# martingoe/physics

Hardware: AMD Instinct MI355X
Metric: rigid_body_steps_per_sec (higher is better)
Workload: dtype f32; 1 GPU; C5_256000_tower; n_bodies=256000, bodies_per_gpu=256000, dt_nanos=16666667, preroll_steps=30, rccl_ranks=0

## Files before the change

include/physics_hip.h:

```cpp
#ifndef PHYSICS_HIP_H
#define PHYSICS_HIP_H

#include <stdint.h>

#ifdef __cplusplus
extern "C" {
#endif

#define PHYS_ABI_VERSION 2u

#define PHYS_OK 0
#define PHYS_ERR_INVALID_ARG (-1)
#define PHYS_ERR_NO_DEVICE (-2)
#define PHYS_ERR_HIP (-3)
#define PHYS_ERR_SINGULAR_INERTIA (-4)
#define PHYS_ERR_CAPACITY (-5)
#define PHYS_ERR_OUT_OF_RANGE (-6)
#define PHYS_ERR_UNSUPPORTED (-7)
#define PHYS_ERR_NO_BODIES (-8)

#define PHYS_SHAPE_NONE 0u
#define PHYS_SHAPE_SPHERE 1u
#define PHYS_SHAPE_BOX 2u
#define PHYS_SHAPE_CAPSULE 3u

#define PHYS_FLAG_COLLISIONS 0x1u
#define PHYS_FLAG_GROUND_PLANE 0x2u
#define PHYS_FLAG_EXACT_ROTATION 0x4u
#define PHYS_FLAG_BROADPHASE_ONLY 0x8u
#define PHYS_FLAG_SOLVER_PER_COLOR 0x10u
#define PHYS_FLAG_SHARED_GPU 0x20u
#define PHYS_FLAG_EXCLUSIVE_GPU 0x80u
#define PHYS_FLAG_SOLVER_CLUSTER 0x40u
#define PHYS_FLAG_NO_WARM_START 0x100u

typedef struct phys_config {
    uint32_t abi_version;
    int32_t device;
    uint32_t flags;
    float gravity_force[3];
    float gravity_offset[3];
    uint32_t cg_max_iterations;
    float cg_max_error;
    float cg_min_error;
    uint32_t solver_iterations;
    float baumgarte;
    float slop;
    float friction;
    float contact_margin;
    float ground_height;
    float max_bias;
    uint64_t max_pairs;
    uint64_t max_manifolds;
    uint64_t max_ghosts;
} phys_config;

typedef struct phys_world phys_world;

typedef struct phys_stats {
    uint64_t n_bodies;
    uint64_t n_pairs;
    uint64_t n_manifolds;
    uint64_t n_contacts;
    uint32_t n_colors;
    uint32_t color_rounds;
    uint32_t cg_iterations;
    int32_t cg_converged;
    uint64_t steps;
    uint32_t overflow;
    uint32_t n_ground_manifolds;
    float max_extent;
    uint32_t n_halo_records;
    uint64_t n_cross_pairs;
    uint32_t n_ghosts;
    uint32_t n_new_manifolds;
} phys_stats;

void phys_config_default(phys_config* cfg);
const char* phys_last_error(void);
uint32_t phys_abi_version(void);

int32_t phys_create(const phys_config* cfg, phys_world** out);
int32_t phys_destroy(phys_world* w);

int32_t phys_set_bodies(phys_world* w, uint64_t n, const float* pos , const float* rot_ijkw ,
                        const float* lin_vel , const float* ang_vel , const float* mass ,
                        const float* inertia , const uint32_t* shape_type ,
                        const float* half_extent );

int32_t phys_add_constraint_fix_point(phys_world* w, uint64_t body, const float target[3]);
int32_t phys_add_constraint_fix_orientation(phys_world* w, uint64_t body, const float target_rpy[3]);
int32_t phys_clear_constraints(phys_world* w);

int32_t phys_apply_force_centre_of_gravity(phys_world* w, uint64_t body, const float force[3]);
int32_t phys_apply_force_at_position(phys_world* w, uint64_t body, const float force[3], const float point[3]);
int32_t phys_apply_force_at_offset(phys_world* w, uint64_t body, const float force[3], const float offset[3]);

int32_t phys_set_forces(phys_world* w, const float* force , const float* torque );

int32_t phys_update(phys_world* w, uint64_t dt_nanos);
int32_t phys_apply_gravity(phys_world* w);
int32_t phys_step(phys_world* w, uint64_t dt_nanos);
int32_t phys_update_n(phys_world* w, uint64_t dt_nanos, uint32_t n);
int32_t phys_sync(phys_world* w);

int32_t phys_get_transforms(phys_world* w, float* pos_out , float* rot_ijkw_out );
int32_t phys_get_velocities(phys_world* w, float* lin_out , float* ang_out );
int32_t phys_get_forces(phys_world* w, float* force_out , float* torque_out );
int32_t phys_get_instance_matrices(phys_world* w, float* out );
int32_t phys_get_lambda(phys_world* w, float* lambda_out, uint64_t cap, uint64_t* n_rows);

int32_t phys_block_spmv(int32_t device, uint64_t nrows, uint64_t ncols, uint64_t nblocks, const uint64_t* block_desc ,
                        const float* data, const float* vec, uint64_t vec_len, int32_t transpose, float* out);

int32_t phys_broadphase(phys_world* w, uint32_t* pairs_out , uint64_t cap, uint64_t* n_pairs);
int32_t phys_get_aabbs(phys_world* w, float* out );
int32_t phys_get_manifolds(phys_world* w, uint32_t* ids_out , uint32_t* counts_out ,
                           float* normals_out , float* points_out , uint64_t cap,
                           uint64_t* n_manifolds);
int32_t phys_get_stats(phys_world* w, phys_stats* out);
int32_t phys_get_color_counts(phys_world* w, uint32_t* counts_out );

#define PHYS_RAY_MISS 0xFFFFFFFEu
#define PHYS_RAY_GROUND 0xFFFFFFFFu
int32_t phys_raycast(phys_world* w, uint64_t n_rays, const float* origin , const float* dir ,
                     const float* max_t , const uint32_t* ignore_body ,
                     uint32_t* body_out , float* t_out , float* normal_out );
int32_t phys_raycast_device(phys_world* w, uint64_t n_rays, const float* origin, const float* dir, const float* max_t,
                            const uint32_t* ignore_body, uint32_t* body_out, float* t_out, float* normal_out);

int32_t phys_spherecast(phys_world* w, uint64_t n, const float* origin , const float* dir ,
                        const float* radius , const float* max_t ,
                        const uint32_t* ignore_body ,
                        uint32_t* body_out , float* t_out , float* normal_out );
int32_t phys_spherecast_device(phys_world* w, uint64_t n, const float* origin, const float* dir, const float* radius,
                               const float* max_t, const uint32_t* ignore_body, uint32_t* body_out, float* t_out,
                               float* normal_out);
int32_t phys_overlap(phys_world* w, uint64_t n, const uint32_t* shape_type , const float* pos ,
                     const float* rot_ijkw , const float* half_extent ,
                     const uint32_t* ignore_body ,
                     uint64_t cap, uint64_t* offsets_out , uint32_t* ids_out );

#define PHYS_STATIC_ID_BIT 0x80000000u
int32_t phys_set_static_bodies(phys_world* w, uint64_t n, const float* pos , const float* rot_ijkw ,
                               const uint32_t* shape_type , const float* half_extent );
int32_t phys_get_static_stats(phys_world* w, uint64_t* n_static, uint64_t* n_static_pairs, uint64_t* n_static_manifolds);

#define PHYS_FILTER_DEFAULT_CATEGORY 0x0001u
#define PHYS_FILTER_DEFAULT_MASK 0xFFFFu
int32_t phys_set_body_filters(phys_world* w, uint64_t n, const uint16_t* category ,
                              const uint16_t* mask , const int16_t* group );
int32_t phys_get_body_filters(phys_world* w, uint16_t* category_out , uint16_t* mask_out ,
                              int16_t* group_out );
int32_t phys_set_static_filters(phys_world* w, uint64_t n, const uint16_t* category ,
                                const uint16_t* mask , const int16_t* group );
int32_t phys_set_ground_filter(phys_world* w, uint16_t category, uint16_t mask);
int32_t phys_raycast_filtered(phys_world* w, uint64_t n_rays, const float* origin , const float* dir ,
                              const float* max_t , const uint32_t* ignore_body ,
                              const uint16_t* query_mask , uint32_t* body_out , float* t_out ,
                              float* normal_out );
int32_t phys_raycast_device_filtered(phys_world* w, uint64_t n_rays, const float* origin, const float* dir, const float* max_t,
                                     const uint32_t* ignore_body, const uint16_t* query_mask, uint32_t* body_out, float* t_out,
                                     float* normal_out);
int32_t phys_spherecast_filtered(phys_world* w, uint64_t n, const float* origin , const float* dir ,
                                 const float* radius , const float* max_t ,
                                 const uint32_t* ignore_body , const uint16_t* query_mask ,
                                 uint32_t* body_out , float* t_out , float* normal_out );
int32_t phys_spherecast_device_filtered(phys_world* w, uint64_t n, const float* origin, const float* dir, const float* radius,
                                        const float* max_t, const uint32_t* ignore_body, const uint16_t* query_mask,
                                        uint32_t* body_out, float* t_out, float* normal_out);
int32_t phys_overlap_filtered(phys_world* w, uint64_t n, const uint32_t* shape_type , const float* pos ,
                              const float* rot_ijkw , const float* half_extent ,
                              const uint32_t* ignore_body , const uint16_t* query_mask ,
                              uint64_t cap, uint64_t* offsets_out , uint32_t* ids_out );

int32_t phys_set_body_materials(phys_world* w, uint64_t n, const float* friction ,
                                const float* restitution );
int32_t phys_get_body_materials(phys_world* w, float* friction_out , float* restitution_out );
int32_t phys_set_static_materials(phys_world* w, uint64_t n, const float* friction ,
                                  const float* restitution );
int32_t phys_set_ground_material(phys_world* w, float friction, float restitution);
int32_t phys_set_restitution_threshold(phys_world* w, float v );

#define PHYS_CONTACT_BEGIN 1u
#define PHYS_CONTACT_END   2u
typedef struct phys_contact_event {
    uint32_t body_a, body_b;
    uint32_t kind;
    uint32_t step;
    float point[3];
    float impulse;
    float normal[3];
    uint32_t reserved;
} phys_contact_event;

int32_t phys_contact_events_enable(phys_world* w, uint64_t capacity);
int32_t phys_get_contact_events(phys_world* w, phys_contact_event* out, uint64_t cap, uint64_t* n, uint64_t* n_dropped);
int32_t phys_get_contact_impulses(phys_world* w, float* out , uint64_t cap, uint64_t* n_manifolds);

#define PHYS_MAX_TRIGGERS 1024u
#define PHYS_TRIGGER_ENTER 1u
#define PHYS_TRIGGER_EXIT  2u
typedef struct phys_trigger_event {
    uint32_t trigger;
    uint32_t body;
    uint32_t kind;
    uint32_t step;
} phys_trigger_event;

int32_t phys_set_triggers(phys_world* w, uint64_t n, const uint32_t* shape_type , const float* pos ,
                          const float* rot_ijkw , const float* half_extent ,
                          const uint16_t* mask );
int32_t phys_set_trigger_poses(phys_world* w, uint64_t n , const float* pos ,
                               const float* rot_ijkw );
int32_t phys_trigger_events_enable(phys_world* w, uint64_t capacity);
int32_t phys_get_trigger_events(phys_world* w, phys_trigger_event* out, uint64_t cap, uint64_t* n, uint64_t* n_dropped);
int32_t phys_get_trigger_overlaps(phys_world* w, uint64_t cap, uint64_t* offsets_out , uint32_t* ids_out );

#define PHYS_STAGE_STEP_FULL 0u
#define PHYS_STAGE_VELOCITY_AABB 1u
#define PHYS_STAGE_GRID 2u
#define PHYS_STAGE_PAIRS 3u
#define PHYS_STAGE_NARROW 4u
#define PHYS_STAGE_COLOR 5u
#define PHYS_STAGE_ROWS 6u
#define PHYS_STAGE_SOLVE 7u
#define PHYS_STAGE_POSITION 8u
#define PHYS_STAGE_CONSTRAINTS 9u
#define PHYS_STAGE_MISC 10u
#define PHYS_STAGE_SOLVE_TAIL 11u
#define PHYS_STAGE_SOLVE_FLOW 12u
#define PHYS_STAGE_SOLVE_CLUSTER 13u
#define PHYS_STAGE_COUNT 14u
typedef struct phys_profile {
    double ms[PHYS_STAGE_COUNT];
    uint64_t launches[PHYS_STAGE_COUNT];
    uint64_t steps;
} phys_profile;
int32_t phys_profile_enable(phys_world* w, int32_t on);
int32_t phys_profile_get(phys_world* w, phys_profile* out);

typedef struct phys_device_view {
    uint64_t n;
    float* pos;
    float* rot;
    float* lin_vel;
    float* ang_vel;
    float* aabb;
    void* stream;
    uint64_t vel_stride;
} phys_device_view;
int32_t phys_get_device_view(phys_world* w, phys_device_view* out);

int32_t phys_set_global_ids(phys_world* w, const uint32_t* global_ids );
int32_t phys_halo_pack(phys_world* w, float x_lo, float x_hi, float reach, void* dev_records_out, uint64_t cap,
                       uint64_t* n_records);
int32_t phys_halo_pairs(phys_world* w, const void* dev_remote_records, uint64_t n_remote, uint64_t skip_first,
                        uint64_t skip_count, uint64_t* n_cross_pairs);
int32_t phys_get_cross_pairs(phys_world* w, uint32_t* pairs_out , uint64_t cap, uint64_t* n_pairs);

#define PHYS_HALO_BODY_RECORD_BYTES 96u
int32_t phys_set_slab(phys_world* w, float x_lo, float x_hi, float reach);
int32_t phys_halo_pack_bodies(phys_world* w, void* dev_records_out, uint64_t cap);
int32_t phys_halo_pack_bodies_face(phys_world* w, void* dev_records_out, uint64_t cap, int32_t face);
int32_t phys_halo_unpack_ghosts(phys_world* w, const void* dev_records, uint64_t n_records, uint64_t skip_first,
                                uint64_t skip_count);
int32_t phys_get_global_ids(phys_world* w, uint32_t* out );

// ... 23 lines not shown
```

include/spec/collide.h:

```cpp
#ifndef PHYS_SPEC_COLLIDE_H
#define PHYS_SPEC_COLLIDE_H

#include <stdint.h>

#include "vec.h"

#define PHYS_GROUND_ID 0xFFFFFFFFu
#ifndef PHYS_STATIC_ID_BIT
#define PHYS_STATIC_ID_BIT 0x80000000u
#endif
#define PHYS_IS_STATIC_PARTNER(b) (((b) & PHYS_STATIC_ID_BIT) != 0u)
#define PHYS_SPEC_SHAPE_NONE 0u
#define PHYS_SPEC_SHAPE_SPHERE 1u
#define PHYS_SPEC_SHAPE_BOX 2u
#define PHYS_SPEC_SHAPE_CAPSULE 3u

typedef struct { v3 lo, hi; } aabb_t;

typedef struct {
    v3 c;
    m33 R;
    v3 h;
    uint32_t type;
} geom_t;
// ... 76 lines not shown

PHYS_HD void collide_sphere_sphere(const geom_t* A, const geom_t* B, float margin, manifold_t* m) {
    const v3 d = v3_sub(B->c, A->c);
    const float dist2 = v3_dot(d, d);
    const float r = A->h.x + B->h.x;
    const float reach = r + margin;
    if (dist2 > reach * reach) return;
    const float dist = det_sqrtf(dist2);
    v3 n = v3_make(0.0f, 1.0f, 0.0f);
    if (dist > 1.0e-12f) n = v3_div(d, dist);
    const float depth = r - dist;
    m->normal = n;
    m->count = 1;
    m->pt[0] = v3_add(A->c, v3_scale(n, A->h.x - 0.5f * depth));
    m->depth[0] = depth;
}

PHYS_HD void collide_sphere_box_raw(const geom_t* S, const geom_t* X, float margin, manifold_t* m) {
    const v3 p = m33_tmul_v3(&X->R, v3_sub(S->c, X->c));
    v3 q;
    q.x = det_maxf(-X->h.x, det_minf(p.x, X->h.x));
    q.y = det_maxf(-X->h.y, det_minf(p.y, X->h.y));
    q.z = det_maxf(-X->h.z, det_minf(p.z, X->h.z));
    const float r = S->h.x;
    v3 nl;
    float depth;
    if (q.x == p.x && q.y == p.y && q.z == p.z) {
        const float fx = X->h.x - det_absf(p.x), fy = X->h.y - det_absf(p.y), fz = X->h.z - det_absf(p.z);
        if (fx <= fy && fx <= fz) { nl = v3_make(p.x < 0.0f ? -1.0f : 1.0f, 0.0f, 0.0f); depth = fx + r; q.x = p.x < 0.0f ? -X->h.x : X->h.x; }
        else if (fy <= fz)        { nl = v3_make(0.0f, p.y < 0.0f ? -1.0f : 1.0f, 0.0f); depth = fy + r; q.y = p.y < 0.0f ? -X->h.y : X->h.y; }
        else                      { nl = v3_make(0.0f, 0.0f, p.z < 0.0f ? -1.0f : 1.0f); depth = fz + r; q.z = p.z < 0.0f ? -X->h.z : X->h.z; }
    } else {
        const v3 dl = v3_sub(p, q);
        const float dist2 = v3_dot(dl, dl);
        const float reach = r + margin;
        if (dist2 > reach * reach) return;
        const float dist = det_sqrtf(dist2);
        nl = v3_div(dl, dist);
        depth = r - dist;
    }
    const v3 nw = m33_mul_v3(&X->R, nl);
    m->normal = v3_neg(nw);
    m->count = 1;
    m->pt[0] = v3_add(X->c, m33_mul_v3(&X->R, q));
    m->depth[0] = depth;
}

PHYS_HD int clip_poly(v3* p, int n_in, v3 c, v3 u, float lim) {
    int n_out = 0;
    if (n_in <= 0) return 0;
    const v3 first = p[0];
    v3 a = first;
    float da = v3_dot(v3_sub(a, c), u) - lim;
    for (int k = 0; k < 8; ++k) {
        if (k >= n_in) break;
        v3 b = first;
        if (k + 1 != n_in) b = p[k + 1];
        const float db = v3_dot(v3_sub(b, c), u) - lim;
        if (da <= 0.0f) {
            if (n_out < 8) p[n_out++] = a;
            if (db > 0.0f) {
                const float t = da / (da - db);
                if (n_out < 8) p[n_out++] = v3_add(a, v3_scale(v3_sub(b, a), t));
            }
        } else if (db <= 0.0f) {
            const float t = da / (da - db);
            if (n_out < 8) p[n_out++] = v3_add(a, v3_scale(v3_sub(b, a), t));
        }
        a = b; da = db;
    }
    return n_out;
}

PHYS_HD void manifold_reduce(const v3* p, const float* depth, int n, v3 normal, manifold_t* m) {
    if (n <= 4) {
        m->count = n;
        PHYS_UNROLL
        for (int k = 0; k < 4; ++k) if (k < n) { m->pt[k] = p[k]; m->depth[k] = depth[k]; }
        return;
    }
    int i0 = 0;
    for (int k = 1; k < 8; ++k) if (k < n && depth[k] > depth[i0]) i0 = k;
    int i1 = -1; float best = -1.0f;
    for (int k = 0; k < 8; ++k) if (k < n && k != i0) {
        const v3 d = v3_sub(p[k], p[i0]);
        const float dd = v3_dot(d, d);
        if (dd > best) { best = dd; i1 = k; }
    }
    int i2 = -1, i3 = -1; float amax = 0.0f, amin = 0.0f;
    const v3 e = v3_sub(p[i1], p[i0]);
    for (int k = 0; k < 8; ++k) if (k < n && k != i0 && k != i1) {
        const float area = v3_dot(v3_cross(e, v3_sub(p[k], p[i0])), normal);
        if (area > amax) { amax = area; i2 = k; }
        if (area < amin) { amin = area; i3 = k; }
    }
    m->pt[0] = p[i0]; m->depth[0] = depth[i0];
    m->pt[1] = p[i1]; m->depth[1] = depth[i1];
    const int has2 = i2 >= 0, has3 = i3 >= 0;
    const int s2 = has2 ? i2 : i3;
    if (has2 || has3) { m->pt[2] = p[s2]; m->depth[2] = depth[s2]; }
    if (has2 && has3) { m->pt[3] = p[i3]; m->depth[3] = depth[i3]; }
    m->count = 2 + has2 + has3;
}

PHYS_HD void box_face_contact(const geom_t* Ref, const geom_t* Inc, int r, float sgn, float margin, v3 n_ab,
                              manifold_t* m, clip_ws_t* ws) {
    const v3 nref = v3_scale(m33_col(&Ref->R, r), sgn);
    const float d0 = v3_dot(nref, m33_col(&Inc->R, 0));
    const float d1 = v3_dot(nref, m33_col(&Inc->R, 1));
    const float d2 = v3_dot(nref, m33_col(&Inc->R, 2));
    int j = 0; float dj = d0;
    if (det_absf(d1) > det_absf(dj)) { j = 1; dj = d1; }
    if (det_absf(d2) > det_absf(dj)) { j = 2; dj = d2; }
    const float jsgn = dj > 0.0f ? -1.0f : 1.0f;
    const int j1 = (j + 1) % 3, j2 = (j + 2) % 3;
    const v3 fc = v3_add(Inc->c, v3_scale(m33_col(&Inc->R, j), jsgn * v3_get(Inc->h, j)));
    const v3 e1 = v3_scale(m33_col(&Inc->R, j1), v3_get(Inc->h, j1));
    const v3 e2 = v3_scale(m33_col(&Inc->R, j2), v3_get(Inc->h, j2));
    v3* polyA = ws->poly;
    polyA[0] = v3_add(v3_add(fc, e1), e2);
    polyA[1] = v3_add(v3_sub(fc, e1), e2);
    polyA[2] = v3_sub(v3_sub(fc, e1), e2);
    polyA[3] = v3_sub(v3_add(fc, e1), e2);
    int n = 4;
    const int r1 = (r + 1) % 3, r2 = (r + 2) % 3;
    const v3 u1 = m33_col(&Ref->R, r1), u2 = m33_col(&Ref->R, r2);
    const float l1 = v3_get(Ref->h, r1), l2 = v3_get(Ref->h, r2);
    n = clip_poly(polyA, n, Ref->c, u1, l1);
    n = clip_poly(polyA, n, Ref->c, v3_neg(u1), l1);
    n = clip_poly(polyA, n, Ref->c, u2, l2);
    n = clip_poly(polyA, n, Ref->c, v3_neg(u2), l2);
    float lo1 = 3.0e38f, hi1 = -3.0e38f, lo2 = 3.0e38f, hi2 = -3.0e38f;
    v3* cand = ws->poly; float* cdep = ws->depth; int nc = 0;
    const float hr = v3_get(Ref->h, r);
    float deepest = -3.0e38f;
    for (int k = 0; k < 8; ++k) {
        if (k >= n) break;
        const v3 rel = v3_sub(polyA[k], Ref->c);
        const float c1 = v3_dot(rel, u1), c2 = v3_dot(rel, u2);
        lo1 = det_minf(lo1, c1); hi1 = det_maxf(hi1, c1);
        lo2 = det_minf(lo2, c2); hi2 = det_maxf(hi2, c2);
        const float dep = hr - v3_dot(rel, nref);
        if (dep >= -margin) { cand[nc] = polyA[k]; cdep[nc] = dep; deepest = det_maxf(deepest, dep); ++nc; }
    }
    {
        const float kSliverRel = 0.1f, kSliverDepth = 0.25f;
        const float width = det_minf(hi1 - lo1, hi2 - lo2);
        const float face = det_minf(det_minf(l1, l2), det_minf(v3_get(Inc->h, j1), v3_get(Inc->h, j2)));
        if (nc > 0 && width < kSliverRel * face && deepest <= kSliverDepth * margin) nc = 0;
    }
    manifold_reduce(cand, cdep, nc, n_ab, m);
}

PHYS_HD void collide_box_box(const geom_t* A, const geom_t* B, float margin, manifold_t* m, clip_ws_t* ws) {
    const v3 d = v3_sub(B->c, A->c);
    float C[3][3], absC[3][3], tA[3], tB[3], hA[3], hB[3];
    hA[0] = A->h.x; hA[1] = A->h.y; hA[2] = A->h.z;
    hB[0] = B->h.x; hB[1] = B->h.y; hB[2] = B->h.z;
    PHYS_UNROLL
    for (int i = 0; i < 3; ++i) {
        const v3 ai = m33_col(&A->R, i);
        tA[i] = v3_dot(d, ai);
        PHYS_UNROLL
        for (int j = 0; j < 3; ++j) {
            C[i][j] = v3_dot(ai, m33_col(&B->R, j));
            absC[i][j] = det_absf(C[i][j]) + 1.0e-6f;
        }
    }
    PHYS_UNROLL
    for (int j = 0; j < 3; ++j) tB[j] = v3_dot(d, m33_col(&B->R, j));

    float aMax = -3.0e38f; int aAxis = 0;
    PHYS_UNROLL
    for (int i = 0; i < 3; ++i) {
        const float s = det_absf(tA[i]) - (hA[i] + ((absC[i][0] * hB[0] + absC[i][1] * hB[1]) + absC[i][2] * hB[2]));
        if (s > margin) return;
        if (s > aMax) { aMax = s; aAxis = i; }
    }
    float bMax = -3.0e38f; int bAxis = 0;
    PHYS_UNROLL
    for (int j = 0; j < 3; ++j) {
        const float s = det_absf(tB[j]) - (hB[j] + ((absC[0][j] * hA[0] + absC[1][j] * hA[1]) + absC[2][j] * hA[2]));
        if (s > margin) return;
        if (s > bMax) { bMax = s; bAxis = j; }
    }
    float eMax = -3.0e38f; int eI = -1, eJ = -1;
    PHYS_UNROLL
    for (int i = 0; i < 3; ++i) {
        const int i1 = (i + 1) % 3, i2 = (i + 2) % 3;
        PHYS_UNROLL
        for (int j = 0; j < 3; ++j) {
            const int j1 = (j + 1) % 3, j2 = (j + 2) % 3;
            const float len2 = 1.0f - C[i][j] * C[i][j];
            if (len2 < 1.0e-4f) continue;
            const float ra = hA[i1] * absC[i2][j] + hA[i2] * absC[i1][j];
            const float rb = hB[j1] * absC[i][j2] + hB[j2] * absC[i][j1];
            const float dist = det_absf(tA[i2] * C[i1][j] - tA[i1] * C[i2][j]);
            const float s = (dist - (ra + rb)) / det_sqrtf(len2);
            if (s > margin) return;
            if (s > eMax) { eMax = s; eI = i; eJ = j; }
        }
    }
    const float kRel = 0.95f, kAbs = 0.01f;
    const float faceMax = det_maxf(aMax, bMax);
    if (eI >= 0 && eMax > kRel * faceMax + kAbs) {
        const v3 ai = m33_col(&A->R, eI), bj = m33_col(&B->R, eJ);
        v3 n = v3_cross(ai, bj);
        const float nl = v3_norm(n);
        n = v3_div(n, nl);
        if (v3_dot(n, d) < 0.0f) n = v3_neg(n);
        v3 pA = A->c, pB = B->c;
        PHYS_UNROLL
        for (int k = 0; k < 3; ++k) {
            if (k != eI) {
                const v3 ak = m33_col(&A->R, k);
                const float sg = v3_dot(n, ak) > 0.0f ? 1.0f : -1.0f;
                pA = v3_add(pA, v3_scale(ak, sg * hA[k]));
            }
            if (k != eJ) {
                const v3 bk = m33_col(&B->R, k);
                const float sg = v3_dot(n, bk) > 0.0f ? -1.0f : 1.0f;
                pB = v3_add(pB, v3_scale(bk, sg * hB[k]));
            }
        }
        const v3 w = v3_sub(pA, pB);
        const float b = v3_dot(ai, bj);
        const float dd = v3_dot(ai, w), ee = v3_dot(bj, w);
        const float den = 1.0f - b * b;
        const float sa = (b * ee - dd) / den;
        const float tb = (ee - b * dd) / den;
        const v3 qa = v3_add(pA, v3_scale(ai, sa));
        const v3 qb = v3_add(pB, v3_scale(bj, tb));
        m->normal = n;
        m->count = 1;
        m->pt[0] = v3_scale(v3_add(qa, qb), 0.5f);
        m->depth[0] = -eMax;
        return;
    }
    if (bMax > kRel * aMax + kAbs) {
        const float sgn = sel3(tB, bAxis) > 0.0f ? -1.0f : 1.0f;
        const v3 nref = v3_scale(m33_col(&B->R, bAxis), sgn);
        m->normal = v3_neg(nref);
        box_face_contact(B, A, bAxis, sgn, margin, m->normal, m, ws);
    } else {
        const float sgn = sel3(tA, aAxis) < 0.0f ? -1.0f : 1.0f;
        m->normal = v3_scale(m33_col(&A->R, aAxis), sgn);
        box_face_contact(A, B, aAxis, sgn, margin, m->normal, m, ws);
    }
}

PHYS_HD void collide_pair_sphere_box(const geom_t* A, const geom_t* B, float margin, manifold_t* m, clip_ws_t* ws) {
    manifold_clear(m);
    if (A->type == PHYS_SPEC_SHAPE_SPHERE && B->type == PHYS_SPEC_SHAPE_SPHERE) {
        collide_sphere_sphere(A, B, margin, m);
    } else if (A->type == PHYS_SPEC_SHAPE_SPHERE && B->type == PHYS_SPEC_SHAPE_BOX) {
        collide_sphere_box_raw(A, B, margin, m);
    } else if (A->type == PHYS_SPEC_SHAPE_BOX && B->type == PHYS_SPEC_SHAPE_SPHERE) {
        collide_sphere_box_raw(B, A, margin, m);
        m->normal = v3_neg(m->normal);
    } else if (A->type == PHYS_SPEC_SHAPE_BOX && B->type == PHYS_SPEC_SHAPE_BOX) {
        collide_box_box(A, B, margin, m, ws);
    }
}

PHYS_HD void collide_ground_sphere_box(const geom_t* A, float ground, float margin, manifold_t* m, clip_ws_t* ws) {
    manifold_clear(m);
    m->normal = v3_make(0.0f, -1.0f, 0.0f);
    if (A->type == PHYS_SPEC_SHAPE_SPHERE) {
        const float bottom = A->c.y - A->h.x;
        const float depth = ground - bottom;
        if (depth < -margin) return;
        m->count = 1;
        m->pt[0] = v3_make(A->c.x, bottom + 0.5f * depth, A->c.z);
        m->depth[0] = depth;
    } else if (A->type == PHYS_SPEC_SHAPE_BOX) {
        v3* cand = ws->poly; float* cdep = ws->depth; int nc = 0;
        const v3 ex = v3_scale(m33_col(&A->R, 0), A->h.x);
        const v3 ey = v3_scale(m33_col(&A->R, 1), A->h.y);
        const v3 ez = v3_scale(m33_col(&A->R, 2), A->h.z);
        for (int k = 0; k < 8; ++k) {
            v3 p = A->c;
            p = (k & 1) ? v3_add(p, ex) : v3_sub(p, ex);
            p = (k & 2) ? v3_add(p, ey) : v3_sub(p, ey);
            p = (k & 4) ? v3_add(p, ez) : v3_sub(p, ez);
            const float depth = ground - p.y;
            if (depth >= -margin) { cand[nc] = p; cdep[nc] = depth; ++nc; }
        }
        if (nc == 0) return;
        manifold_reduce(cand, cdep, nc, v3_make(0.0f, 1.0f, 0.0f), m);
    }
}



PHYS_HD v3 capsule_axis(const geom_t* A) { return v3_make(A->R.m[1], A->R.m[4], A->R.m[7]); }

PHYS_HD geom_t capsule_ball(v3 p, float r) {
    geom_t g;
    g.c = p;
    g.R.m[0] = 1.0f; g.R.m[1] = 0.0f; g.R.m[2] = 0.0f;
    g.R.m[3] = 0.0f; g.R.m[4] = 1.0f; g.R.m[5] = 0.0f;
    g.R.m[6] = 0.0f; g.R.m[7] = 0.0f; g.R.m[8] = 1.0f;
    g.h = v3_make(r, r, r);
    g.type = PHYS_SPEC_SHAPE_SPHERE;
    return g;
}

PHYS_HD float segment_param(v3 c, v3 u, float hl, v3 p) {
    const float uu = v3_dot(u, u);
    float s = 0.0f;
    if (uu > 1.0e-12f) s = v3_dot(v3_sub(p, c), u) / uu;
    return det_maxf(-hl, det_minf(s, hl));
}

PHYS_HD void segment_closest(v3 ca, v3 ua, float ha, v3 cb, v3 ub, float hb, float* s_out, float* t_out) {
    const v3 r = v3_sub(ca, cb);
    const float a = v3_dot(ua, ua), e = v3_dot(ub, ub), b = v3_dot(ua, ub);
    const float c = v3_dot(ua, r), f = v3_dot(ub, r);
    const float denom = a * e - b * b;
    float s = 0.0f, t = 0.0f;
    if (denom > 1.0e-4f * (a * e)) s = det_maxf(-ha, det_minf((b * f - c * e) / denom, ha));
    if (e > 1.0e-12f) t = (b * s + f) / e;
    if (t < -hb || t > hb) {
        t = t < -hb ? -hb : hb;
        s = a > 1.0e-12f ? det_maxf(-ha, det_minf((b * t - c) / a, ha)) : 0.0f;
    }
    *s_out = s;
    *t_out = t;
}

PHYS_HD void collide_capsule_sphere(const geom_t* A, const geom_t* B, float margin, manifold_t* m) {
    const v3 u = capsule_axis(A);
    const float s = segment_param(A->c, u, A->h.y, B->c);
    const geom_t S = capsule_ball(v3_add(A->c, v3_scale(u, s)), A->h.x);
    collide_sphere_sphere(&S, B, margin, m);
}

PHYS_HD void collide_capsule_capsule(const geom_t* A, const geom_t* B, float margin, manifold_t* m) {
    const v3 ua = capsule_axis(A), ub = capsule_axis(B);
    const float ra = A->h.x, rb = B->h.x;
    const float a = v3_dot(ua, ua), e = v3_dot(ub, ub), b = v3_dot(ua, ub);
    if (a > 1.0e-12f && e > 1.0e-12f && a * e - b * b <= 1.0e-4f * (a * e)) {
        const v3 d = v3_sub(B->c, A->c);
        const float sb = v3_dot(d, ua) / a;
        const float pb = B->h.y * (det_absf(b) / a);
        const float lo = det_maxf(-A->h.y, sb - pb), hi = det_minf(A->h.y, sb + pb);
        if (lo < hi) {
            const v3 perp = v3_sub(d, v3_scale(ua, sb));
            const float dist = v3_norm(perp);
            v3 n = v3_make(0.0f, 1.0f, 0.0f);
            if (dist > 1.0e-12f) n = v3_div(perp, dist);
            const float r = ra + rb;
            int nc = 0;
            PHYS_UNROLL
            for (int k = 0; k < 2; ++k) {
                const float s = k == 0 ? lo : hi;
                const v3 pa = v3_add(A->c, v3_scale(ua, s));
                const float t = segment_param(B->c, ub, B->h.y, pa);
                const v3 qb = v3_add(B->c, v3_scale(ub, t));
                const float depth = r - v3_dot(v3_sub(qb, pa), n);
                if (depth >= -margin) {
                    const v3 p = v3_add(pa, v3_scale(n, ra - 0.5f * depth));
                    if (nc == 0) { m->pt[0] = p; m->depth[0] = depth; }
                    else { m->pt[1] = p; m->depth[1] = depth; }
                    ++nc;
                }
            }
            m->normal = n;
            m->count = nc;
            return;
        }
    }
    float s, t;
    segment_closest(A->c, ua, A->h.y, B->c, ub, B->h.y, &s, &t);
    const geom_t SA = capsule_ball(v3_add(A->c, v3_scale(ua, s)), ra);
    const geom_t SB = capsule_ball(v3_add(B->c, v3_scale(ub, t)), rb);
    collide_sphere_sphere(&SA, &SB, margin, m);
}

PHYS_HD void capsule_edge_closest(v3 pc, v3 dl, float hl, v3 qe, v3 ue, float he, float* best, v3* bp, v3* bq) {
    float s, t;
    segment_closest(pc, dl, hl, qe, ue, he, &s, &t);
    const v3 p = v3_add(pc, v3_scale(dl, s)), q = v3_add(qe, v3_scale(ue, t));
    const v3 d = v3_sub(p, q);
    const float d2 = v3_dot(d, d);
    if (d2 < *best) { *best = d2; *bp = p; *bq = q; }
}

PHYS_HD void capsule_face_edges(v3 pc, v3 dl, float hl, int f, float sg, v3 e, float* best, v3* bp, v3* bq) {
    const int ja = f == 0 ? 1 : 0, ka = f == 2 ? 1 : 2;
    const float ef = f == 0 ? e.x : (f == 1 ? e.y : e.z);
    PHYS_UNROLL
    for (int k = 0; k < 4; ++k) {
        const int along = k < 2 ? ka : ja, across = k < 2 ? ja : ka;
        const float side = (k & 1) ? 1.0f : -1.0f;
        const float ec = across == 0 ? e.x : (across == 1 ? e.y : e.z);
        const float qx = f == 0 ? sg * ef : (across == 0 ? side * ec : 0.0f);
        const float qy = f == 1 ? sg * ef : (across == 1 ? side * ec : 0.0f);
        const float qz = f == 2 ? sg * ef : (across == 2 ? side * ec : 0.0f);
        const v3 ue = v3_make(along == 0 ? 1.0f : 0.0f, along == 1 ? 1.0f : 0.0f, along == 2 ? 1.0f : 0.0f);
        const float he = along == 0 ? e.x : (along == 1 ? e.y : e.z);
        capsule_edge_closest(pc, dl, hl, v3_make(qx, qy, qz), ue, he, best, bp, bq);
    }
}

PHYS_HD void capsule_box_point(const geom_t* A, const geom_t* B, v3 p, v3 q, v3 nf, float sep_f, float margin, manifold_t* m) {
    const float r = A->h.x;
    const v3 d = v3_sub(p, q);
    const float dist = v3_norm(d);
    v3 n = nf;
    float depth = r - sep_f;
    if (sep_f > 0.0f && dist > 1.0e-6f) { n = v3_div(d, dist); depth = r - dist; }
    if (depth < -margin) return;
    m->normal = v3_neg(m33_mul_v3(&B->R, n));
    m->count = 1;
    m->pt[0] = v3_add(B->c, m33_mul_v3(&B->R, v3_sub(p, v3_scale(n, r - 0.5f * depth))));
    m->depth[0] = depth;
}

PHYS_HD void collide_capsule_box(const geom_t* A, const geom_t* B, float margin, manifold_t* m) {
    const float r = A->h.x, hl = A->h.y;
    const v3 pc = m33_tmul_v3(&B->R, v3_sub(A->c, B->c));
    const v3 dl = m33_tmul_v3(&B->R, capsule_axis(A));
    const float ex = B->h.x, ey = B->h.y, ez = B->h.z;
    const float fx = det_absf(pc.x) - (ex + hl * det_absf(dl.x));
    const float fy = det_absf(pc.y) - (ey + hl * det_absf(dl.y));
    const float fz = det_absf(pc.z) - (ez + hl * det_absf(dl.z));
    if (fx - r > margin || fy - r > margin || fz - r > margin) return;
    int fAxis = 0; float fMax = fx;
    if (fy > fMax) { fAxis = 1; fMax = fy; }
    if (fz > fMax) { fAxis = 2; fMax = fz; }
    float eMax = -3.0e38f; int eAxis = -1;
    PHYS_UNROLL
    for (int i = 0; i < 3; ++i) {
        const v3 n = i == 0 ? v3_make(0.0f, dl.z, -dl.y) : (i == 1 ? v3_make(-dl.z, 0.0f, dl.x) : v3_make(dl.y, -dl.x, 0.0f));
        const float len2 = v3_dot(n, n);
        if (len2 < 1.0e-4f) continue;
        const float rb = (ex * det_absf(n.x) + ey * det_absf(n.y)) + ez * det_absf(n.z);
        const float s = (det_absf(v3_dot(pc, n)) - rb) / det_sqrtf(len2);
        if (s - r > margin) return;
        if (s > eMax) { eMax = s; eAxis = i; }
    }
    v3 nl;
    if (eAxis >= 0 && eMax > fMax + (0.05f * det_absf(fMax) + 0.01f)) {
        v3 n = eAxis == 0 ? v3_make(0.0f, dl.z, -dl.y) : (eAxis == 1 ? v3_make(-dl.z, 0.0f, dl.x) : v3_make(dl.y, -dl.x, 0.0f));
        n = v3_div(n, v3_norm(n));
        if (v3_dot(n, pc) < 0.0f) n = v3_neg(n);
        const float sx = n.x > 0.0f ? ex : -ex, sy = n.y > 0.0f ? ey : -ey, sz = n.z > 0.0f ? ez : -ez;
        const v3 qe = v3_make(eAxis == 0 ? 0.0f : sx, eAxis == 1 ? 0.0f : sy, eAxis == 2 ? 0.0f : sz);
        const v3 ue = v3_make(eAxis == 0 ? 1.0f : 0.0f, eAxis == 1 ? 1.0f : 0.0f, eAxis == 2 ? 1.0f : 0.0f);
        const float he = eAxis == 0 ? ex : (eAxis == 1 ? ey : ez);
        float best = 3.0e38f;
        v3 p = pc, q = qe;
        capsule_edge_closest(pc, dl, hl, qe, ue, he, &best, &p, &q);
        capsule_box_point(A, B, p, q, n, eMax, margin, m);
        return;
    }
    const float pf = fAxis == 0 ? pc.x : (fAxis == 1 ? pc.y : pc.z);
    const float sg = pf < 0.0f ? -1.0f : 1.0f;
    float lo = -hl, hi = hl;
    PHYS_UNROLL
    for (int j = 0; j < 3; ++j) {
        if (j == fAxis) continue;
        const float pj = j == 0 ? pc.x : (j == 1 ? pc.y : pc.z);
        const float dj = j == 0 ? dl.x : (j == 1 ? dl.y : dl.z);
        const float ej = j == 0 ? ex : (j == 1 ? ey : ez);
        if (dj == 0.0f) {
            if (det_absf(pj) > ej) { lo = 1.0f; hi = -1.0f; }
        } else {
            const float t0 = (-ej - pj) / dj, t1 = (ej - pj) / dj;
            lo = det_maxf(lo, det_minf(t0, t1));
            hi = det_minf(hi, det_maxf(t0, t1));
        }
    }
    if (lo <= hi) {
        nl = v3_make(fAxis == 0 ? sg : 0.0f, fAxis == 1 ? sg : 0.0f, fAxis == 2 ? sg : 0.0f);
        const float ef = fAxis == 0 ? ex : (fAxis == 1 ? ey : ez);
        const int ends = lo < hi ? 2 : 1;
        int nc = 0;
        PHYS_UNROLL
        for (int k = 0; k < 2; ++k) {
            if (k >= ends) break;
            const float s = k == 0 ? lo : hi;
            const v3 pa = v3_add(pc, v3_scale(dl, s));
            const float paf = fAxis == 0 ? pa.x : (fAxis == 1 ? pa.y : pa.z);
            const float depth = r - (sg * paf - ef);
            if (depth >= -margin) {
                const v3 p = v3_add(B->c, m33_mul_v3(&B->R, v3_sub(pa, v3_scale(nl, r - 0.5f * depth))));
                if (nc == 0) { m->pt[0] = p; m->depth[0] = depth; }
                else { m->pt[1] = p; m->depth[1] = depth; }
                ++nc;
            }
        }
        m->normal = v3_neg(m33_mul_v3(&B->R, nl));
        m->count = nc;
        const float sep = det_maxf(fMax, eMax);
        if (sep > 0.0f) {
            float best = 3.0e38f;
            v3 p = pc, q = pc;
            capsule_face_edges(pc, dl, hl, fAxis, sg, B->h, &best, &p, &q);
            const float edge_depth = r - det_sqrtf(best);
            const float deepest = nc == 0 ? -3.0e38f : (nc == 1 ? m->depth[0] : det_maxf(m->depth[0], m->depth[1]));
            if (edge_depth > deepest + 1.0e-6f) {
                manifold_clear(m);
                capsule_box_point(A, B, p, q, nl, sep, margin, m);
            }
        }
        return;
    }
    float best = 3.0e38f;
    v3 p = pc, q = pc;
    capsule_face_edges(pc, dl, hl, fAxis, sg, B->h, &best, &p, &q);
    capsule_box_point(A, B, p, q, v3_make(fAxis == 0 ? sg : 0.0f, fAxis == 1 ? sg : 0.0f, fAxis == 2 ? sg : 0.0f),
                      det_maxf(fMax, eMax), margin, m);
}

PHYS_HD void collide_capsule_any(const geom_t* A, const geom_t* B, float margin, manifold_t* m) {
    if (B->type == PHYS_SPEC_SHAPE_SPHERE) collide_capsule_sphere(A, B, margin, m);
    else if (B->type == PHYS_SPEC_SHAPE_CAPSULE) collide_capsule_capsule(A, B, margin, m);
    else if (B->type == PHYS_SPEC_SHAPE_BOX) collide_capsule_box(A, B, margin, m);
}

PHYS_HD void collide_pair(const geom_t* A, const geom_t* B, float margin, manifold_t* m, clip_ws_t* ws) {
    if (A->type == PHYS_SPEC_SHAPE_CAPSULE) {
        manifold_clear(m);
        collide_capsule_any(A, B, margin, m);
    } else if (B->type == PHYS_SPEC_SHAPE_CAPSULE) {
        manifold_clear(m);
        if (A->type != PHYS_SPEC_SHAPE_NONE) {
            collide_capsule_any(B, A, margin, m);
            m->normal = v3_neg(m->normal);
        }
    } else {
        collide_pair_sphere_box(A, B, margin, m, ws);
    }
}

PHYS_HD void collide_capsule_ground(const geom_t* A, float ground, float margin, manifold_t* m) {
    const v3 ax = v3_scale(capsule_axis(A), A->h.y);
    const v3 p0 = v3_sub(A->c, ax), p1 = v3_add(A->c, ax);
    const float b0 = p0.y - A->h.x, b1 = p1.y - A->h.x;
    const float d0 = ground - b0, d1 = ground - b1;
    const int k0 = d0 >= -margin;
    const int k1 = d1 >= -margin && !(p0.x == p1.x && p0.y == p1.y && p0.z == p1.z);
    const v3 q0 = v3_make(p0.x, b0 + 0.5f * d0, p0.z), q1 = v3_make(p1.x, b1 + 0.5f * d1, p1.z);
    if (k0) { m->pt[0] = q0; m->depth[0] = d0; }
    if (k1) {
        if (k0) { m->pt[1] = q1; m->depth[1] = d1; }
        else { m->pt[0] = q1; m->depth[0] = d1; }
    }
    m->count = k0 + k1;
}

PHYS_HD void collide_ground(const geom_t* A, float ground, float margin, manifold_t* m, clip_ws_t* ws) {
    if (A->type == PHYS_SPEC_SHAPE_CAPSULE) {
        manifold_clear(m);
        m->normal = v3_make(0.0f, -1.0f, 0.0f);
        collide_capsule_ground(A, ground, margin, m);
    } else {
        collide_ground_sphere_box(A, ground, margin, m, ws);
    }
}

#endif
```

physics_amd/_abi.py:

```python
import ctypes as C
import os

PHYS_ABI_VERSION = 2

PHYS_OK = 0
PHYS_ERR_INVALID_ARG = -1
PHYS_ERR_NO_DEVICE = -2
PHYS_ERR_HIP = -3
PHYS_ERR_SINGULAR_INERTIA = -4
PHYS_ERR_CAPACITY = -5
PHYS_ERR_OUT_OF_RANGE = -6
PHYS_ERR_UNSUPPORTED = -7
PHYS_ERR_NO_BODIES = -8

SHAPE_NONE, SHAPE_SPHERE, SHAPE_BOX = 0, 1, 2
SHAPE_CAPSULE = 3
FLAG_COLLISIONS, FLAG_GROUND_PLANE, FLAG_EXACT_ROTATION, FLAG_BROADPHASE_ONLY = 1, 2, 4, 8
FLAG_SOLVER_PER_COLOR = 16
FLAG_SHARED_GPU = 32
FLAG_SOLVER_CLUSTER = 64
FLAG_EXCLUSIVE_GPU = 128
FLAG_NO_WARM_START = 256
GROUND_ID = 0xFFFFFFFF
RAY_MISS = 0xFFFFFFFE
RAY_GROUND = 0xFFFFFFFF
STATIC_ID_BIT = 0x80000000
FILTER_DEFAULT_CATEGORY = 0x0001
FILTER_DEFAULT_MASK = 0xFFFF
CONTACT_BEGIN, CONTACT_END = 1, 2
MAX_TRIGGERS = 1024
TRIGGER_ENTER, TRIGGER_EXIT = 1, 2

f32p = C.POINTER(C.c_float)
u32p = C.POINTER(C.c_uint32)
u64p = C.POINTER(C.c_uint64)
u16p = C.POINTER(C.c_uint16)
i16p = C.POINTER(C.c_int16)


class PhysConfig(C.Structure):
    _fields_ = [
        ("abi_version", C.c_uint32),
        ("device", C.c_int32),
        ("flags", C.c_uint32),
        ("gravity_force", C.c_float * 3),
        ("gravity_offset", C.c_float * 3),
        ("cg_max_iterations", C.c_uint32),
        ("cg_max_error", C.c_float),
        ("cg_min_error", C.c_float),
        ("solver_iterations", C.c_uint32),
        ("baumgarte", C.c_float),
        ("slop", C.c_float),
        ("friction", C.c_float),
        ("contact_margin", C.c_float),
        ("ground_height", C.c_float),
        ("max_bias", C.c_float),
        ("max_pairs", C.c_uint64),
        ("max_manifolds", C.c_uint64),
        ("max_ghosts", C.c_uint64),
    ]


class PhysStats(C.Structure):
    _fields_ = [
        ("n_bodies", C.c_uint64),
        ("n_pairs", C.c_uint64),
        ("n_manifolds", C.c_uint64),
        ("n_contacts", C.c_uint64),
        ("n_colors", C.c_uint32),
        ("color_rounds", C.c_uint32),
        ("cg_iterations", C.c_uint32),
        ("cg_converged", C.c_int32),
        ("steps", C.c_uint64),
        ("overflow", C.c_uint32),
        ("n_ground_manifolds", C.c_uint32),
        ("max_extent", C.c_float),
        ("n_halo_records", C.c_uint32),
        ("n_cross_pairs", C.c_uint64),
        ("n_ghosts", C.c_uint32),
        ("n_new_manifolds", C.c_uint32),
    ]


STAGE_COUNT = 14
STAGE_NAMES = ["step_full", "velocity_aabb", "grid", "pairs", "narrow", "color", "rows", "solve", "position",
               "constraints", "misc", "solve_tail", "solve_flow", "solve_cluster"]


class PhysProfile(C.Structure):
    _fields_ = [("ms", C.c_double * STAGE_COUNT), ("launches", C.c_uint64 * STAGE_COUNT), ("steps", C.c_uint64)]


class PhysDeviceView(C.Structure):
    _fields_ = [
        ("n", C.c_uint64),
        ("pos", C.c_void_p),
        ("rot", C.c_void_p),
        ("lin_vel", C.c_void_p),
        ("ang_vel", C.c_void_p),
        ("aabb", C.c_void_p),
        ("stream", C.c_void_p),
        ("vel_stride", C.c_uint64),
    ]


class PhysContactEvent(C.Structure):
    _fields_ = [
        ("body_a", C.c_uint32),
        ("body_b", C.c_uint32),
        ("kind", C.c_uint32),
        ("step", C.c_uint32),
        ("point", C.c_float * 3),
        ("impulse", C.c_float),
        ("normal", C.c_float * 3),
        ("reserved", C.c_uint32),
    ]


class PhysTriggerEvent(C.Structure):
    _fields_ = [("trigger", C.c_uint32), ("body", C.c_uint32), ("kind", C.c_uint32), ("step", C.c_uint32)]


def default_config(**overrides):
    cfg = PhysConfig()
    cfg.abi_version = PHYS_ABI_VERSION
    cfg.device = 0
    cfg.flags = 0
    cfg.gravity_force[:] = (0.0, -9.81, 0.0)
    cfg.gravity_offset[:] = (0.0, 0.0, 1.5)
    cfg.cg_max_iterations = 1000
    cfg.cg_max_error = 1e-2
    cfg.cg_min_error = 1e-3
    cfg.solver_iterations = 8
    cfg.baumgarte = 0.2
    cfg.slop = 0.01
    cfg.friction = 0.5
    cfg.contact_margin = 0.02
    cfg.ground_height = 0.0
    cfg.max_bias = 3.0
    cfg.max_pairs = 0
    cfg.max_manifolds = 0
    cfg.max_ghosts = 0
    for k, v in overrides.items():
        if k in ("gravity_force", "gravity_offset"):
            getattr(cfg, k)[:] = tuple(v)
        else:
            setattr(cfg, k, v)
    return cfg


PROTOTYPES = {
    "phys_config_default": (None, [C.POINTER(PhysConfig)]),
    "phys_last_error": (C.c_char_p, []),
    "phys_abi_version": (C.c_uint32, []),
    "phys_create": (C.c_int32, [C.POINTER(PhysConfig), C.POINTER(C.c_void_p)]),
    "phys_destroy": (C.c_int32, [C.c_void_p]),
    "phys_set_bodies": (C.c_int32, [C.c_void_p, C.c_uint64, f32p, f32p, f32p, f32p, f32p, f32p, u32p, f32p]),
    "phys_add_constraint_fix_point": (C.c_int32, [C.c_void_p, C.c_uint64, f32p]),
    "phys_add_constraint_fix_orientation": (C.c_int32, [C.c_void_p, C.c_uint64, f32p]),
    "phys_clear_constraints": (C.c_int32, [C.c_void_p]),
    "phys_apply_force_centre_of_gravity": (C.c_int32, [C.c_void_p, C.c_uint64, f32p]),
    "phys_apply_force_at_position": (C.c_int32, [C.c_void_p, C.c_uint64, f32p, f32p]),
    "phys_apply_force_at_offset": (C.c_int32, [C.c_void_p, C.c_uint64, f32p, f32p]),
    "phys_set_forces": (C.c_int32, [C.c_void_p, f32p, f32p]),
    "phys_update": (C.c_int32, [C.c_void_p, C.c_uint64]),
    "phys_apply_gravity": (C.c_int32, [C.c_void_p]),
    "phys_step": (C.c_int32, [C.c_void_p, C.c_uint64]),
    "phys_update_n": (C.c_int32, [C.c_void_p, C.c_uint64, C.c_uint32]),
    "phys_sync": (C.c_int32, [C.c_void_p]),
    "phys_get_transforms": (C.c_int32, [C.c_void_p, f32p, f32p]),
    "phys_get_velocities": (C.c_int32, [C.c_void_p, f32p, f32p]),
    "phys_get_forces": (C.c_int32, [C.c_void_p, f32p, f32p]),
    "phys_get_instance_matrices": (C.c_int32, [C.c_void_p, f32p]),
    "phys_get_lambda": (C.c_int32, [C.c_void_p, f32p, C.c_uint64, u64p]),
    "phys_block_spmv": (C.c_int32, [C.c_int32, C.c_uint64, C.c_uint64, C.c_uint64, u64p, f32p, f32p, C.c_uint64, C.c_int32, f32p]),
    "phys_broadphase": (C.c_int32, [C.c_void_p, u32p, C.c_uint64, u64p]),
    "phys_get_aabbs": (C.c_int32, [C.c_void_p, f32p]),
    "phys_get_manifolds": (C.c_int32, [C.c_void_p, u32p, u32p, f32p, f32p, C.c_uint64, u64p]),
    "phys_get_stats": (C.c_int32, [C.c_void_p, C.POINTER(PhysStats)]),
    "phys_get_color_counts": (C.c_int32, [C.c_void_p, u32p]),
    "phys_raycast": (C.c_int32, [C.c_void_p, C.c_uint64, f32p, f32p, f32p, u32p, u32p, f32p, f32p]),
    "phys_raycast_device": (C.c_int32, [C.c_void_p, C.c_uint64, C.c_void_p, C.c_void_p, C.c_void_p, C.c_void_p, C.c_void_p,
                                        C.c_void_p, C.c_void_p]),
    "phys_spherecast": (C.c_int32, [C.c_void_p, C.c_uint64, f32p, f32p, f32p, f32p, u32p, u32p, f32p, f32p]),
    "phys_spherecast_device": (C.c_int32, [C.c_void_p, C.c_uint64, C.c_void_p, C.c_void_p, C.c_void_p, C.c_void_p, C.c_void_p,
                                           C.c_void_p, C.c_void_p, C.c_void_p]),
    "phys_overlap": (C.c_int32, [C.c_void_p, C.c_uint64, u32p, f32p, f32p, f32p, u32p, C.c_uint64, u64p, u32p]),
    "phys_set_static_bodies": (C.c_int32, [C.c_void_p, C.c_uint64, f32p, f32p, u32p, f32p]),
    "phys_set_body_filters": (C.c_int32, [C.c_void_p, C.c_uint64, u16p, u16p, i16p]),
    "phys_get_body_filters": (C.c_int32, [C.c_void_p, u16p, u16p, i16p]),
    "phys_set_static_filters": (C.c_int32, [C.c_void_p, C.c_uint64, u16p, u16p, i16p]),
    "phys_set_ground_filter": (C.c_int32, [C.c_void_p, C.c_uint16, C.c_uint16]),
    "phys_raycast_filtered": (C.c_int32, [C.c_void_p, C.c_uint64, f32p, f32p, f32p, u32p, u16p, u32p, f32p, f32p]),
    "phys_raycast_device_filtered": (C.c_int32, [C.c_void_p, C.c_uint64, C.c_void_p, C.c_void_p, C.c_void_p, C.c_void_p,
                                                 C.c_void_p, C.c_void_p, C.c_void_p, C.c_void_p]),
    "phys_spherecast_filtered": (C.c_int32, [C.c_void_p, C.c_uint64, f32p, f32p, f32p, f32p, u32p, u16p, u32p, f32p, f32p]),
    "phys_spherecast_device_filtered": (C.c_int32, [C.c_void_p, C.c_uint64, C.c_void_p, C.c_void_p, C.c_void_p, C.c_void_p,
                                                    C.c_void_p, C.c_void_p, C.c_void_p, C.c_void_p, C.c_void_p]),
    "phys_overlap_filtered": (C.c_int32, [C.c_void_p, C.c_uint64, u32p, f32p, f32p, f32p, u32p, u16p, C.c_uint64, u64p, u32p]),
    "phys_set_body_materials": (C.c_int32, [C.c_void_p, C.c_uint64, f32p, f32p]),
    "phys_get_body_materials": (C.c_int32, [C.c_void_p, f32p, f32p]),
    "phys_set_static_materials": (C.c_int32, [C.c_void_p, C.c_uint64, f32p, f32p]),
    "phys_set_ground_material": (C.c_int32, [C.c_void_p, C.c_float, C.c_float]),
    "phys_set_restitution_threshold": (C.c_int32, [C.c_void_p, C.c_float]),
    "phys_get_static_stats": (C.c_int32, [C.c_void_p, u64p, u64p, u64p]),
    "phys_contact_events_enable": (C.c_int32, [C.c_void_p, C.c_uint64]),
    "phys_get_contact_events": (C.c_int32, [C.c_void_p, C.POINTER(PhysContactEvent), C.c_uint64, u64p, u64p]),
    "phys_get_contact_impulses": (C.c_int32, [C.c_void_p, f32p, C.c_uint64, u64p]),
    "phys_set_triggers": (C.c_int32, [C.c_void_p, C.c_uint64, u32p, f32p, f32p, f32p, u16p]),
    "phys_set_trigger_poses": (C.c_int32, [C.c_void_p, C.c_uint64, f32p, f32p]),
    "phys_trigger_events_enable": (C.c_int32, [C.c_void_p, C.c_uint64]),
    "phys_get_trigger_events": (C.c_int32, [C.c_void_p, C.POINTER(PhysTriggerEvent), C.c_uint64, u64p, u64p]),
    "phys_get_trigger_overlaps": (C.c_int32, [C.c_void_p, C.c_uint64, u64p, u32p]),
    "phys_profile_enable": (C.c_int32, [C.c_void_p, C.c_int32]),
    "phys_profile_get": (C.c_int32, [C.c_void_p, C.POINTER(PhysProfile)]),
    "phys_get_device_view": (C.c_int32, [C.c_void_p, C.POINTER(PhysDeviceView)]),
    "phys_set_global_ids": (C.c_int32, [C.c_void_p, u32p]),
    "phys_halo_pack": (C.c_int32, [C.c_void_p, C.c_float, C.c_float, C.c_float, C.c_void_p, C.c_uint64, u64p]),
    "phys_halo_pairs": (C.c_int32, [C.c_void_p, C.c_void_p, C.c_uint64, C.c_uint64, C.c_uint64, u64p]),
    "phys_get_cross_pairs": (C.c_int32, [C.c_void_p, u32p, C.c_uint64, u64p]),
    "phys_set_slab": (C.c_int32, [C.c_void_p, C.c_float, C.c_float, C.c_float]),
    "phys_halo_pack_bodies": (C.c_int32, [C.c_void_p, C.c_void_p, C.c_uint64]),
    "phys_halo_pack_bodies_face": (C.c_int32, [C.c_void_p, C.c_void_p, C.c_uint64, C.c_int32]),
    "phys_halo_unpack_ghosts": (C.c_int32, [C.c_void_p, C.c_void_p, C.c_uint64, C.c_uint64, C.c_uint64]),
    "phys_get_global_ids": (C.c_int32, [C.c_void_p, u32p]),
    "phys_comm_unique_id": (C.c_int32, [C.POINTER(C.c_uint8)]),
    "phys_comm_create": (C.c_int32, [C.c_void_p, C.POINTER(C.c_uint8), C.c_int32, C.c_int32, C.c_uint64, C.POINTER(C.c_void_p)]),
    "phys_comm_create_local": (C.c_int32, [C.POINTER(C.c_void_p), C.c_int32, C.c_uint64, C.POINTER(C.c_void_p)]),
    "phys_comm_destroy": (C.c_int32, [C.c_void_p]),
    "phys_comm_set_neighbours": (C.c_int32, [C.c_void_p, C.c_int32]),
    "phys_halo_exchange": (C.c_int32, [C.c_void_p, C.c_void_p]),
    "phys_halo_exchange_all": (C.c_int32, [C.POINTER(C.c_void_p), C.POINTER(C.c_void_p), C.c_int32]),
    "phys_slab_histogram": (C.c_int32, [f32p, C.c_uint64, C.c_float, C.c_float, C.c_uint32, u64p]),
    "phys_slab_cuts": (C.c_int32, [u64p, C.c_uint32, C.c_float, C.c_float, C.c_int32, f32p]),
    "phys_slab_owners": (C.c_int32, [f32p, C.c_uint64, f32p, C.c_int32, C.POINTER(C.c_int32)]),
}

LIB_PATH = os.path.join(os.path.dirname(os.path.abspath(__file__)), "csrc", "libphysics_hip.so")
_lib = None


class PhysicsHipMissing(RuntimeError):
    pass


def rocm_runtime_mapped():
    try:
        return sorted({line.split()[-1] for line in open("/proc/self/maps") if "libamdhip64" in line})
    except OSError:
        return []


def torch_bundled_rocm_dir():
    import importlib.util
    try:
        spec = importlib.util.find_spec("torch")
    except (ImportError, ValueError):
        return None
    if spec is None or not spec.origin:
        return None
    d = os.path.join(os.path.dirname(spec.origin), "lib")
    return d if os.path.exists(os.path.join(d, "libamdhip64.so")) else None


def share_rocm_runtime_with_torch():
    if os.environ.get("PHYS_ROCM_RUNTIME") == "system" or rocm_runtime_mapped():
        return None
    d = torch_bundled_rocm_dir()
    if d is None:
        return None
    for name in ("libhsa-runtime64.so", "libamdhip64.so"):
        path = os.path.join(d, name)
        if os.path.exists(path):
            C.CDLL(path, mode=C.RTLD_GLOBAL)
    rccl = os.path.join(d, "librccl.so")
    if os.path.exists(rccl):
        os.environ.setdefault("PHYS_RCCL_PATH", rccl)
    return d


def load_library():
    global _lib
    if _lib is not None:
        return _lib
    if not os.path.exists(LIB_PATH):
        raise PhysicsHipMissing(
            f"{LIB_PATH} not found: build it with `python -c 'import __graft_entry__ as g; g.build()'` "
            "(hipcc --offload-arch=gfx950). physics_amd has no CPU fallback.")
    share_rocm_runtime_with_torch()
    lib = C.CDLL(LIB_PATH)
    for name, (res, args) in PROTOTYPES.items():
        fn = getattr(lib, name)
        fn.restype = res
        fn.argtypes = args
    _lib = lib
    return lib
```

physics_amd/csrc/abi.hip:

```cpp
#include <algorithm>
#include <atomic>
#include <cmath>
#include <cstdlib>
#include <cstring>
#include <limits>
#include <string>
#include <vector>

#include "kernels.hpp"

namespace phys {
static thread_local std::string g_error;
void set_error(const std::string& msg) { g_error = msg; }
const char* get_error() { return g_error.c_str(); }
}

using namespace phys;

namespace phys {
void poll_snapshots(phys_world* w);
StepCounters* snapshot_acquire(phys_world* w) {
    const uint32_t k = w->snap_next;
    if (w->snap_pending[k]) {
        (void)hipEventSynchronize(w->snap_event[k]);
        poll_snapshots(w);
    }
    if (!w->h_snap[k]) {
        if (hipHostMalloc((void**)&w->h_snap[k], sizeof(StepCounters), hipHostMallocDefault) != hipSuccess) return nullptr;
        if (hipEventCreateWithFlags(&w->snap_event[k], hipEventDisableTiming) != hipSuccess) return nullptr;
    }
    return w->h_snap[k];
}
void snapshot_commit(phys_world* w, bool full) {
    const uint32_t k = w->snap_next;
    (void)hipEventRecord(w->snap_event[k], w->stream);
    w->snap_pending[k] = true;
    w->snap_full[k] = full;
    w->snap_next = (k + 1) % phys_world::kSnapRing;
}
void snapshot_counters_async(phys_world* w, bool full) {
    StepCounters* slot = snapshot_acquire(w);
    if (!slot) return;
    (void)hipMemcpyAsync(slot, w->counters.p, sizeof(StepCounters), hipMemcpyDeviceToHost, w->stream);
    snapshot_commit(w, full);
}

void hint_adopt(StepHint& hint, const StepCounters& c, bool full, bool exact) {
    hint.valid = true;
    hint.n_manifolds = c.n_manifolds;
    hint.n_pairs = c.n_pairs;
    hint.n_contacts = c.n_contacts;
    if (c.max_region) hint.max_region = c.max_region;
    hint.n_used_buckets = c.n_used_buckets;
    hint.n_colors = c.n_colors;
    if (c.n_active) hint.n_active = c.n_active;
    if (full) {
        hint.full_rounds = c.color_rounds;
    } else if (exact) {
        hint.color_rounds = c.color_rounds;
    } else {
        hint.recent_new[hint.recent_pos % 8] = c.n_new_manifolds;
        hint.recent_rounds[hint.recent_pos++ % 8] = c.color_rounds;
        uint32_t mx = 0, mn = 0;
        for (int q = 0; q < 8; ++q) {
            mx = hint.recent_rounds[q] > mx ? hint.recent_rounds[q] : mx;
            mn = hint.recent_new[q] > mn ? hint.recent_new[q] : mn;
        }
        hint.color_rounds = mx;
        hint.n_new = mn;
    }
    for (int q = 0; q < kMaxColors; ++q) hint.color_count[q] = c.color_count[q];
}

void poll_snapshots(phys_world* w) {
    for (int i = 0; i < phys_world::kSnapRing; ++i) {
        const uint32_t k = (w->snap_next + i) % phys_world::kSnapRing;
        if (!w->snap_pending[k]) continue;
        if (hipEventQuery(w->snap_event[k]) != hipSuccess) {
            (void)hipGetLastError();
            continue;
        }
        const StepCounters& c = *w->h_snap[k];
        w->snap_pending[k] = false;
        w->host_sticky_overflow |= c.overflow | c.sticky_overflow;
        if (c.n_static_pairs > w->static_pairs_seen) w->static_pairs_seen = c.n_static_pairs;
        if (c.overflow) continue;
        hint_adopt(w->hint, c, w->snap_full[k], false);
    }
}
}

namespace phys {
static std::atomic<int> g_worlds[64];
int worlds_on_device(int device) { return g_worlds[device & 63].load(std::memory_order_relaxed); }
bool gpu_is_exclusive(const phys_world* w) {
    return (w->cfg.flags & PHYS_FLAG_EXCLUSIVE_GPU) && !(w->cfg.flags & PHYS_FLAG_SHARED_GPU) && worlds_on_device(w->device) == 1;
}

static PlanInputs plan_inputs(const phys_world* w) {
    PlanInputs in;
    in.flags = w->cfg.flags; in.solver_iterations = w->cfg.solver_iterations;
    in.n = w->n; in.n_owned = w->n_owned; in.max_manifolds = w->max_manifolds;
    in.grid_table_size = w->grid_table_size;
    in.cus = w->cus;
    in.exclusive = gpu_is_exclusive(w);
    in.warm = w->warm;
    in.flow_vel = w->flow_vel.p != nullptr;
    in.cluster_count = w->cluster_count; in.cluster_dynamic = w->cluster_dynamic;
    in.ctab_valid = w->ctab_valid; in.color_epoch = w->color_epoch;
    uint64_t st_cap = 0;
    const uint32_t* st_pairs = nullptr;
    const float* st_geo = nullptr;
    static_narrow_args(w, &st_cap, &st_pairs, &st_geo);
    const uint64_t n_ground = (w->cfg.flags & PHYS_FLAG_GROUND_PLANE) ? (uint32_t)w->n : 0u;
    in.statics = st_pairs != nullptr;
    in.capsules = w->body_capsules || (in.statics && w->static_capsules) || w->max_ghosts > 0;
    in.filters = w->body_filters_set || (in.statics && w->static_filters_set) || (n_ground && w->ground_filter_set) || w->max_ghosts > 0;
    in.materials = materials_active(w);
    in.np_items = n_ground + w->max_pairs + st_cap;
    return in;
}

template <class Parse>
static auto debug_env(const char* name, Parse parse) -> std::optional<decltype(parse(""))> {
    if (const char* v = getenv(name)) return parse(v);
    return std::nullopt;
}
static bool debug_set(const char* name) { return getenv(name) != nullptr; }
static uint64_t parse_u64(const char* v) { return strtoull(v, nullptr, 10); }
static bool parse_one(const char* v) { return v[0] == '1'; }

const DebugSwitches& debug_switches() {
    static const DebugSwitches d = [] {
        DebugSwitches s;
        s.no_cluster = debug_set("PHYS_DEBUG_NO_CLUSTER");
        s.cluster_min = debug_env("PHYS_DEBUG_CLUSTER_MIN", parse_u64);
        s.clusters_per_cu = debug_env("PHYS_DEBUG_CLUSTERS_PER_CU", atoi);
        s.cluster_dynamic = debug_set("PHYS_DEBUG_CLUSTER_DYNAMIC");
        s.cluster_cap = debug_env("PHYS_DEBUG_CLUSTER_CAP", parse_u64).value_or(0);
        s.flow_max = debug_env("PHYS_DEBUG_FLOW_MAX", parse_u64);
        s.flow_quad_max = debug_env("PHYS_DEBUG_FLOW_QUAD_MAX", parse_u64).value_or(0);
        s.flow_pipeline = debug_env("PHYS_DEBUG_FLOW_PIPELINE", parse_one);
        s.np_early_probe = debug_env("PHYS_DEBUG_NP_EARLY_PROBE", parse_one);
        s.no_flow_preference = debug_set("PHYS_DEBUG_NO_FLOW_PREFERENCE");
        s.flow_stall = debug_set("PHYS_DEBUG_FLOW_STALL");
        s.flow_epoch = debug_env("PHYS_DEBUG_FLOW_EPOCH", [](const char* v) { return (uint32_t)strtoul(v, nullptr, 0); }).value_or(0u);
        s.ctab_slots = debug_env("PHYS_DEBUG_CTAB_SLOTS", parse_u64).value_or(0);
        s.color_kernel_lane = debug_env("PHYS_DEBUG_COLOR_KERNEL", [](const char* v) { return v[0] == 'l'; });
        s.np_threads = debug_env("PHYS_DEBUG_NP_THREADS", atoi).value_or(0);
        s.pair_lanes = debug_env("PHYS_DEBUG_PAIR_LANES", atoi).value_or(0);
        s.pair_kernel_brick = debug_env("PHYS_DEBUG_PAIR_KERNEL", [](const char* v) { return v[0] != 'b' || v[1] == 'r'; });
        s.brick_stage = debug_env("PHYS_DEBUG_BRICK_STAGE", atoi).value_or(0);
        s.raycast_stats = debug_set("PHYS_DEBUG_RAYCAST_STATS");
        return s;
    }();
    return d;
}
}

static float duration_as_secs_f32(uint64_t nanos_total) {
    const uint64_t secs = nanos_total / 1000000000ull;
    const uint32_t nanos = (uint32_t)(nanos_total % 1000000000ull);
    return (float)secs + (float)nanos / 1.0e9f;
}

phys_world::~phys_world() {
    (void)hipSetDevice(device);
    if (stream) (void)hipStreamSynchronize(stream);
    prof.destroy();
    for (int k = 0; k < kSnapRing; ++k) {
        if (h_snap[k]) (void)hipHostFree(h_snap[k]);
        if (snap_event[k]) (void)hipEventDestroy(snap_event[k]);
    }
    if (h_counters) (void)hipHostFree(h_counters);
    if (stream) (void)hipStreamDestroy(stream);
}

template <typename T>
static int32_t upload_pairs(phys_world* w, DevBuf<T>& dst, const std::vector<T>& h, bool& set_flag) {
    if (!h.empty()) PHYS_HIP_TRY(hipMemcpyAsync(dst.p, h.data(), sizeof(T) * h.size(), hipMemcpyHostToDevice, w->stream));
    PHYS_HIP_TRY(hipStreamSynchronize(w->stream));
    set_flag = true;
    return PHYS_OK;
}
template <typename T>
static int32_t download_body_pairs(phys_world* w, const DevBuf<T>& src, std::vector<T>& h) {
    h.resize(2 * w->n_owned);
    if (!h.empty()) PHYS_HIP_TRY(hipMemcpyAsync(h.data(), src.p, sizeof(T) * h.size(), hipMemcpyDeviceToHost, w->stream));
    PHYS_HIP_TRY(hipStreamSynchronize(w->stream));
    return PHYS_OK;
}

struct Staging {
    struct Array { void* host; size_t bytes, offset; };
    template <typename T>
    struct Slot { size_t offset; bool there; };
    phys_world* w;
    DevBuf<uint8_t>& buf;
    Array arrays[6] = {};
    int count = 0;
    size_t total = 0;
    template <typename T>
    Slot<T> add(const T* host, size_t n, size_t align = alignof(T)) {
        if (!host) return {0, false};
        const size_t offset = (total + align - 1) / align * align;
        arrays[count++] = {const_cast<T*>(host), n * sizeof(T), offset};
        total = offset + n * sizeof(T);
        return {offset, true};
    }
    int32_t reserve() { PHYS_HIP_TRY(buf.resize(total)); return PHYS_OK; }
    template <typename T>
    T* at(Slot<T> s) const { return s.there ? reinterpret_cast<T*>(buf.p + s.offset) : nullptr; }
    int32_t copy(hipMemcpyKind kind) {
        for (int k = 0; k < count; ++k) {
            const Array& a = arrays[k];
            if (kind == hipMemcpyHostToDevice) PHYS_HIP_TRY(hipMemcpyAsync(buf.p + a.offset, a.host, a.bytes, kind, w->stream));
            else PHYS_HIP_TRY(hipMemcpyAsync(a.host, buf.p + a.offset, a.bytes, kind, w->stream));
        }
        return PHYS_OK;
    }
};

extern "C" {

void phys_config_default(phys_config* cfg) {
    if (!cfg) return;
    std::memset(cfg, 0, sizeof(*cfg));
    cfg->abi_version = PHYS_ABI_VERSION;
    cfg->device = 0;
    cfg->flags = 0;
    cfg->gravity_force[0] = 0.0f; cfg->gravity_force[1] = -9.81f; cfg->gravity_force[2] = 0.0f;
    cfg->gravity_offset[0] = 0.0f; cfg->gravity_offset[1] = 0.0f; cfg->gravity_offset[2] = 1.5f;
    cfg->cg_max_iterations = 1000;
    cfg->cg_max_error = 1e-2f;
    cfg->cg_min_error = 1e-3f;
    cfg->solver_iterations = 8;
    cfg->baumgarte = 0.2f;
    cfg->slop = 0.01f;
    cfg->friction = 0.5f;
    cfg->contact_margin = 0.02f;
    cfg->ground_height = 0.0f;
    cfg->max_bias = 3.0f;
    cfg->max_pairs = 0;
    cfg->max_manifolds = 0;
    cfg->max_ghosts = 0;
}

const char* phys_last_error(void) { return get_error(); }
uint32_t phys_abi_version(void) { return PHYS_ABI_VERSION; }

int32_t phys_create(const phys_config* cfg, phys_world** out) {
    if (!cfg || !out) return fail(PHYS_ERR_INVALID_ARG, "null argument");
    if (cfg->abi_version != PHYS_ABI_VERSION) return fail(PHYS_ERR_INVALID_ARG, "phys_config.abi_version mismatch");
    int count = 0;
    if (hipGetDeviceCount(&count) != hipSuccess || count <= 0)
        return fail(PHYS_ERR_NO_DEVICE, "no HIP device visible: libphysics_hip has no CPU fallback");
    if (cfg->device < 0 || cfg->device >= count) return fail(PHYS_ERR_NO_DEVICE, "device ordinal out of range");
    hipDeviceProp_t prop;
    PHYS_HIP_TRY(hipGetDeviceProperties(&prop, cfg->device));
    if (std::strncmp(prop.gcnArchName, "gfx950", 6) != 0)
        return fail(PHYS_ERR_NO_DEVICE, "device is not gfx950 (MI355X); this library carries gfx950 code only");
    PHYS_HIP_TRY(hipSetDevice(cfg->device));
    int cus = 0;
    PHYS_HIP_TRY(hipDeviceGetAttribute(&cus, hipDeviceAttributeMultiprocessorCount, cfg->device));
    phys_world* w = new phys_world();
    w->cfg = *cfg;
    w->device = cfg->device;
    w->cus = cus;
    hipError_t e = hipStreamCreateWithFlags(&w->stream, hipStreamNonBlocking);
    if (e != hipSuccess) { delete w; return fail(PHYS_ERR_HIP, "hipStreamCreate failed"); }
    e = w->counters.resize(1);
    if (e == hipSuccess) e = hipHostMalloc((void**)&w->h_counters, sizeof(StepCounters), hipHostMallocDefault);
    if (e == hipSuccess) e = hipMemsetAsync(w->counters.p, 0, sizeof(StepCounters), w->stream);
    if (e != hipSuccess) { delete w; return fail(PHYS_ERR_HIP, "counter allocation failed"); }
    std::memset(w->h_counters, 0, sizeof(StepCounters));
    phys::g_worlds[w->device & 63].fetch_add(1);
    *out = w;
    return PHYS_OK;
}

int32_t phys_destroy(phys_world* w) {
    if (!w) return PHYS_OK;
    phys::g_worlds[w->device & 63].fetch_sub(1);
    delete w;
    return PHYS_OK;
}

int32_t phys_set_bodies(phys_world* w, uint64_t n, const float* pos, const float* rot, const float* lin,
                        const float* ang, const float* mass, const float* inertia, const uint32_t* shape_type,
                        const float* half_extent) {
    ENTER(w);
    if (n && !pos) return fail(PHYS_ERR_INVALID_ARG, "pos is required");
    if (n >= 0x7FFFFFFFull) return fail(PHYS_ERR_INVALID_ARG, "too many bodies (u32 indices)");
    PHYS_HIP_TRY(hipStreamSynchronize(w->stream));
    const uint64_t G = (w->cfg.flags & PHYS_FLAG_COLLISIONS) && !(w->cfg.flags & PHYS_FLAG_BROADPHASE_ONLY) ? w->cfg.max_ghosts : 0;
    const uint64_t nt = n ? n + G : 0;
// ... 115 lines not shown

int32_t phys_step(phys_world* w, uint64_t dt_nanos) {
    ENTER(w);
    if (w->singular_inertia) return fail(PHYS_ERR_SINGULAR_INERTIA, "singular inertia tensor (reference: unwrap panic, rigid_body.rs:31)");
    launch_step_full(w, duration_as_secs_f32(dt_nanos), false);
    PHYS_HIP_TRY(hipGetLastError());
    return PHYS_OK;
}

static int32_t enqueue_update(phys_world* w, float dt) {
    const bool collisions = (w->cfg.flags & PHYS_FLAG_COLLISIONS) != 0 && dt > 0.0f;
    if (collisions) poll_snapshots(w);
    const DebugSwitches& dbg = debug_switches();
    const bool have_constraints = !w->constraints.empty();
    bool gravity_pending = true;
    if (have_constraints) {
        PHYS_TRY(constraints_alloc(w));
        launch_constraint_phase(w, gravity_pending);
    }
    if (!collisions) {
        launch_step_full(w, dt, gravity_pending, have_constraints);
    } else {
        const bool restart_extent = w->steps % 32 == 0 || w->step_zero_reset_bytes % 16 != 0 || (w->step_zero_reset_bytes >> 36) != 0;
        if (restart_extent) zero_step_state(w, true);
        launch_step_velocity_aabb(w, dt, gravity_pending, !restart_extent, have_constraints);
        launch_broadphase(w, plan_pairs(plan_inputs(w), w->hint, dbg));
        if (!(w->cfg.flags & PHYS_FLAG_BROADPHASE_ONLY)) {
            PHYS_TRY(launch_static_pairs(w));
            const PlanInputs in = plan_inputs(w);
            launch_narrowphase(w, plan_narrowphase(in, w->hint, dbg));
            const ColorPlan coloring = plan_coloring(in, w->hint, dbg);
            const bool cluster = coloring.wants_cluster && (!w->cluster_dynamic || cluster_plan_dynamic(w, w->hint, dbg));
            launch_coloring(w, coloring, cluster);
            launch_solver(w, dt, plan_solver(in, w->hint, dbg, cluster), coloring);
            if (w->ev_capacity) launch_events(w, (uint32_t)(w->steps + 1), plan_event_blocks(in, w->hint));
        } else {
            snapshot_counters_async(w, false);
        }
        launch_step_position(w, dt);
    }
    if (w->n_triggers) launch_triggers(w, (uint32_t)(w->steps + 1));
    PHYS_HIP_TRY(hipGetLastError());
    w->steps++;
    if (w->prof.on) { w->prof.steps++; if (w->prof.used > 4096) w->prof.collect(w->stream); }
    return PHYS_OK;
}

int32_t phys_update_n(phys_world* w, uint64_t dt_nanos, uint32_t n) {
    ENTER(w);
    if (w->n == 0) return fail(PHYS_ERR_NO_BODIES, "update with no bodies (reference: index panic, physics.rs:48)");
    if (w->singular_inertia) return fail(PHYS_ERR_SINGULAR_INERTIA, "singular inertia tensor (reference: unwrap panic, rigid_body.rs:31)");
    const float dt = duration_as_secs_f32(dt_nanos);
    for (uint32_t k = 0; k < n; ++k) PHYS_TRY(enqueue_update(w, dt));
    return PHYS_OK;
}

int32_t phys_update(phys_world* w, uint64_t dt_nanos) { return phys_update_n(w, dt_nanos, 1); }

int32_t phys_sync(phys_world* w) {
    ENTER(w);
    PHYS_TRY(fetch_counters(w));
    poll_snapshots(w);
    const uint32_t bits = w->h_counters->overflow | w->h_counters->sticky_overflow | w->host_sticky_overflow;
    if (w->h_counters->n_static_pairs > w->static_pairs_seen) w->static_pairs_seen = w->h_counters->n_static_pairs;
    w->host_sticky_overflow = 0;
    if (w->h_counters->sticky_overflow) {
        PHYS_HIP_TRY(hipMemsetAsync(&w->counters.p->sticky_overflow, 0, sizeof(uint32_t), w->stream));
        PHYS_HIP_TRY(hipStreamSynchronize(w->stream));
    }
    if (!(bits & kOvfCorruptRow) && w->h_counters->debug[0] != 0u) {
        PHYS_HIP_TRY(hipMemsetAsync(w->counters.p->debug, 0, sizeof(w->counters.p->debug), w->stream));
        PHYS_HIP_TRY(hipStreamSynchronize(w->stream));
    }
    const SyncError err = sync_error(bits, w->h_counters->debug);
    return err.code == PHYS_OK ? PHYS_OK : fail(err.code, err.message.c_str());
}

static int32_t d2h(phys_world* w, void* dst, const void* src, size_t bytes) {
    if (!dst || bytes == 0) return PHYS_OK;
    PHYS_HIP_TRY(hipMemcpyAsync(dst, src, bytes, hipMemcpyDeviceToHost, w->stream));
    return PHYS_OK;
}

int32_t phys_get_transforms(phys_world* w, float* pos_out, float* rot_out) {
    ENTER(w);
    PHYS_TRY(d2h(w, pos_out, w->pos.p, 12 * w->n_owned));
    PHYS_TRY(d2h(w, rot_out, w->rot.p, 16 * w->n_owned));
    PHYS_HIP_TRY(hipStreamSynchronize(w->stream));
    return PHYS_OK;
}
int32_t phys_get_velocities(phys_world* w, float* lin_out, float* ang_out) {
    ENTER(w);
    if (lin_out && w->n_owned) PHYS_HIP_TRY(hipMemcpy2DAsync(lin_out, 12, w->vel.p, 32, 12, w->n_owned, hipMemcpyDeviceToHost, w->stream));
    if (ang_out && w->n_owned) PHYS_HIP_TRY(hipMemcpy2DAsync(ang_out, 12, w->vel.p + 4, 32, 12, w->n_owned, hipMemcpyDeviceToHost, w->stream));
    PHYS_HIP_TRY(hipStreamSynchronize(w->stream));
    return PHYS_OK;
}
int32_t phys_get_forces(phys_world* w, float* force_out, float* torque_out) {
    ENTER(w);
    PHYS_TRY(d2h(w, force_out, w->force.p, 12 * w->n_owned));
    PHYS_TRY(d2h(w, torque_out, w->torque.p, 12 * w->n_owned));
    PHYS_HIP_TRY(hipStreamSynchronize(w->stream));
    return PHYS_OK;
}

int32_t phys_get_instance_matrices(phys_world* w, float* out) {
    ENTER(w);
    if (!out) return fail(PHYS_ERR_INVALID_ARG, "null output");
    if (w->n == 0) return PHYS_OK;
    DevBuf<float> d;
    PHYS_HIP_TRY(d.resize(16 * w->n));
    launch_instance_matrices(w, d.p);
    PHYS_HIP_TRY(hipMemcpyAsync(out, d.p, 64 * w->n_owned, hipMemcpyDeviceToHost, w->stream));
    PHYS_HIP_TRY(hipStreamSynchronize(w->stream));
    return PHYS_OK;
}

int32_t phys_get_lambda(phys_world* w, float* lambda_out, uint64_t cap, uint64_t* n_rows) {
    ENTER(w);
    if (!n_rows) return fail(PHYS_ERR_INVALID_ARG, "null n_rows");
    PHYS_HIP_TRY(hipStreamSynchronize(w->stream));
    uint32_t st[4] = {0, 0, 0, 0};
    if (w->cg_status.p && !w->constraints_dirty) PHYS_HIP_TRY(hipMemcpy(st, w->cg_status.p, 16, hipMemcpyDeviceToHost));
    const uint64_t rows = st[2] ? 3 * (uint64_t)w->constraints.size() : 0;
    *n_rows = rows;
    if (lambda_out && rows) {
        const uint64_t m = rows < cap ? rows : cap;
        PHYS_HIP_TRY(hipMemcpy(lambda_out, w->cg_x.p, 4 * m, hipMemcpyDeviceToHost));
    }
    return PHYS_OK;
}

int32_t phys_get_aabbs(phys_world* w, float* out) {
    ENTER(w);
    if (!out) return fail(PHYS_ERR_INVALID_ARG, "null output");
    launch_aabb_only(w);
    PHYS_TRY(d2h(w, out, w->aabb.p, 24 * w->n_owned));
    PHYS_HIP_TRY(hipStreamSynchronize(w->stream));
    return PHYS_OK;
}

int32_t phys_broadphase(phys_world* w, uint32_t* pairs_out, uint64_t cap, uint64_t* n_pairs) {
    ENTER(w);
    if (!n_pairs) return fail(PHYS_ERR_INVALID_ARG, "null n_pairs");
    if (!(w->cfg.flags & PHYS_FLAG_COLLISIONS)) return fail(PHYS_ERR_UNSUPPORTED, "world created without PHYS_FLAG_COLLISIONS");
    if (w->n == 0) { *n_pairs = 0; return PHYS_OK; }
    zero_step_state(w, true);
    launch_aabb_only(w);
    launch_broadphase(w, plan_pairs(plan_inputs(w), w->hint, debug_switches()));
    PHYS_HIP_TRY(hipGetLastError());
    return sorted_pairs_to_host(w, pairs_out, cap, n_pairs);
}

int32_t phys_get_manifolds(phys_world* w, uint32_t* ids_out, uint32_t* counts_out, float* normals_out,
                           float* points_out, uint64_t cap, uint64_t* n_manifolds) {
    ENTER(w);
    if (!n_manifolds) return fail(PHYS_ERR_INVALID_ARG, "null n_manifolds");
    PHYS_TRY(fetch_counters(w));
    const uint64_t m = w->h_counters->n_manifolds < w->max_manifolds ? w->h_counters->n_manifolds : w->max_manifolds;
    *n_manifolds = m;
    if (m == 0 || (!ids_out && !counts_out && !normals_out && !points_out)) return PHYS_OK;
    std::vector<uint32_t> ab(2 * m), c(m);
    std::vector<float> nrm(3 * m), pts(16 * m);
    {
        std::vector<float> geo(32 * m);
        PHYS_HIP_TRY(hipMemcpy(geo.data(), w->man_geo.p, 128 * m, hipMemcpyDeviceToHost));
        for (uint64_t k = 0; k < m; ++k) {
            const float* g = &geo[32 * k];
            std::memcpy(&ab[2 * k], g, 8); std::memcpy(&c[k], g + 2, 4);
            std::memcpy(&nrm[3 * k], g + 4, 12);
            std::memcpy(&pts[16 * k], g + 8, 64);
        }
    }
    const std::vector<uint64_t> order = manifold_order(ab.data(), 2, m);
    for (uint64_t k = 0; k < m && k < cap; ++k) {
        const uint64_t s = order[k];
        if (ids_out) { ids_out[2 * k] = ab[2 * s]; ids_out[2 * k + 1] = ab[2 * s + 1]; }
        if (counts_out) counts_out[k] = c[s];
        if (normals_out) std::memcpy(normals_out + 3 * k, &nrm[3 * s], 12);
        if (points_out) std::memcpy(points_out + 16 * k, &pts[16 * s], 64);
    }
    return PHYS_OK;
}

int32_t phys_get_stats(phys_world* w, phys_stats* out) {
    ENTER(w);
    if (!out) return fail(PHYS_ERR_INVALID_ARG, "null output");
    PHYS_TRY(fetch_counters(w));
    std::memset(out, 0, sizeof(*out));
    const StepCounters& c = *w->h_counters;
    out->n_bodies = w->n_owned;
    out->n_pairs = c.n_pairs;
    out->n_manifolds = c.n_manifolds;
    out->n_contacts = c.n_contacts;
    out->n_colors = c.n_colors;
    out->color_rounds = c.color_rounds;
    out->n_new_manifolds = c.n_new_manifolds;
    if (w->cg_status.p && !w->constraints.empty()) {
        uint32_t st[2] = {1, 0};
        PHYS_HIP_TRY(hipMemcpy(st, w->cg_status.p, 8, hipMemcpyDeviceToHost));
        out->cg_converged = (int32_t)st[0];
        out->cg_iterations = st[1];
    } else {
        out->cg_converged = 1;
        out->cg_iterations = w->steps ? 1u : 0u;
    }
    out->steps = w->steps;
    out->overflow = c.overflow | c.sticky_overflow | w->host_sticky_overflow;
    out->n_ground_manifolds = c.n_ground_manifolds;
    std::memcpy(&out->max_extent, &c.max_extent_bits, 4);
    out->n_halo_records = c.n_halo + c.n_halo_low;
    out->n_cross_pairs = c.n_cross_pairs;
    out->n_ghosts = c.n_ghosts;
    return PHYS_OK;
}

int32_t phys_set_static_bodies(phys_world* w, uint64_t n, const float* pos, const float* rot, const uint32_t* shape_type,
                               const float* half_extent) {
    if (n >= 0x7FFFFFFEull) return fail(PHYS_ERR_INVALID_ARG, "too many static colliders (ids are PHYS_STATIC_ID_BIT | k below 0x7FFFFFFE)");
    if (n && (!pos || !shape_type || !half_extent)) return fail(PHYS_ERR_INVALID_ARG, "static colliders need pos, shape_type and half_extent");
    std::string bad;
    if (shape_set_error("static collider", n, shape_type, pos, rot, half_extent, bad)) return fail(PHYS_ERR_INVALID_ARG, bad.c_str());
    ENTER(w);
    w->ctab_valid = false;
    w->color_epoch = 0;
    w->static_pairs_seen = 0;
    w->static_filters_set = false;
    w->static_materials_set = false;
    PHYS_TRY(events_reset(w));
    return static_set(w, n, pos, rot, shape_type, half_extent);
}

static int32_t set_filters(phys_world* w, DevBuf<uint32_t>& dst, uint64_t expected, bool& set_flag, const char* wrong_count,
                           uint64_t n, const uint16_t* category, const uint16_t* mask, const int16_t* group) {
    if (n != expected) return fail(PHYS_ERR_INVALID_ARG, wrong_count);
    std::vector<uint32_t> h;
    pack_filters(n, category, mask, group, h);
    return upload_pairs(w, dst, h, set_flag);
}

int32_t phys_set_body_filters(phys_world* w, uint64_t n, const uint16_t* category, const uint16_t* mask, const int16_t* group) {
    ENTER(w);
    return set_filters(w, w->filt, w->n_owned, w->body_filters_set, "phys_set_body_filters: n must equal the body count", n, category, mask, group);
}

int32_t phys_set_static_filters(phys_world* w, uint64_t n, const uint16_t* category, const uint16_t* mask, const int16_t* group) {
    ENTER(w);
    return set_filters(w, w->st_filt, w->n_static, w->static_filters_set, "phys_set_static_filters: n must equal the static collider count", n,
                       category, mask, group);
}

int32_t phys_get_body_filters(phys_world* w, uint16_t* category_out, uint16_t* mask_out, int16_t* group_out) {
    ENTER(w);
    std::vector<uint32_t> h;
    PHYS_TRY(download_body_pairs(w, w->filt, h));
    for (uint64_t k = 0; k < w->n_owned; ++k) {
        if (category_out) category_out[k] = (uint16_t)(h[2 * k] & 0xFFFFu);
        if (mask_out) mask_out[k] = (uint16_t)(h[2 * k] >> 16);
        if (group_out) group_out[k] = (int16_t)(uint16_t)h[2 * k + 1];
    }
    return PHYS_OK;
}

int32_t phys_set_ground_filter(phys_world* w, uint16_t category, uint16_t mask) {
    ENTER(w);
    w->ground_filt = (uint32_t)category | ((uint32_t)mask << 16);
    w->ground_filter_set = true;
    return PHYS_OK;
}

static const char* const kMaterialRange = "a friction must be finite and >= 0, a restitution in [0, 1]";
#define PHYS_NO_MATERIALS_WHEN_SHARDED(w) \
    do { if ((w)->cfg.max_ghosts > 0) return fail(PHYS_ERR_UNSUPPORTED, "materials are not supported in a world with max_ghosts > 0"); } while (0)

static int32_t set_materials(phys_world* w, DevBuf<float>& dst, uint64_t expected, bool& set_flag, const char* wrong_count, uint64_t n,
                             const float* friction, const float* restitution) {
    PHYS_NO_MATERIALS_WHEN_SHARDED(w);
    if (n != expected) return fail(PHYS_ERR_INVALID_ARG, wrong_count);
    std::vector<float> h;
    if (!pack_materials(n, friction, restitution, w->cfg.friction, h)) return fail(PHYS_ERR_INVALID_ARG, kMaterialRange);
    return upload_pairs(w, dst, h, set_flag);
}

int32_t phys_set_body_materials(phys_world* w, uint64_t n, const float* friction, const float* restitution) {
    ENTER(w);
    return set_materials(w, w->mat, w->n_owned, w->body_materials_set, "phys_set_body_materials: n must equal the body count", n, friction, restitution);
}

int32_t phys_set_static_materials(phys_world* w, uint64_t n, const float* friction, const float* restitution) {
    ENTER(w);
    return set_materials(w, w->st_mat, w->n_static, w->static_materials_set, "phys_set_static_materials: n must equal the static collider count", n,
                         friction, restitution);
}

int32_t phys_get_body_materials(phys_world* w, float* friction_out, float* restitution_out) {
    ENTER(w);
    PHYS_NO_MATERIALS_WHEN_SHARDED(w);
    std::vector<float> h;
    PHYS_TRY(download_body_pairs(w, w->mat, h));
    for (uint64_t k = 0; k < w->n_owned; ++k) {
        if (friction_out) friction_out[k] = h[2 * k];
        if (restitution_out) restitution_out[k] = h[2 * k + 1];
    }
    return PHYS_OK;
}

// ... 286 lines not shown
```

physics_amd/csrc/broadphase.hip:

```cpp
#include <algorithm>
#include <vector>

#include <cstdlib>

#include "kernels.hpp"

namespace phys {

constexpr uint32_t kInvalid = 0xFFFFFFFFu;

__device__ __forceinline__ float grid_inv_cell(const StepCounters* ctr) {
    const float ext = __uint_as_float(ctr->max_extent_bits);
    const float cell = ext > 0.0f ? ext * 1.001f : 1.0f;
    return 1.0f / cell;
}

__global__ __launch_bounds__(256) void k_cell_assign(uint32_t n, const float* __restrict__ aabb,
                                                     const uint32_t* __restrict__ shape,
                                                     const StepCounters* __restrict__ ctr, GridShape axis_mask,
                                                     uint32_t* __restrict__ bucket_of, uint32_t* __restrict__ rank,
                                                     uint32_t* __restrict__ bucket_count) {
    const uint32_t i = blockIdx.x * blockDim.x + threadIdx.x;
    if (i >= n) return;
    if (shape[i] == PHYS_SPEC_SHAPE_NONE) { bucket_of[i] = kInvalid; return; }
    const float inv_cell = grid_inv_cell(ctr);
    const v3 lo = ld3(aabb, 2 * i), hi = ld3(aabb, 2 * i + 1);
    const int cx = grid_cell_coord(0.5f * (lo.x + hi.x), inv_cell);
    const int cy = grid_cell_coord(0.5f * (lo.y + hi.y), inv_cell);
    const int cz = grid_cell_coord(0.5f * (lo.z + hi.z), inv_cell);
    const uint32_t bk = grid_bucket(cx, cy, cz, axis_mask);
    bucket_of[i] = bk;
    rank[i] = atomicAdd(&bucket_count[bk], 1u);
}

__global__ __launch_bounds__(256) void k_scatter(uint32_t n, const float* __restrict__ aabb,
                                                 const uint32_t* __restrict__ bucket_of,
                                                 const uint32_t* __restrict__ rank,
                                                 const uint32_t* __restrict__ bucket_start,
                                                 uint32_t* __restrict__ sorted_ids, float* __restrict__ sorted_box) {
    const uint32_t i = blockIdx.x * blockDim.x + threadIdx.x;
    if (i >= n) return;
    const uint32_t bk = bucket_of[i];
    if (bk == kInvalid) return;
    const uint32_t s = bucket_start[bk] + rank[i];
    sorted_ids[s] = i;
    st3(sorted_box, 2 * s, ld3(aabb, 2 * i));
    st3(sorted_box, 2 * s + 1, ld3(aabb, 2 * i + 1));
}

constexpr int kStagePerWave = 512;

struct PairStage {
    uint32_t* lds;
    uint32_t count;
};

__device__ __forceinline__ void stage_flush(PairStage& st, uint32_t* __restrict__ pairs, uint64_t max_pairs,
                                            StepCounters* __restrict__ ctr) {
    const int lane = threadIdx.x & 63;
    if (st.count == 0) return;
    uint32_t base = 0;
    if (lane == 0) base = atomicAdd(&ctr->n_pairs, st.count);
    base = (uint32_t)__shfl((int)base, 0, 64);
    if ((uint64_t)base + st.count > max_pairs) {
        if (lane == 0) flag_overflow(ctr, kOvfPairs);
    }
    for (uint32_t k = lane; k < st.count; k += 64) {
        const uint64_t dst = (uint64_t)base + k;
        if (dst < max_pairs) {
            const uint2 pr = reinterpret_cast<const uint2*>(st.lds)[k];
            reinterpret_cast<uint2*>(pairs)[dst] = pr;
        }
    }
    st.count = 0;
}

template <int kStageCap = kStagePerWave>
__device__ __forceinline__ void stage_push(PairStage& st, bool hit, uint32_t a, uint32_t b,
                                           uint32_t* __restrict__ pairs, uint64_t max_pairs,
                                           StepCounters* __restrict__ ctr) {
    const unsigned long long mask = __ballot(hit);
    if (mask == 0ull) return;
    const uint32_t hits = (uint32_t)__popcll(mask);
    if (st.count + hits > (uint32_t)kStageCap) stage_flush(st, pairs, max_pairs, ctr);
    if (hit) reinterpret_cast<uint2*>(st.lds)[st.count + lane_rank(mask)] = make_uint2(a, b);
    st.count += hits;
}

template <int kLanesPerBody>
__global__ __launch_bounds__(kPairThreads) void k_find_pairs(const uint32_t* __restrict__ bucket_start,
                                                             uint32_t table_size, GridShape axis_mask,
                                                             const uint32_t* __restrict__ sorted_ids,
                                                             const float* __restrict__ sorted_box,
                                                             uint32_t* __restrict__ pairs, uint64_t max_pairs,
                                                             StepCounters* __restrict__ ctr) {
    constexpr int kCellsPerLane = (14 + kLanesPerBody - 1) / kLanesPerBody;
    __shared__ uint32_t stage[(kPairThreads / 64) * kStagePerWave * 2];
    PairStage st;
    st.lds = stage + (threadIdx.x >> 6) * kStagePerWave * 2;
    st.count = 0;
    const uint32_t n_active = bucket_start[table_size];
    const uint32_t g = blockIdx.x * blockDim.x + threadIdx.x;
    const uint32_t s = g / kLanesPerBody;
    const uint32_t sub = g % kLanesPerBody;
    const bool live = s < n_active;
    const float inv_cell = grid_inv_cell(ctr);
    uint32_t i = 0;
    aabb_t bi;
    bi.lo = v3_make(0, 0, 0); bi.hi = v3_make(0, 0, 0);
    int cx = 0, cy = 0, cz = 0;
    if (live) {
        i = sorted_ids[s];
        bi.lo = ld3(sorted_box, 2 * s);
        bi.hi = ld3(sorted_box, 2 * s + 1);
        cx = grid_cell_coord(0.5f * (bi.lo.x + bi.hi.x), inv_cell);
        cy = grid_cell_coord(0.5f * (bi.lo.y + bi.hi.y), inv_cell);
        cz = grid_cell_coord(0.5f * (bi.lo.z + bi.hi.z), inv_cell);
    }
    uint32_t t0[kCellsPerLane], t1[kCellsPerLane];
#pragma unroll
    for (int k = 0; k < kCellsPerLane; ++k) {
        const int c = (int)sub + kLanesPerBody * k;
        int dx, dy, dz;
        if (c == 0) { dx = 0; dy = 0; dz = 0; }
        else if (c == 1) { dx = 1; dy = 0; dz = 0; }
        else if (c < 5) { dx = c - 3; dy = 1; dz = 0; }
        else { dx = (c - 5) % 3 - 1; dy = ((c - 5) / 3) % 3 - 1; dz = 1; }
        t0[k] = 0; t1[k] = 0;
        if (live && c < 14) {
            const uint32_t bk = grid_bucket(cx + dx, cy + dy, cz + dz, axis_mask);
            t0[k] = bucket_start[bk];
            t1[k] = bucket_start[bk + 1];
        }
    }
#pragma unroll
    for (int k = 0; k < kCellsPerLane; ++k) {
        const bool own_cell = (sub == 0 && k == 0);
        uint32_t t = t0[k];
        const uint32_t t_end = t1[k];
        while (__any(t < t_end)) {
            bool hit = false;
            uint32_t j = 0;
            if (t < t_end) {
                j = sorted_ids[t];
                aabb_t bj;
                bj.lo = ld3(sorted_box, 2 * t);
                bj.hi = ld3(sorted_box, 2 * t + 1);
                hit = aabb_overlap(bi, bj) && (!own_cell || i < j);
                ++t;
            }
            stage_push(st, hit, i < j ? i : j, i < j ? j : i, pairs, max_pairs, ctr);
        }
    }
    stage_flush(st, pairs, max_pairs, ctr);
}

constexpr int kBrickLanesPerBody = 4;

template <int kBrickStagePerWave>
__device__ __forceinline__ void workgroup_flush(PairStage& st, uint32_t* s_cnt, uint32_t* s_base, uint32_t* __restrict__ pairs,
                                                uint64_t max_pairs, StepCounters* __restrict__ ctr, bool force) {
    const uint32_t wave = threadIdx.x >> 6, lane = threadIdx.x & 63u;
    if (lane == 0) s_cnt[wave] = st.count;
    __syncthreads();
    const uint32_t total = s_cnt[0] + s_cnt[1] + s_cnt[2] + s_cnt[3];
    const bool go = total != 0u && (force || total >= (uint32_t)(2 * kBrickStagePerWave));
    if (go && threadIdx.x == 0) {
        const uint32_t base = atomicAdd(&ctr->n_pairs, total);
        if ((uint64_t)base + total > max_pairs) flag_overflow(ctr, kOvfPairs);
        *s_base = base;
    }
    __syncthreads();
    if (go) {
        uint32_t off = *s_base;
        for (uint32_t k = 0; k < wave; ++k) off += s_cnt[k];
        for (uint32_t k = lane; k < st.count; k += 64) {
            const uint64_t dst = (uint64_t)off + k;
            if (dst < max_pairs) reinterpret_cast<uint2*>(pairs)[dst] = reinterpret_cast<const uint2*>(st.lds)[k];
        }
        st.count = 0;
    }
    __syncthreads();
}

template <int kBrickStagePerWave>
__global__ __launch_bounds__(kPairThreads, 7) void k_find_pairs_brick(const uint32_t* __restrict__ bucket_start, uint32_t n_bricks,
                                                                   GridShape g, const uint32_t* __restrict__ sorted_ids,
                                                                   const float* __restrict__ sorted_box,
                                                                   uint32_t* __restrict__ pairs, uint64_t max_pairs,
                                                                   StepCounters* __restrict__ ctr, uint32_t cap) {
    __shared__ uint32_t stage[(kPairThreads / 64) * kBrickStagePerWave * 2];
    __shared__ uint32_t s_gstart[kRegCells];
    __shared__ uint32_t s_off[kRegCells + 1];
    extern __shared__ float s_rec[];
    __shared__ uint32_t s_wsum[4], s_cnt[4], s_base;
    PairStage st;
    st.lds = stage + (threadIdx.x >> 6) * kBrickStagePerWave * 2;
    st.count = 0;
    const float inv_cell = grid_inv_cell(ctr);
    const uint32_t sub = threadIdx.x % kBrickLanesPerBody;
    uint32_t first = blockIdx.x, last = n_bricks, step = gridDim.x;
    if (gridDim.x >= 8u && n_bricks >= 8u) {
        const uint32_t label = blockIdx.x & 7u, per = n_bricks >> 3;
        step = (gridDim.x - label + 7u) >> 3;
        first = label * per + (blockIdx.x >> 3);
        last = (label + 1u) * per;
    }
    uint32_t nx_begin = 0, nx_end = 0, nx_c0 = 0, nx_cnt = 0;
    auto ask = [&](uint32_t brick) {
        nx_begin = bucket_start[brick * 64u];
        nx_end = bucket_start[brick * 64u + 64u];
        nx_c0 = 0; nx_cnt = 0;
        if (threadIdx.x < (uint32_t)kRegCells) {
            const uint32_t bx = brick & ((1u << g.sx) - 1u), by = (brick >> g.sx) & ((1u << g.sy) - 1u), bz = brick >> (g.sx + g.sy);
            const uint32_t r = threadIdx.x;
            const uint32_t rx = r % kRegX, ry = (r / kRegX) % kRegY, rz = r / (kRegX * kRegY);
            const uint32_t bk = grid_bucket_masked(((bx << 2) + rx - 1u) & g.mx, ((by << 2) + ry - 1u) & g.my, ((bz << 2) + rz) & g.mz, g);
            nx_c0 = bucket_start[bk];
            nx_cnt = bucket_start[bk + 1] - nx_c0;
        }
    };
    if (first < last) ask(first);
    uint32_t seen_max = 0;
    for (uint32_t brick = first; brick < last; brick += step) {
        const uint32_t own_begin = nx_begin, own_end = nx_end, my_c0 = nx_c0, my_cnt = nx_cnt;
        if (brick + step < last) ask(brick + step);
        if (own_begin == own_end) continue;
        constexpr uint32_t kBodiesPerTrip = kPairThreads / kBrickLanesPerBody;
        const uint32_t n_own = own_end - own_begin;
        uint32_t i0 = 0;
        aabb_t b0;
        b0.lo = v3_make(0, 0, 0); b0.hi = v3_make(0, 0, 0);
        if (threadIdx.x / kBrickLanesPerBody < n_own) {
            const uint32_t sidx = own_begin + threadIdx.x / kBrickLanesPerBody;
            i0 = sorted_ids[sidx];
            b0.lo = ld3(sorted_box, 2 * sidx);
            b0.hi = ld3(sorted_box, 2 * sidx + 1);
        }
        {
            const uint32_t cnt = my_cnt;
            if (threadIdx.x < (uint32_t)kRegCells) s_gstart[threadIdx.x] = my_c0;
            const uint32_t inc = wave_inclusive_scan(cnt);
            if ((threadIdx.x & 63u) == 63u) s_wsum[threadIdx.x >> 6] = inc;
            __syncthreads();
            uint32_t base = 0;
            for (uint32_t k = 0; k < (threadIdx.x >> 6); ++k) base += s_wsum[k];
            if (threadIdx.x < (uint32_t)kRegCells) s_off[threadIdx.x] = base + inc - cnt;
            if (threadIdx.x == (uint32_t)kRegCells - 1u) s_off[kRegCells] = base + inc;
            __syncthreads();
        }
        const uint32_t total = s_off[kRegCells];
        const bool staged = total <= cap;
        seen_max = total > seen_max ? total : seen_max;
        if (staged) {
            for (uint32_t q = threadIdx.x; q < total; q += kPairThreads) {
                uint32_t lo = 0, hi = kRegCells;
                while (hi - lo > 1u) {
                    const uint32_t mid = (lo + hi) >> 1;
                    if (s_off[mid] <= q) lo = mid; else hi = mid;
                }
                const uint32_t t = s_gstart[lo] + (q - s_off[lo]);
                const v3 blo = ld3(sorted_box, 2 * t), bhi = ld3(sorted_box, 2 * t + 1);
                float* rec = s_rec + 7u * q;
                rec[0] = blo.x; rec[1] = blo.y; rec[2] = blo.z; rec[3] = bhi.x; rec[4] = bhi.y; rec[5] = bhi.z;
                rec[6] = __uint_as_float(sorted_ids[t]);
            }
            __syncthreads();
        }
        for (uint32_t base = 0; base < n_own; base += kBodiesPerTrip) {
            const uint32_t jo = base + threadIdx.x / kBrickLanesPerBody;
            const bool live = jo < n_own;
            uint32_t i = i0;
            aabb_t bi = b0;
            if (base != 0u && live) {
                const uint32_t sidx = own_begin + jo;
                i = sorted_ids[sidx];
                bi.lo = ld3(sorted_box, 2 * sidx);
                bi.hi = ld3(sorted_box, 2 * sidx + 1);
            }
            const uint32_t lx = (uint32_t)grid_cell_coord(0.5f * (bi.lo.x + bi.hi.x), inv_cell) & 3u;
            const uint32_t ly = (uint32_t)grid_cell_coord(0.5f * (bi.lo.y + bi.hi.y), inv_cell) & 3u;
            const uint32_t lz = (uint32_t)grid_cell_coord(0.5f * (bi.lo.z + bi.hi.z), inv_cell) & 3u;
#pragma unroll
            for (int k = 0; k < (14 + kBrickLanesPerBody - 1) / kBrickLanesPerBody; ++k) {
                const int c = (int)sub + kBrickLanesPerBody * k;
                int dx, dy, dz;
                if (c == 0) { dx = 0; dy = 0; dz = 0; }
                else if (c == 1) { dx = 1; dy = 0; dz = 0; }
                else if (c < 5) { dx = c - 3; dy = 1; dz = 0; }
                else { dx = (c - 5) % 3 - 1; dy = ((c - 5) / 3) % 3 - 1; dz = 1; }
                uint32_t t = 0, t_end = 0;
                if (live && c < 14) {
                    const uint32_t rid = ((lz + (uint32_t)dz) * kRegY + (ly + (uint32_t)(dy + 1))) * kRegX + (lx + (uint32_t)(dx + 1));
                    t = staged ? s_off[rid] : s_gstart[rid];
                    t_end = t + (s_off[rid + 1] - s_off[rid]);
                }
                const bool own_cell = c == 0;
                while (__any(t < t_end)) {
                    bool hit = false;
                    uint32_t j = 0;
                    if (t < t_end) {
                        aabb_t bj;
                        if (staged) {
                            const float* rec = s_rec + 7u * t;
                            bj.lo = v3_make(rec[0], rec[1], rec[2]);
                            bj.hi = v3_make(rec[3], rec[4], rec[5]);
                            j = __float_as_uint(rec[6]);
                        } else {
                            j = sorted_ids[t];
                            bj.lo = ld3(sorted_box, 2 * t);
                            bj.hi = ld3(sorted_box, 2 * t + 1);
                        }
                        hit = aabb_overlap(bi, bj) && (!own_cell || i < j);
                        ++t;
                    }
                    stage_push<kBrickStagePerWave>(st, hit, i < j ? i : j, i < j ? j : i, pairs, max_pairs, ctr);
                }
            }
        }
        workgroup_flush<kBrickStagePerWave>(st, s_cnt, &s_base, pairs, max_pairs, ctr, false);
    }
    workgroup_flush<kBrickStagePerWave>(st, s_cnt, &s_base, pairs, max_pairs, ctr, true);
    if (threadIdx.x == 0 && seen_max > ctr->max_region) atomicMax(&ctr->max_region, seen_max);
}

constexpr uint32_t kSlotsPerBucket = 8;

__global__ __launch_bounds__(256) void k_cell_insert(uint32_t n, const float* __restrict__ aabb,
                                                     const uint32_t* __restrict__ shape, StepCounters* __restrict__ ctr,
                                                     GridShape axis_mask, uint32_t* __restrict__ rank,
                                                     uint32_t* __restrict__ bucket_count, uint32_t* __restrict__ slot_ids,
                                                     float* __restrict__ slot_box, uint32_t* __restrict__ ovf) {
    const uint32_t i = blockIdx.x * blockDim.x + threadIdx.x;
    if (i >= n || shape[i] == PHYS_SPEC_SHAPE_NONE) return;
    const float inv_cell = grid_inv_cell(ctr);
    const v3 lo = ld3(aabb, 2 * i), hi = ld3(aabb, 2 * i + 1);
    const int cx = grid_cell_coord(0.5f * (lo.x + hi.x), inv_cell);
    const int cy = grid_cell_coord(0.5f * (lo.y + hi.y), inv_cell);
    const int cz = grid_cell_coord(0.5f * (lo.z + hi.z), inv_cell);
    const uint32_t bk = grid_bucket(cx, cy, cz, axis_mask);
    const uint32_t r = atomicAdd(&bucket_count[bk], 1u);
    rank[i] = r;
    if (r < kSlotsPerBucket) {
        slot_ids[kSlotsPerBucket * bk + r] = i;
        st3(slot_box, 2 * (kSlotsPerBucket * bk + r), lo);
        st3(slot_box, 2 * (kSlotsPerBucket * bk + r) + 1, hi);
    } else {
        ovf[atomicAdd(&ctr->n_grid_ovf, 1u)] = i;
    }
}

template <int kLanesPerBody>
__global__ __launch_bounds__(kPairThreads) void k_find_pairs_slots(uint32_t n, const float* __restrict__ aabb,
                                                                   const uint32_t* __restrict__ shape,
                                                                   const uint32_t* __restrict__ rank,
                                                                   const uint32_t* __restrict__ bucket_count,
                                                                   const uint32_t* __restrict__ slot_ids,
                                                                   const float* __restrict__ slot_box,
                                                                   const uint32_t* __restrict__ ovf, GridShape axis_mask,
                                                                   uint32_t* __restrict__ pairs, uint64_t max_pairs,
                                                                   StepCounters* __restrict__ ctr) {
    constexpr int kCellsPerLane = (14 + kLanesPerBody - 1) / kLanesPerBody;
    __shared__ uint32_t stage[(kPairThreads / 64) * kStagePerWave * 2];
    PairStage st;
    st.lds = stage + (threadIdx.x >> 6) * kStagePerWave * 2;
    st.count = 0;
    const uint32_t g = blockIdx.x * blockDim.x + threadIdx.x;
    const uint32_t i = g / kLanesPerBody;
    const uint32_t sub = g % kLanesPerBody;
    const bool live = i < n && shape[i] != PHYS_SPEC_SHAPE_NONE;
    const float inv_cell = grid_inv_cell(ctr);
    aabb_t bi;
    bi.lo = v3_make(0, 0, 0); bi.hi = v3_make(0, 0, 0);
    int cx = 0, cy = 0, cz = 0;
    bool in_overflow = false;
    if (live) {
        bi.lo = ld3(aabb, 2 * i);
        bi.hi = ld3(aabb, 2 * i + 1);
        cx = grid_cell_coord(0.5f * (bi.lo.x + bi.hi.x), inv_cell);
        cy = grid_cell_coord(0.5f * (bi.lo.y + bi.hi.y), inv_cell);
        cz = grid_cell_coord(0.5f * (bi.lo.z + bi.hi.z), inv_cell);
        in_overflow = rank[i] >= kSlotsPerBucket;
    }
    uint32_t cnt[kCellsPerLane], first[kCellsPerLane];
#pragma unroll
    for (int k = 0; k < kCellsPerLane; ++k) {
        const int c = (int)sub + kLanesPerBody * k;
        int dx, dy, dz;
        if (c == 0) { dx = 0; dy = 0; dz = 0; }
        else if (c == 1) { dx = 1; dy = 0; dz = 0; }
        else if (c < 5) { dx = c - 3; dy = 1; dz = 0; }
        else { dx = (c - 5) % 3 - 1; dy = ((c - 5) / 3) % 3 - 1; dz = 1; }
        cnt[k] = 0; first[k] = 0;
        if (live && !in_overflow && c < 14) {
            const uint32_t bk = grid_bucket(cx + dx, cy + dy, cz + dz, axis_mask);
            const uint32_t have = bucket_count[bk];
            first[k] = kSlotsPerBucket * bk;
            cnt[k] = have < kSlotsPerBucket ? have : kSlotsPerBucket;
        }
    }
#pragma unroll
    for (int k = 0; k < kCellsPerLane; ++k) {
        const bool own_cell = (sub == 0 && k == 0);
        for (uint32_t r = 0; __any(r < cnt[k]); ++r) {
            bool hit = false;
            uint32_t j = 0;
            if (r < cnt[k]) {
                const uint32_t slot = first[k] + r;
                j = slot_ids[slot];
                aabb_t bj;
                bj.lo = ld3(slot_box, 2 * slot);
                bj.hi = ld3(slot_box, 2 * slot + 1);
                hit = aabb_overlap(bi, bj) && (!own_cell || i < j);
            }
            stage_push(st, hit, i < j ? i : j, i < j ? j : i, pairs, max_pairs, ctr);
        }
    }
    const uint32_t n_ovf = ctr->n_grid_ovf;
    for (uint32_t o = 0; o < n_ovf; ++o) {
        const uint32_t j = ovf[o];
        bool hit = false;
        if (live && sub == 0 && j != i && (!in_overflow || i < j)) {
            aabb_t bj;
            bj.lo = ld3(aabb, 2 * j);
            bj.hi = ld3(aabb, 2 * j + 1);
            hit = aabb_overlap(bi, bj);
        }
        stage_push(st, hit, i < j ? i : j, i < j ? j : i, pairs, max_pairs, ctr);
    }
    stage_flush(st, pairs, max_pairs, ctr);
}

int32_t collision_alloc(phys_world* w) {
    const uint64_t n = w->n;
    const CollisionSizes sz = collision_sizes(w->cfg, n, debug_switches());
    w->max_pairs = sz.max_pairs;
    w->max_manifolds = sz.max_manifolds;
    if (!sz.ok) {
        set_error("max_pairs / max_manifolds exceed u32 indexing");
        return PHYS_ERR_INVALID_ARG;
    }
    const uint32_t T = w->grid_table_size;
    {
        const size_t b_bytes = sz.bucket_bytes, c_bytes = sz.color_bytes;
        w->step_zero.free();
        PHYS_HIP_TRY(w->step_zero.resize(b_bytes + c_bytes + sz.counter_bytes));
        w->bucket_count.point_at(reinterpret_cast<uint32_t*>(w->step_zero.p), T);
        w->color_state.point_at(reinterpret_cast<unsigned long long*>(w->step_zero.p + b_bytes), c_bytes / 8);
        w->counters.point_at(reinterpret_cast<StepCounters*>(w->step_zero.p + b_bytes + c_bytes), 1);
        w->step_zero_reset_bytes = b_bytes + c_bytes + kCountersStepResetBytes;
        w->step_zero_full_bytes = b_bytes + c_bytes + kCountersExtentResetBytes;
        PHYS_HIP_TRY(hipMemsetAsync(w->step_zero.p, 0, b_bytes + c_bytes + sz.counter_bytes, w->stream));
    }
    PHYS_HIP_TRY(w->bucket_of.resize(n));
    PHYS_HIP_TRY(w->bucket_cursor.resize(n));
    PHYS_HIP_TRY(w->bucket_start.resize((size_t)T + 1));
    PHYS_HIP_TRY(w->scan_block_sums.resize(2 * std::max<size_t>(scan_scratch_words(T) + 1, 64)));
    PHYS_HIP_TRY(w->sorted_ids.resize(n));
    PHYS_HIP_TRY(w->slot_ids.resize((size_t)kSlotsPerBucket * T));
    PHYS_HIP_TRY(w->slot_box.resize((size_t)6 * kSlotsPerBucket * T));
    PHYS_HIP_TRY(w->grid_ovf.resize(n));
    w->sorted_grid_valid = false;
    PHYS_HIP_TRY(w->sorted_box.resize(6 * n));
    PHYS_HIP_TRY(w->pairs.resize(2 * w->max_pairs));
    if (!(w->cfg.flags & PHYS_FLAG_BROADPHASE_ONLY)) {
        const uint64_t M = w->max_manifolds;
        PHYS_HIP_TRY(w->man_a.resize(M)); PHYS_HIP_TRY(w->man_b.resize(M));
        PHYS_HIP_TRY(w->man_color.resize(M));
        PHYS_HIP_TRY(w->man_geo.resize(32 * M));
        w->warm = sz.warm;
        if (w->warm) {
            PHYS_HIP_TRY(w->man_geo_prev.resize(32 * M));
            PHYS_HIP_TRY(w->man_imp.resize(12 * M));
            PHYS_HIP_TRY(w->man_imp_prev.resize(12 * M));
            PHYS_HIP_TRY(w->man_prev.resize(4));
        }
        PHYS_HIP_TRY(w->man_prio.resize(M));
        PHYS_HIP_TRY(w->row_src.resize(M));
        PHYS_HIP_TRY(w->unc_list.resize(2 * M));
        PHYS_HIP_TRY(w->ctab.resize(2 * sz.ctab_slots));
        w->ctab_mask = (uint32_t)(sz.ctab_slots - 1);
        w->ctab_valid = false;
        w->color_epoch = 0;
        PHYS_HIP_TRY(w->color_block_hist.resize((size_t)kMaxColors * 512));
        w->row_all.free();
        PHYS_HIP_TRY(w->row_all.resize(64 * M));
        w->row_hdr.point_at(reinterpret_cast<uint32_t*>(w->row_all.p), 4 * M);
        w->row_n.point_at(w->row_all.p + 4 * M, 4 * M);
        w->row_tb.point_at(w->row_all.p + 8 * M, 8 * M);
        w->row_pt.point_at(w->row_all.p + 16 * M, 32 * M);
        w->row_acc.point_at(w->row_all.p + 48 * M, 16 * M);
        w->flow_vel.free();
        if (sz.flow_buffers) {
            PHYS_HIP_TRY(w->flow_vel.resize(8 * n));
            PHYS_HIP_TRY(hipMemsetAsync(w->flow_vel.p, 0, 8 * n * sizeof(float), w->stream));
            PHYS_HIP_TRY(hipMemsetAsync(w->row_acc.p, 0, 16 * M * sizeof(float), w->stream));
            w->flow_epoch = debug_switches().flow_epoch;
        }
    }
    return PHYS_OK;
}

void zero_step_state(phys_world* w, bool including_extent) {
    PHYS_PROF(w, PHYS_STAGE_MISC);
    (void)hipMemsetAsync(w->step_zero.p, 0, including_extent ? w->step_zero_full_bytes : w->step_zero_reset_bytes, w->stream);
}

void build_sorted_grid(phys_world* w) {
    const uint32_t n = (uint32_t)w->n;
    const uint32_t T = w->grid_table_size;
    const GridShape axis_mask = w->grid_shape;
    hipStream_t s = w->stream;
    const dim3 gb((n + 255) / 256), tb(256);
    w->sorted_grid_valid = true;
    { PHYS_PROF(w, PHYS_STAGE_GRID); hipLaunchKernelGGL(k_cell_assign, gb, tb, 0, s, n, w->aabb.p, w->shape.p, w->counters.p, axis_mask, w->bucket_of.p,
                       w->bucket_cursor.p, w->bucket_count.p); }
    launch_exclusive_scan(w, w->bucket_count.p, T, w->bucket_start.p, false, w->scan_block_sums.p,
                          w->scan_block_sums.p + w->scan_block_sums.n / 2, w->counters.p, PHYS_STAGE_GRID);
    { PHYS_PROF(w, PHYS_STAGE_GRID); hipLaunchKernelGGL(k_scatter, gb, tb, 0, s, n, w->aabb.p, w->bucket_of.p, w->bucket_cursor.p, w->bucket_start.p,
                       w->sorted_ids.p, w->sorted_box.p); }
}

void launch_broadphase(phys_world* w, const PairPlan& plan) {
    const uint32_t n = (uint32_t)w->n;
    if (n == 0) return;
    w->grid_valid = true;
    const uint32_t T = w->grid_table_size;
    const GridShape axis_mask = w->grid_shape;
    hipStream_t s = w->stream;
    const dim3 wgs(plan.wgs), tb(kPairThreads);
    if (plan.kernel == PairKernel::Slots) {
        w->sorted_grid_valid = false;
        { PHYS_PROF(w, PHYS_STAGE_GRID); hipLaunchKernelGGL(k_cell_insert, dim3((n + 255) / 256), dim3(256), 0, s, n, w->aabb.p, w->shape.p, w->counters.p,
                           axis_mask, w->bucket_cursor.p, w->bucket_count.p, w->slot_ids.p, w->slot_box.p, w->grid_ovf.p); }
        PHYS_PROF(w, PHYS_STAGE_PAIRS);
        hipLaunchKernelGGL((k_find_pairs_slots<4>), wgs, tb, 0, s,
                           n, w->aabb.p, w->shape.p, w->bucket_cursor.p, w->bucket_count.p, w->slot_ids.p, w->slot_box.p, w->grid_ovf.p, axis_mask,
                           w->pairs.p, w->max_pairs, w->counters.p);
        return;
    }
    build_sorted_grid(w);
    if (plan.kernel == PairKernel::Brick128 || plan.kernel == PairKernel::Brick256) {
        static bool attr_set[64] = {};
        (void)allow_dynamic_lds(attr_set, w->device, {reinterpret_cast<const void*>(&k_find_pairs_brick<128>),
                                                      reinterpret_cast<const void*>(&k_find_pairs_brick<256>)}, 150 * 1024);
        const uint32_t n_bricks = T >> 6;
        PHYS_PROF(w, PHYS_STAGE_PAIRS);
        if (plan.kernel == PairKernel::Brick128)
            hipLaunchKernelGGL(k_find_pairs_brick<128>, wgs, tb, plan.lds, s, w->bucket_start.p, n_bricks, axis_mask,
                               w->sorted_ids.p, w->sorted_box.p, w->pairs.p, w->max_pairs, w->counters.p, plan.cap);
        else
            hipLaunchKernelGGL(k_find_pairs_brick<256>, wgs, tb, plan.lds, s, w->bucket_start.p, n_bricks, axis_mask,
                               w->sorted_ids.p, w->sorted_box.p, w->pairs.p, w->max_pairs, w->counters.p, plan.cap);
        return;
    }
    PHYS_PROF(w, PHYS_STAGE_PAIRS);
    if (plan.kernel == PairKernel::Lanes4)
        hipLaunchKernelGGL((k_find_pairs<4>), wgs, tb, 0, s,
                           w->bucket_start.p, T, axis_mask, w->sorted_ids.p, w->sorted_box.p, w->pairs.p, w->max_pairs, w->counters.p);
    else
        hipLaunchKernelGGL((k_find_pairs<1>), wgs, tb, 0, s,
                           w->bucket_start.p, T, axis_mask, w->sorted_ids.p, w->sorted_box.p, w->pairs.p, w->max_pairs, w->counters.p);
}

int32_t sorted_pairs_to_host(phys_world* w, uint32_t* pairs_out, uint64_t cap, uint64_t* n_pairs) {
    PHYS_TRY(fetch_counters(w));
    if (w->h_counters->overflow & kOvfPairs) {
        set_error("pair capacity exceeded: raise phys_config.max_pairs");
        return PHYS_ERR_CAPACITY;
    }
    const uint64_t m = w->h_counters->n_pairs;
    *n_pairs = m;
    if (!pairs_out || m == 0) return PHYS_OK;
    std::vector<uint32_t> raw(2 * m);
    PHYS_HIP_TRY(hipMemcpy(raw.data(), w->pairs.p, 8 * m, hipMemcpyDeviceToHost));
    sort_pairs(raw.data(), m, pairs_out, cap);
    return PHYS_OK;
}

}
```

physics_amd/csrc/narrowphase.hip:

```cpp
#include <cstdlib>
#include <utility>

#include "kernels.hpp"

namespace phys {

__device__ __forceinline__ geom_t load_geom(uint32_t i, const float* __restrict__ geo) {
    const float4* g = reinterpret_cast<const float4*>(geo) + 4 * (size_t)i;
    const float4 g0 = g[0], qq = g[1], g2 = g[2];
    quat q; q.i = qq.x; q.j = qq.y; q.k = qq.z; q.w = qq.w;
    return geom_make(v3_make(g0.x, g0.y, g0.z), q, v3_make(g2.x, g2.y, g2.z), __float_as_uint(g0.w));
}

template <int kNpThreads, int kNpItems, bool kStatics, bool kCapsules, bool kFilters, typename... Filt>
__global__ __launch_bounds__(kNpThreads) void k_narrowphase(
    uint32_t n_ground , uint32_t n_owned ,
    const uint32_t* __restrict__ pairs,
    uint64_t max_pairs, const float* __restrict__ geo ,
    float margin, float ground, uint64_t max_manifolds, uint32_t* __restrict__ man_a, uint32_t* __restrict__ man_b,
    uint32_t* __restrict__ man_color, float* __restrict__ man_geo ,
    uint64_t* __restrict__ man_prio, unsigned long long* __restrict__ used,
    unsigned long long* __restrict__ top0, ulonglong2* __restrict__ cache ,
    uint32_t cache_mask , uint32_t early_probe , uint32_t stamp ,
    uint32_t* __restrict__ unc_list ,
    const uint32_t* __restrict__ man_prev ,
    float* __restrict__ man_imp ,
    StepCounters* __restrict__ ctr,
    uint64_t max_static_pairs ,
    const uint32_t* __restrict__ static_pairs, const float* __restrict__ static_geo ,
    Filt... filt ) {
    static_assert(sizeof...(Filt) == (kFilters ? 1u : 0u), "one NpFilters argument exactly in the filtered instance");
    NpFilters flt{};
    if constexpr (kFilters) flt = filter_arg(filt...);
    __shared__ uint32_t wtot[2][4][kNpThreads / 64];
    __shared__ uint32_t block_base, unc_base;
    constexpr int kWsStride = sizeof(clip_ws_t) / 4 + 1;
    __shared__ float ws_lds[kNpThreads * kWsStride];
    clip_ws_t* ws = reinterpret_cast<clip_ws_t*>(ws_lds + threadIdx.x * kWsStride);
    const uint32_t np_raw = ctr->n_pairs;
    const uint32_t n_pairs = (uint64_t)np_raw < max_pairs ? np_raw : (uint32_t)max_pairs;
    uint32_t n_static = 0;
    if (kStatics) {
        const uint32_t ns_raw = ctr->n_static_pairs;
        n_static = (uint64_t)ns_raw < max_static_pairs ? ns_raw : (uint32_t)max_static_pairs;
    }
    const uint32_t n_body_items = n_ground + n_pairs;
    const uint32_t total = n_body_items + n_static;
    const int lane = threadIdx.x & 63, wave = threadIdx.x >> 6;
    uint32_t trip = 0;
    uint32_t acc_pts = 0, acc_ground = 0, acc_unc = 0;
    uint32_t acc_static = 0;
    struct Item {
        manifold_t m;
        uint32_t a, b, col, prev_m, kept_h;
        unsigned long long prio, seen, bit;
        bool has, uncolored;
    };
    for (uint64_t base = (uint64_t)blockIdx.x * (kNpThreads * kNpItems); base < total;
         base += (uint64_t)gridDim.x * (kNpThreads * kNpItems), ++trip) {
        uint32_t* wcount = wtot[trip & 1u][0];
        uint32_t* wpts = wtot[trip & 1u][1];
        uint32_t* wground = wtot[trip & 1u][2];
        uint32_t* wunc = wtot[trip & 1u][3];
        Item item[kNpItems];
#pragma unroll
        for (int j = 0; j < kNpItems; ++j) {
            Item& it = item[j];
            manifold_t& m = it.m;
            const uint64_t idx = base + (uint64_t)j * kNpThreads + threadIdx.x;
            m.count = 0;
            uint32_t a = 0, b = PHYS_GROUND_ID;
            ulonglong2 early = make_ulonglong2(0ull, 0ull);
            uint32_t early_h = 0;
            bool have_early = false;
            if (idx < n_ground) {
                a = (uint32_t)idx;
                if (kFilters && !filter_pass(flt.body[a], flt.ground)) {
                } else {
                const float4 g2 = reinterpret_cast<const float4*>(geo)[4 * (size_t)a + 2];
                const float lo_y = g2.w;
                if (lo_y <= (ground + margin) + 1.0e-3f * (1.0f + det_absf(lo_y))) {
                    const geom_t ga = load_geom(a, geo);
                    if (ga.type != PHYS_SPEC_SHAPE_NONE) {
                        if (kCapsules) collide_ground(&ga, ground, margin, &m, ws);
                        else collide_ground_sphere_box(&ga, ground, margin, &m, ws);
                    }
                }
                }
            } else if (idx < total) {
                const bool body_pair = !kStatics || idx < n_body_items;
                const uint2 pr = body_pair ? reinterpret_cast<const uint2*>(pairs)[idx - n_ground]
                                           : reinterpret_cast<const uint2*>(static_pairs)[idx - n_body_items];
                a = pr.x; b = body_pair ? pr.y : (PHYS_STATIC_ID_BIT | pr.y);
                if (a < n_owned && (!kFilters || filter_pass(flt.body[a], body_pair ? flt.body[pr.y] : flt.st[pr.y]))) {
                    if (cache_mask && early_probe) {
                        early_h = (uint32_t)(color_priority(a, b) >> 20) & cache_mask;
                        early = cache[early_h];
                        have_early = true;
                    }
                    const geom_t ga = load_geom(a, geo);
                    const geom_t gb = body_pair ? load_geom(b, geo) : load_geom(pr.y, static_geo);
                    if (kCapsules) collide_pair(&ga, &gb, margin, &m, ws);
                    else collide_pair_sphere_box(&ga, &gb, margin, &m, ws);
                }
            }
            const bool has = m.count > 0;
            unsigned long long prio = 0ull, seen_a = 0ull, seen_b = 0ull, bit = 0ull;
            uint32_t col = kUncolored, prev_m = 0xFFFFFFFFu, kept_h = 0;
            bool uncolored = false;
            if (has) {
                prio = color_priority(a, b);
                if (cache_mask) {
                    const unsigned long long key = ((unsigned long long)a << 32) | b;
                    uint32_t h = (uint32_t)(prio >> 20) & cache_mask;
                    bool ended = false;
                    for (uint32_t walked = 0; walked < kColorTableMaxWalk; ++walked) {
                        const ulonglong2 e = (have_early && h == early_h) ? early : cache[h];
                        have_early = false;
                        if (e.x == key) {
                            if ((uint32_t)(e.y >> 32) + 1u == stamp) {
                                col = (uint32_t)e.y & 63u;
                                prev_m = ((uint32_t)e.y >> 6);
                                kept_h = h;
                            }
                            ended = true;
                            break;
                        }
                        if (e.x == ~0ull) { ended = true; break; }
                        h = (h + 1) & cache_mask;
                    }
                    if (!ended) flag_overflow(ctr, kOvfColorTable);
                }
                if (col != kUncolored) {
                    bit = 1ull << col;
                    seen_a = atomicOr(&used[a], bit);
                    if (!PHYS_IS_STATIC_PARTNER(b)) seen_b = atomicOr(&used[b], bit);
                } else {
                    uncolored = true;
                    atomicMax(&top0[a], prio);
                    if (!PHYS_IS_STATIC_PARTNER(b)) atomicMax(&top0[b], prio);
                }
            }
            it.a = a; it.b = b; it.col = col; it.prev_m = prev_m; it.kept_h = kept_h;
            it.prio = prio; it.seen = seen_a | seen_b; it.bit = bit; it.has = has; it.uncolored = uncolored;
        }
        unsigned long long mask[kNpItems], umask[kNpItems];
        uint32_t n_has = 0, n_gnd = 0, n_unc = 0, pts = 0;
#pragma unroll
        for (int j = 0; j < kNpItems; ++j) {
            mask[j] = __ballot(item[j].has);
            umask[j] = __ballot(item[j].uncolored);
            n_has += (uint32_t)__popcll(mask[j]);
            n_unc += (uint32_t)__popcll(umask[j]);
            n_gnd += (uint32_t)__popcll(__ballot(item[j].has && item[j].b == PHYS_GROUND_ID));
            if (kStatics) acc_static += (uint32_t)__popcll(__ballot(item[j].has && item[j].b != PHYS_GROUND_ID && PHYS_IS_STATIC_PARTNER(item[j].b)));
            pts += item[j].has ? (uint32_t)item[j].m.count : 0u;
        }
#pragma unroll
        for (int off = 32; off > 0; off >>= 1) pts += (uint32_t)__shfl_xor((int)pts, off, 64);
        if (lane == 0) {
            wcount[wave] = n_has;
            wpts[wave] = pts;
            wground[wave] = n_gnd;
            wunc[wave] = n_unc;
        }
        __syncthreads();
        if (threadIdx.x == 0) {
            uint32_t t = 0, tp = 0, tg = 0, tu = 0;
            for (int k = 0; k < kNpThreads / 64; ++k) { t += wcount[k]; tp += wpts[k]; tg += wground[k]; tu += wunc[k]; }
            uint32_t bb = 0, ub = 0;
            if (t) {
                const unsigned long long got = atomicAdd(reinterpret_cast<unsigned long long*>(&ctr->n_manifolds),
                                                         ((unsigned long long)tu << 32) | t);
                bb = (uint32_t)got;
                ub = (uint32_t)(got >> 32);
                const uint64_t room = (uint64_t)bb < max_manifolds ? max_manifolds - bb : 0;
                const uint32_t stored = (uint64_t)t <= room ? t : (uint32_t)room;
                if (stored != t) flag_overflow(ctr, kOvfManifolds);
                acc_pts += tp; acc_ground += tg; acc_unc += tu;
            }
            block_base = bb;
            unc_base = ub;
        }
        __syncthreads();
        uint32_t woff = 0, uoff = 0;
        for (int k = 0; k < wave; ++k) { woff += wcount[k]; uoff += wunc[k]; }
        const unsigned long long below = (1ull << lane) - 1ull;
#pragma unroll
        for (int j = 0; j < kNpItems; ++j) {
            const Item& it = item[j];
            if (it.has) {
                const manifold_t& m = it.m;
                const uint32_t a = it.a, b = it.b, col = it.col;
                const uint64_t slot = (uint64_t)block_base + woff + (uint32_t)__popcll(mask[j] & below);
                if (slot < max_manifolds) {
                    man_a[slot] = a;
                    man_b[slot] = b;
                    man_prio[slot] = it.prio;
                    man_color[slot] = col;
                    if (col != kUncolored) cache[it.kept_h].y = ((unsigned long long)stamp << 32) | ((unsigned long long)((uint32_t)slot & 0x3FFFFFFu) << 6) | col;
                    if (man_prev) {
                        float4* imp = reinterpret_cast<float4*>(man_imp) + 3 * slot;
                        imp[0] = make_float4(0.0f, 0.0f, 0.0f, 0.0f); imp[1] = imp[0]; imp[2] = imp[0];
                    }
                    float4* o = reinterpret_cast<float4*>(man_geo) + 8 * slot;
                    o[0] = make_float4(__uint_as_float(a), __uint_as_float(b), __uint_as_float((uint32_t)m.count),
                                       __uint_as_float(col != kUncolored ? col + 1u : 0u));
                    o[1] = make_float4(m.normal.x, m.normal.y, m.normal.z, __uint_as_float(it.prev_m));
#pragma unroll
                    for (int k = 0; k < 4; ++k) o[2 + k] = make_float4(m.pt[k].x, m.pt[k].y, m.pt[k].z, m.depth[k]);
                }
                if (it.uncolored) {
                    const uint32_t at = unc_base + uoff + (uint32_t)__popcll(umask[j] & below);
                    unc_list[at < max_manifolds ? at : (uint32_t)max_manifolds - 1u] =
                        slot < max_manifolds ? (uint32_t)slot : (uint32_t)max_manifolds - 1u;
                } else if ((it.seen & it.bit) != 0ull) {
                    flag_overflow(ctr, kOvfColors);
                }
            }
            woff += (uint32_t)__popcll(mask[j]);
            uoff += (uint32_t)__popcll(umask[j]);
        }
    }
    if (threadIdx.x == 0) {
        if (acc_pts) atomicAdd(&ctr->n_contacts, acc_pts);
        if (acc_ground) atomicAdd(&ctr->n_ground_manifolds, acc_ground);
        if (acc_unc) { atomicAdd(&ctr->n_uncolored, acc_unc); atomicAdd(&ctr->n_new_manifolds, acc_unc); }
    }
    if (kStatics && (threadIdx.x & 63) == 0 && acc_static) atomicAdd(&ctr->n_static_manifolds, acc_static);
}

void launch_narrowphase(phys_world* w, const NarrowPlan& plan) {
    const uint32_t n = (uint32_t)w->n;
    if (n == 0) return;
    const uint32_t n_owned = n;
    const uint32_t n_ground = (w->cfg.flags & PHYS_FLAG_GROUND_PLANE) ? n : 0u;
    uint64_t st_cap = 0;
    const uint32_t* st_pairs = nullptr;
    const float* st_geo = nullptr;
    static_narrow_args(w, &st_cap, &st_pairs, &st_geo);
    const uint32_t cache_mask = w->ctab_valid ? w->ctab_mask : 0u;
    const uint32_t stamp = (uint32_t)w->color_epoch + 1u;
    if (w->warm) {
        std::swap(w->man_geo.p, w->man_geo_prev.p);
        std::swap(w->man_imp.p, w->man_imp_prev.p);
    }
    NpFilters flt{};
    flt.body = reinterpret_cast<const uint2*>(w->filt.p);
    flt.st = st_pairs ? reinterpret_cast<const uint2*>(w->st_filt.p) : nullptr;
    flt.ground = make_uint2(w->ground_filt, 0u);
    PHYS_PROF(w, PHYS_STAGE_NARROW);
    dispatch_bool(plan.threads == 128, [&](auto few_t) { dispatch_bool(plan.statics, [&](auto st_t) {
    dispatch_bool(plan.capsules, [&](auto cap_t) { dispatch_bool(plan.filters, [&](auto flt_t) {
        constexpr int T = decltype(few_t)::value ? 128 : 512;
        constexpr bool S = decltype(st_t)::value, CAP = decltype(cap_t)::value, FLT = decltype(flt_t)::value;
        auto launch = [&](auto... filters) {
            hipLaunchKernelGGL((k_narrowphase<T, 1, S, CAP, FLT>), dim3(plan.blocks), dim3(T), 0, w->stream, n_ground, n_owned, w->pairs.p,
                               w->max_pairs, w->geo.p, w->cfg.contact_margin, w->cfg.ground_height, w->max_manifolds, w->man_a.p, w->man_b.p,
                               w->man_color.p, w->man_geo.p, w->man_prio.p, w->color_state.p, w->color_state.p + n,
                               reinterpret_cast<ulonglong2*>(w->ctab.p), cache_mask, plan.early_probe, stamp, w->unc_list.p,
                               w->warm ? w->man_prev.p : nullptr, w->man_imp.p, w->counters.p, st_cap, st_pairs, st_geo, filters...);
        };
        if constexpr (FLT) launch(flt); else launch();
    }); }); }); });
}

}
```

physics_amd/csrc/plan.hpp:

```cpp
#pragma once
#include <algorithm>
#include <cstddef>
#include <cstdint>
#include <optional>

#include "../../include/physics_hip.h"

namespace phys {

constexpr int kMaxColors = 64;
constexpr int kColorCachePeriod = 64;

struct StepHint {
    bool valid = false;
    uint32_t n_manifolds = 0, n_colors = 0, n_pairs = 0, max_region = 0, n_used_buckets = 0, n_contacts = 0;
    uint32_t n_active = 0;
    uint32_t color_rounds = 0;
    uint32_t full_rounds = 0;
    uint32_t recent_rounds[8] = {};
    uint32_t recent_pos = 0;
    uint32_t n_new = 0xFFFFFFFFu;
    uint32_t recent_new[8] = {};
    uint32_t color_count[kMaxColors] = {};
};

struct DebugSwitches {
    bool no_cluster = false, cluster_dynamic = false, no_flow_preference = false, flow_stall = false;
    std::optional<uint64_t> cluster_min, flow_max;
    std::optional<int> clusters_per_cu;
    uint64_t cluster_cap = 0, flow_quad_max = 0, ctab_slots = 0;
    uint32_t flow_epoch = 0;
    int np_threads = 0, pair_lanes = 0, brick_stage = 0;
    bool raycast_stats = false;
    std::optional<bool> flow_pipeline, np_early_probe;
    std::optional<bool> color_kernel_lane;
    std::optional<bool> pair_kernel_brick;
};

struct PlanInputs {
    uint32_t flags = 0, solver_iterations = 0;
    uint64_t n = 0, n_owned = 0, max_manifolds = 0;
    uint32_t grid_table_size = 0;
    int cus = 0;
    bool exclusive = false;
    bool warm = false;
    bool flow_vel = false;
    uint32_t cluster_count = 0;
    bool cluster_dynamic = false;
    bool ctab_valid = false;
    uint64_t color_epoch = 0;
    bool statics = false, capsules = false, filters = false, materials = false;
    uint64_t np_items = 0;
};

constexpr int kPairThreads = 256;
constexpr int kRegX = 6, kRegY = 6, kRegZ = 5, kRegCells = kRegX * kRegY * kRegZ;
constexpr int kColorThreads = 1024;
constexpr int kSmallTrips = 40;
constexpr int kSortBlocksMax = 512;
constexpr int kSortChunk = 4096;
constexpr int kKeysItems = 4;
constexpr int kQuadRowsPerGroup = 64;
constexpr int kEventThreads = 256;

constexpr uint32_t kSlotGridMaxBodies = 32768;
constexpr uint64_t kClusterMinBodies = 32768;
constexpr uint64_t kClusterMinManifolds = 170000;
constexpr long long kFlowTimeoutTicks = 300000000ll;
constexpr uint64_t kFlowMaxManifolds = 400000;
constexpr uint64_t kFlowQuadMaxManifolds = 200000;
constexpr uint32_t kTailMax = 512;
constexpr uint32_t kQuadColorMaxRows = 32768;
constexpr uint32_t kBrickCapMax = 5000;
constexpr size_t kBrickPerCuMax = 7;

inline bool flow_quad_beats_cluster(uint32_t manifolds, uint32_t contacts, uint32_t colors) {
    if (!colors || !contacts) return false;
    const double flow = 8.4e-8 * manifolds + 1.86e-8 * contacts + 0.0009 * colors;
    const double cluster = 1.1 * std::max(0.0041 * colors, 6.9e-8 * manifolds);
    return flow < cluster;
}

enum class PairKernel { Slots, Brick128, Brick256, Lanes4, Lanes1 };
struct PairPlan {
    PairKernel kernel = PairKernel::Slots;
    uint32_t cap = 0;
    size_t lds = 0;
    uint32_t wgs = 0;
};
inline PairPlan plan_pairs(const PlanInputs& in, const StepHint& h, const DebugSwitches& dbg) {
    PairPlan p;
    const uint32_t n = (uint32_t)in.n;
    const uint32_t per_four_lanes = (uint32_t)(((uint64_t)n * 4 + kPairThreads - 1) / kPairThreads);
    if (n <= kSlotGridMaxBodies) {
        p.kernel = PairKernel::Slots;
        p.wgs = per_four_lanes;
        return p;
    }
    const bool crowded = h.valid && h.n_used_buckets && (uint64_t)in.n * 10ull > (uint64_t)h.n_used_buckets * 21ull;
    const bool brick = dbg.pair_kernel_brick.value_or(!crowded);
    if (brick && !dbg.pair_lanes) {
        const uint32_t n_bricks = in.grid_table_size >> 6;
        uint32_t cap = h.valid && h.max_region ? h.max_region + h.max_region / 4 : 1024u;
        cap = std::min(std::max((cap + 63u) & ~63u, 256u), kBrickCapMax);
        const size_t dyn = (size_t)cap * 28;
        const bool small_stage = dbg.brick_stage ? dbg.brick_stage == 128 : (h.valid && (uint64_t)h.n_pairs < 3ull * in.n);
        const size_t fixed = (kPairThreads / 64) * (small_stage ? 128 : 256) * 8 + kRegCells * 8 + 64;
        const uint32_t per_cu = (uint32_t)std::min<size_t>(kBrickPerCuMax, (160 * 1024) / (((dyn + fixed) + 1023) / 1024 * 1024));
        uint32_t wgs = 256u * std::max(per_cu, 1u);
        while (wgs > n_bricks) wgs >>= 1;
        p.kernel = small_stage ? PairKernel::Brick128 : PairKernel::Brick256;
        p.cap = cap;
        p.lds = dyn;
        p.wgs = wgs;
        return p;
    }
    if (dbg.pair_lanes ? dbg.pair_lanes == 4 : n <= 65536u) {
        p.kernel = PairKernel::Lanes4;
        p.wgs = per_four_lanes;
    } else {
        p.kernel = PairKernel::Lanes1;
        p.wgs = (n + kPairThreads - 1) / kPairThreads;
    }
    return p;
}

struct NarrowPlan {
    int threads = 512;
    uint32_t early_probe = 0;
    bool statics = false, capsules = false, filters = false;
    uint32_t blocks = 1;
};
inline NarrowPlan plan_narrowphase(const PlanInputs& in, const StepHint& h, const DebugSwitches& dbg) {
    NarrowPlan p;
    p.early_probe = dbg.np_early_probe.value_or(!h.valid || 2ull * h.n_manifolds >= (uint64_t)h.n_pairs);
    const bool few = h.valid ? h.n_manifolds <= 32768u : (uint32_t)in.n <= 200000u;
    p.threads = (dbg.np_threads ? dbg.np_threads : (few ? 128 : 512)) == 128 ? 128 : 512;
    p.statics = in.statics; p.capsules = in.capsules; p.filters = in.filters;
    uint64_t blocks = (in.np_items + p.threads - 1) / p.threads;
    if (blocks > 256 * 16) blocks = 256 * 16;
    p.blocks = (uint32_t)blocks;
    return p;
}

enum class ColorPath {
    Small,
    Known,
    Probe
};
struct ColorPlan {
    ColorPath path = ColorPath::Probe;
    uint32_t rounds = 0;
    uint32_t round_blocks = 1;
    uint32_t sort_blocks = 1;
    uint32_t cluster_sort_blocks = 1, cluster_key_blocks = 1;
    bool full = false;
    bool rebuild = false;
    uint32_t stamp = 0;
    bool wants_cluster = false;
};
inline ColorPlan plan_coloring(const PlanInputs& in, const StepHint& h, const DebugSwitches& dbg) {
    ColorPlan p;
    uint64_t blocks64 = (in.max_manifolds + kColorThreads - 1) / kColorThreads;
    if (blocks64 > 512) blocks64 = 512;
    if (h.valid) {
        const uint64_t want = ((uint64_t)h.n_manifolds * 5 / 4 + kColorThreads) / kColorThreads;
        if (want < blocks64) blocks64 = want ? want : 1;
    }
    p.round_blocks = (uint32_t)blocks64;
    p.full = !in.ctab_valid;
    p.rebuild = p.full || (in.color_epoch % kColorCachePeriod) == 0;
    p.stamp = (uint32_t)in.color_epoch + 1u;
    const bool known = h.valid && (!p.full || h.full_rounds > 0);
    const bool small = h.valid && h.n_manifolds <= (uint32_t)(kSmallTrips * kColorThreads);
    p.path = small ? ColorPath::Small : (known ? ColorPath::Known : ColorPath::Probe);
    if (p.path == ColorPath::Known) p.rounds = p.full ? h.full_rounds : h.color_rounds;
    uint32_t nb = kSortBlocksMax;
    if (h.valid) {
        const uint64_t want = ((uint64_t)h.n_manifolds * 5 / 4) / kSortChunk + 1;
        nb = 1;
        while (nb < want && nb < (uint32_t)kSortBlocksMax) nb <<= 1;
    }
    p.sort_blocks = nb;
    p.cluster_sort_blocks = p.round_blocks * (kColorThreads / 256);
    const uint64_t key_trips = h.valid ? ((uint64_t)h.n_manifolds * 5 / 4) / (256u * kKeysItems) + 1 : p.cluster_sort_blocks;
    p.cluster_key_blocks = (uint32_t)std::min<uint64_t>(p.cluster_sort_blocks, std::max<uint64_t>(1, key_trips));
    const bool cluster_forced = (in.flags & PHYS_FLAG_SOLVER_CLUSTER) != 0u;
    const uint64_t cluster_min = cluster_forced ? 0 : dbg.cluster_min.value_or(kClusterMinManifolds);
    const bool dense = cluster_forced || dbg.cluster_min.has_value() || in.cluster_dynamic || 2ull * h.n_manifolds >= 3ull * in.n_owned;
    p.wants_cluster = (in.cluster_count > 0 || in.cluster_dynamic) && h.valid && !small && dense && h.n_manifolds >= cluster_min &&
                      !(in.flags & PHYS_FLAG_SOLVER_PER_COLOR) && in.solver_iterations > 0 && in.solver_iterations < 1000 &&
                      h.n_colors > 0;
    if (p.wants_cluster && !cluster_forced && !dbg.cluster_min.has_value() && !dbg.no_flow_preference && in.exclusive &&
        h.n_manifolds <= kFlowMaxManifolds && flow_quad_beats_cluster(h.n_manifolds, h.n_contacts, h.n_colors))
        p.wants_cluster = false;
    return p;
}

enum class SolverPath { Cluster, FlowQuad, FlowLane, PerColor };
struct SolverPlan {
    SolverPath path = SolverPath::PerColor;
    bool materials = false;
    uint32_t rows_blocks = 1;
    bool stall = false;
    long long timeout_ticks = kFlowTimeoutTicks;
    bool guarded = true;
    uint32_t items = 0, pipeline = 0;
    uint32_t big = 0;
    bool color_quad[kMaxColors] = {};
    uint32_t color_blocks[kMaxColors] = {};
    bool flow() const { return path != SolverPath::PerColor; }
};
inline SolverPlan plan_solver(const PlanInputs& in, const StepHint& h, const DebugSwitches& dbg, bool cluster) {
    SolverPlan p;
    p.materials = in.materials;
    const uint64_t cap = in.max_manifolds;
    const uint64_t m_hint = h.valid ? h.n_manifolds : cap;
    auto grid_for_count = [&](uint64_t count, uint64_t rows_per_group, uint64_t most) {
        uint64_t b = (count * 5 / 4 + rows_per_group - 1) / rows_per_group + 1;
        const uint64_t hi = (cap + rows_per_group - 1) / rows_per_group;
        if (b > hi) b = hi;
        if (b > most) b = most;
        return (uint32_t)(b ? b : 1);
    };
    p.rows_blocks = grid_for_count(m_hint, 256, 4096);
    p.stall = dbg.flow_stall;
    p.timeout_ticks = p.stall ? 2000000ll : kFlowTimeoutTicks;
    p.guarded = !in.exclusive;
    const uint64_t flow_max = dbg.flow_max.value_or(kFlowMaxManifolds);
    const bool flow = cluster || (in.flow_vel && h.valid && m_hint <= flow_max && in.solver_iterations > 0 && in.solver_iterations < 1000);
    if (cluster) {
        p.path = SolverPath::Cluster;
        return p;
    }
    if (flow) {
        const bool quad = m_hint <= (dbg.flow_quad_max ? dbg.flow_quad_max : (in.exclusive ? kFlowMaxManifolds : kFlowQuadMaxManifolds));
        const uint32_t sweeps = in.solver_iterations + (in.warm ? 1u : 0u);
        const uint32_t threads = 256u;
        const uint32_t rows_per_item = quad ? threads / 4 : threads;
        uint64_t items = (uint64_t)sweeps * ((m_hint * 5 / 4 + rows_per_item - 1) / rows_per_item) + 1;
        const uint64_t most = quad ? (in.exclusive && m_hint > 32768u ? (uint64_t)(3 * (in.cus - in.cus / 8)) : 224) : 256;
        if (items > most) items = most;
        const uint64_t per_color = m_hint / (h.valid && h.n_colors ? h.n_colors : 1u);
        p.path = quad ? SolverPath::FlowQuad : SolverPath::FlowLane;
        p.items = (uint32_t)items;
        p.pipeline = (uint32_t)dbg.flow_pipeline.value_or(4 * per_color >= threads * items);
        return p;
    }
    p.path = SolverPath::PerColor;
    if (h.valid) {
        p.big = h.n_colors;
        while (p.big > 0 && h.color_count[p.big - 1] <= kTailMax) --p.big;
        if (h.n_colors - p.big < 2) p.big = h.n_colors;
    }
    for (uint32_t col = 0; col < p.big; ++col) {
        p.color_quad[col] = !dbg.color_kernel_lane.value_or(h.color_count[col] > kQuadColorMaxRows);
        p.color_blocks[col] = p.color_quad[col] ? grid_for_count(h.color_count[col], kQuadRowsPerGroup, 16384)
                                                : grid_for_count(h.color_count[col], 256, 4096);
    }
    return p;
}

inline uint32_t plan_event_blocks(const PlanInputs& in, const StepHint& h) {
    const uint64_t m_guess = h.valid ? (uint64_t)h.n_manifolds * 5 / 4 + kEventThreads : in.max_manifolds;
    const uint64_t blocks = (std::min<uint64_t>(m_guess, in.max_manifolds) + kEventThreads - 1) / kEventThreads;
    return (uint32_t)std::max<uint64_t>(1, std::min<uint64_t>(blocks, 2048));
}

}
```

physics_amd/world.py:

```python
import ctypes as C

import numpy as np

from . import _abi
from ._abi import STAGE_NAMES, PhysContactEvent, PhysDeviceView, PhysProfile, PhysStats, PhysTriggerEvent, f32p, i16p, u16p, u32p

CONTACT_EVENT_DTYPE = np.dtype([("body_a", "<u4"), ("body_b", "<u4"), ("kind", "<u4"), ("step", "<u4"), ("point", "<f4", (3,)),
                                ("impulse", "<f4"), ("normal", "<f4", (3,)), ("reserved", "<u4")])
TRIGGER_EVENT_DTYPE = np.dtype([("trigger", "<u4"), ("body", "<u4"), ("kind", "<u4"), ("step", "<u4")])


class PhysError(RuntimeError):
    def __init__(self, code, msg):
        super().__init__(f"physics_hip error {code}: {msg}")
        self.code = code


def _f(a):
    return None if a is None else np.ascontiguousarray(a, dtype=np.float32)


def _p(a, t=f32p):
    return None if a is None else a.ctypes.data_as(t)

# ... 102 lines not shown
        for a, w in ((rot, 4), (st, 1), (he, 3)):
            if a is not None and a.size != n * w:
                raise ValueError("array size does not match the static collider count")
        self._ck(self.lib.phys_set_static_bodies(self.h, n, _p(pos), _p(rot), _p(st, u32p), _p(he)))
        self.n_static = n

    def set_body_filters(self, category=None, mask=None, group=None):
        n = self.n
        c = _filter_field(category, n, "category", 0, 0xFFFF, np.uint16)
        m = _filter_field(mask, n, "mask", 0, 0xFFFF, np.uint16)
        g = _filter_field(group, n, "group", -0x8000, 0x7FFF, np.int16)
        self._ck(self.lib.phys_set_body_filters(self.h, n, _p(c, u16p), _p(m, u16p), _p(g, i16p)))

    def get_body_filters(self):
        c = np.empty(self.n, np.uint16)
        m = np.empty(self.n, np.uint16)
        g = np.empty(self.n, np.int16)
        self._ck(self.lib.phys_get_body_filters(self.h, _p(c, u16p), _p(m, u16p), _p(g, i16p)))
        return c, m, g

    def set_static_filters(self, category=None, mask=None, group=None):
        n = self.n_static
        c = _filter_field(category, n, "category", 0, 0xFFFF, np.uint16)
        m = _filter_field(mask, n, "mask", 0, 0xFFFF, np.uint16)
        g = _filter_field(group, n, "group", -0x8000, 0x7FFF, np.int16)
        self._ck(self.lib.phys_set_static_filters(self.h, n, _p(c, u16p), _p(m, u16p), _p(g, i16p)))

    def set_ground_filter(self, category, mask):
        for name, v in (("category", category), ("mask", mask)):
            if not isinstance(v, (int, np.integer)) or isinstance(v, bool) or not 0 <= int(v) <= 0xFFFF:
                raise ValueError(f"{name}: needs an integer in [0, 65535]")
        self._ck(self.lib.phys_set_ground_filter(self.h, int(category), int(mask)))

    def set_body_materials(self, friction=None, restitution=None):
        n = self.n
        f = _material_field(friction, n, "friction", np.inf)
        e = _material_field(restitution, n, "restitution", 1.0)
        self._ck(self.lib.phys_set_body_materials(self.h, n, _p(f), _p(e)))

    def get_body_materials(self):
        f = np.empty(self.n, np.float32)
        e = np.empty(self.n, np.float32)
        self._ck(self.lib.phys_get_body_materials(self.h, _p(f), _p(e)))
        return f, e

    def set_static_materials(self, friction=None, restitution=None):
        n = self.n_static
        f = _material_field(friction, n, "friction", np.inf)
        e = _material_field(restitution, n, "restitution", 1.0)
        self._ck(self.lib.phys_set_static_materials(self.h, n, _p(f), _p(e)))

    def set_ground_material(self, friction, restitution=0.0):
        f = _material_field(friction, 1, "friction", np.inf)
        e = _material_field(restitution, 1, "restitution", 1.0)
        if f is None or e is None:
            raise ValueError("the ground's friction and restitution are numbers")
        self._ck(self.lib.phys_set_ground_material(self.h, float(f[0]), float(e[0])))

    def set_restitution_threshold(self, v):
        t = _material_field(v, 1, "threshold", np.inf)
        if t is None:
            raise ValueError("the threshold is a number")
        self._ck(self.lib.phys_set_restitution_threshold(self.h, float(t[0])))

    def get_static_stats(self):
        out = [C.c_uint64() for _ in range(3)]
        self._ck(self.lib.phys_get_static_stats(self.h, *[C.byref(x) for x in out]))
        return tuple(x.value for x in out)

    def add_constraint_fix_point(self, body, target):
        t = _f(target)
        self._ck(self.lib.phys_add_constraint_fix_point(self.h, body, _p(t)))

    def add_constraint_fix_orientation(self, body, target_rpy):
        t = _f(target_rpy)
        self._ck(self.lib.phys_add_constraint_fix_orientation(self.h, body, _p(t)))

    def clear_constraints(self):
        self._ck(self.lib.phys_clear_constraints(self.h))

    def apply_force_centre_of_gravity(self, body, force):
        f = _f(force)
        self._ck(self.lib.phys_apply_force_centre_of_gravity(self.h, body, _p(f)))

    def apply_force_at_position(self, body, force, point):
        f, p = _f(force), _f(point)
        self._ck(self.lib.phys_apply_force_at_position(self.h, body, _p(f), _p(p)))

    def apply_force_at_offset(self, body, force, offset):
        f, o = _f(force), _f(offset)
        self._ck(self.lib.phys_apply_force_at_offset(self.h, body, _p(f), _p(o)))

    def set_forces(self, force=None, torque=None):
        f, t = _f(force), _f(torque)
        self._ck(self.lib.phys_set_forces(self.h, _p(f), _p(t)))

    def apply_gravity(self):
        self._ck(self.lib.phys_apply_gravity(self.h))

    def step(self, dt_nanos):
        self._ck(self.lib.phys_step(self.h, dt_nanos))

    def update(self, dt_nanos):
        self._ck(self.lib.phys_update(self.h, dt_nanos))

    def update_n(self, dt_nanos, n):
        self._ck(self.lib.phys_update_n(self.h, dt_nanos, n))

    def sync(self):
        self._ck(self.lib.phys_sync(self.h))

    def get_transforms(self):
        pos = np.empty((self.n, 3), np.float32)
        rot = np.empty((self.n, 4), np.float32)
        self._ck(self.lib.phys_get_transforms(self.h, _p(pos), _p(rot)))
        return pos, rot

    def get_velocities(self):
        lin = np.empty((self.n, 3), np.float32)
        ang = np.empty((self.n, 3), np.float32)
        self._ck(self.lib.phys_get_velocities(self.h, _p(lin), _p(ang)))
        return lin, ang

    def get_forces(self):
        f = np.empty((self.n, 3), np.float32)
        t = np.empty((self.n, 3), np.float32)
        self._ck(self.lib.phys_get_forces(self.h, _p(f), _p(t)))
        return f, t

    def get_instance_matrices(self):
        m = np.empty((self.n, 16), np.float32)
        self._ck(self.lib.phys_get_instance_matrices(self.h, _p(m)))
        return m

    def get_lambda(self):
        n = C.c_uint64()
        self._ck(self.lib.phys_get_lambda(self.h, None, 0, C.byref(n)))
        out = np.empty(n.value, np.float32)
        if n.value:
            self._ck(self.lib.phys_get_lambda(self.h, _p(out), n.value, C.byref(n)))
        return out

    def get_stats(self):
        s = PhysStats()
        self._ck(self.lib.phys_get_stats(self.h, C.byref(s)))
        return s

    def broadphase(self):
        n = C.c_uint64()
        self._ck(self.lib.phys_broadphase(self.h, None, 0, C.byref(n)))
        out = np.empty((n.value, 2), np.uint32)
        if n.value:
            self._ck(self.lib.phys_broadphase(self.h, _p(out, u32p), n.value, C.byref(n)))
        return out

    def get_aabbs(self):
        out = np.empty((self.n, 6), np.float32)
        self._ck(self.lib.phys_get_aabbs(self.h, _p(out)))
        return out

    def raycast(self, origins, dirs, max_t=None, ignore=None, mask=None):
        o = _f(origins).reshape(-1, 3)
        d = _f(dirs).reshape(-1, 3)
        n = o.shape[0]
        if d.shape[0] != n:
            raise ValueError("origins and dirs differ in length")
        mt = None if max_t is None else _f(max_t).reshape(-1)
        ig = None if ignore is None else np.ascontiguousarray(ignore, dtype=np.uint32).reshape(-1)
        for a in (mt, ig):
            if a is not None and a.size != n:
                raise ValueError("max_t / ignore do not match the ray count")
        qm = _query_mask(mask, n)
        body = np.empty(n, np.uint32)
        t = np.empty(n, np.float32)
        normal = np.empty((n, 3), np.float32)
        if n and qm is None:
            self._ck(self.lib.phys_raycast(self.h, n, _p(o), _p(d), _p(mt), _p(ig, u32p), _p(body, u32p), _p(t), _p(normal)))
        elif n:
            self._ck(self.lib.phys_raycast_filtered(self.h, n, _p(o), _p(d), _p(mt), _p(ig, u32p), _p(qm, u16p), _p(body, u32p),
                                                    _p(t), _p(normal)))
        return body, t, normal

    def raycast_device(self, origins, dirs, body_out, t_out, normal_out=None, max_t=None, ignore=None, mask=None):
        n = int(origins.shape[0])
        args = _device_args(n, (("origins", origins, 3), ("dirs", dirs, 3), ("max_t", max_t, 1), ("ignore", ignore, 1)))
        out = _device_args(n, (("body_out", body_out, 1), ("t_out", t_out, 1), ("normal_out", normal_out, 3)))
        if mask is None:
            self._ck(self.lib.phys_raycast_device(self.h, n, *args, *out))
        else:
            self._ck(self.lib.phys_raycast_device_filtered(self.h, n, *args, _device_mask(mask, n), *out))

    def spherecast(self, origins, dirs, radius, max_t=None, ignore=None, mask=None):
        o = _f(origins).reshape(-1, 3)
        d = _f(dirs).reshape(-1, 3)
        n = o.shape[0]
        if d.shape[0] != n:
            raise ValueError("origins and dirs differ in length")
        rad = np.ascontiguousarray(np.broadcast_to(np.asarray(radius, np.float32), (n,)))
        mt = None if max_t is None else _f(max_t).reshape(-1)
        ig = None if ignore is None else np.ascontiguousarray(ignore, dtype=np.uint32).reshape(-1)
        for a in (mt, ig):
            if a is not None and a.size != n:
                raise ValueError("max_t / ignore do not match the ball count")
        qm = _query_mask(mask, n)
        body = np.empty(n, np.uint32)
        t = np.empty(n, np.float32)
        normal = np.empty((n, 3), np.float32)
        if n and qm is None:
            self._ck(self.lib.phys_spherecast(self.h, n, _p(o), _p(d), _p(rad), _p(mt), _p(ig, u32p), _p(body, u32p), _p(t),
                                              _p(normal)))
        elif n:
            self._ck(self.lib.phys_spherecast_filtered(self.h, n, _p(o), _p(d), _p(rad), _p(mt), _p(ig, u32p), _p(qm, u16p),
                                                       _p(body, u32p), _p(t), _p(normal)))
        return body, t, normal

    def spherecast_device(self, origins, dirs, radius, body_out, t_out, normal_out=None, max_t=None, ignore=None, mask=None):
        n = int(origins.shape[0])
        args = _device_args(n, (("origins", origins, 3), ("dirs", dirs, 3), ("radius", radius, 1), ("max_t", max_t, 1),
                                ("ignore", ignore, 1)))
        out = _device_args(n, (("body_out", body_out, 1), ("t_out", t_out, 1), ("normal_out", normal_out, 3)))
        if mask is None:
            self._ck(self.lib.phys_spherecast_device(self.h, n, *args, *out))
        else:
            self._ck(self.lib.phys_spherecast_device_filtered(self.h, n, *args, _device_mask(mask, n), *out))

    def overlap(self, shape_type, pos, rot=None, half_extent=None, ignore=None, cap=None, mask=None):
        p = _f(pos).reshape(-1, 3)
        n = p.shape[0]
        if half_extent is None:
            raise ValueError("half_extent is required")
        st = np.ascontiguousarray(np.broadcast_to(np.asarray(shape_type, np.uint32), (n,)))
        he = np.ascontiguousarray(np.broadcast_to(np.asarray(half_extent, np.float32).reshape(-1, 3), (n, 3)))
        r = None if rot is None else _f(rot).reshape(-1, 4)
        ig = None if ignore is None else np.ascontiguousarray(ignore, dtype=np.uint32).reshape(-1)
        for a, k in ((r, 4), (ig, 1)):
            if a is not None and a.size != n * k:
                raise ValueError("rot / ignore do not match the query count")
        qm = _query_mask(mask, n)
        offsets = np.zeros(n + 1, np.uint64)
        cap = 8 * n + 64 if cap is None else int(cap)
        for attempt in range(2):
            ids = np.empty(max(cap, 1), np.uint32)
            if qm is None:
                rc = self.lib.phys_overlap(self.h, n, _p(st, u32p), _p(p), _p(r), _p(he), _p(ig, u32p), cap, _p(offsets, _abi.u64p),
                                           _p(ids, u32p))
            else:
                rc = self.lib.phys_overlap_filtered(self.h, n, _p(st, u32p), _p(p), _p(r), _p(he), _p(ig, u32p), _p(qm, u16p), cap,
                                                    _p(offsets, _abi.u64p), _p(ids, u32p))
            if rc == _abi.PHYS_ERR_CAPACITY and attempt == 0:
                cap = int(offsets[n])
                continue
            self._ck(rc)
            break
        return offsets, ids[:int(offsets[n])]

    def get_manifolds(self):
        n = C.c_uint64()
        self._ck(self.lib.phys_get_manifolds(self.h, None, None, None, None, 0, C.byref(n)))
        m = n.value
        ids = np.empty((m, 2), np.uint32)
        counts = np.empty(m, np.uint32)
        normals = np.empty((m, 3), np.float32)
        points = np.empty((m, 4, 4), np.float32)
        if m:
            self._ck(self.lib.phys_get_manifolds(self.h, _p(ids, u32p), _p(counts, u32p), _p(normals), _p(points), m,
                                                 C.byref(n)))
        return ids, counts, normals, points

    def enable_contact_events(self, capacity):
        self._ck(self.lib.phys_contact_events_enable(self.h, int(capacity)))

    def get_contact_events(self):
        n, dropped = C.c_uint64(), C.c_uint64()
        self._ck(self.lib.phys_get_contact_events(self.h, None, 0, C.byref(n), C.byref(dropped)))
        while True:
            out = np.zeros(n.value, CONTACT_EVENT_DTYPE)
            rc = self.lib.phys_get_contact_events(self.h, out.ctypes.data_as(C.POINTER(PhysContactEvent)), out.shape[0],
                                                  C.byref(n), C.byref(dropped))
            if rc != _abi.PHYS_ERR_CAPACITY:
                self._ck(rc)
                return out[:n.value], dropped.value

    def get_contact_impulses(self):
        n = C.c_uint64()
        self._ck(self.lib.phys_get_contact_impulses(self.h, None, 0, C.byref(n)))
        out = np.zeros((n.value, 4, 3), np.float32)
        if n.value:
            self._ck(self.lib.phys_get_contact_impulses(self.h, _p(out), n.value, C.byref(n)))
        return out

    def set_triggers(self, shape_type, pos, rot=None, half_extent=None, mask=None):
        p = _f(pos).reshape(-1, 3)
        n = p.shape[0]
        if n and half_extent is None:
            raise ValueError("half_extent is required")
        st = np.asarray(shape_type if n else np.zeros(0, np.uint32))
        if st.ndim > 1 or (st.ndim == 1 and st.shape[0] != n):
            raise ValueError(f"shape_type: needs {n} values, got shape {st.shape}")
        st = np.ascontiguousarray(np.broadcast_to(st.astype(np.uint32), (n,)))
        he = np.asarray(half_extent if n else np.zeros((0, 3)), np.float32).reshape(-1, 3)
        if he.shape[0] not in (1, n):
            raise ValueError(f"half_extent: needs 3 or {n} x 3 values, got shape {np.shape(half_extent)}")
        he = np.ascontiguousarray(np.broadcast_to(he, (n, 3)))
        r = None if rot is None else _f(rot).reshape(-1, 4)
        if r is not None and r.shape[0] != n:
            raise ValueError("rot does not match the trigger count")
# ... 150 lines not shown
```

rust/physics_hip_sys/src/lib.rs:

```rust
#![allow(non_camel_case_types)]
use std::os::raw::{c_char, c_void};

pub const PHYS_ABI_VERSION: u32 = 2;
pub const PHYS_OK: i32 = 0;
pub const PHYS_ERR_SINGULAR_INERTIA: i32 = -4;
pub const PHYS_ERR_CAPACITY: i32 = -5;
pub const PHYS_ERR_NO_BODIES: i32 = -8;
pub const PHYS_SHAPE_NONE: u32 = 0;
pub const PHYS_SHAPE_SPHERE: u32 = 1;
pub const PHYS_SHAPE_BOX: u32 = 2;
pub const PHYS_SHAPE_CAPSULE: u32 = 3;
pub const PHYS_STATIC_ID_BIT: u32 = 0x8000_0000;
pub const PHYS_FILTER_DEFAULT_CATEGORY: u16 = 0x0001;
pub const PHYS_FILTER_DEFAULT_MASK: u16 = 0xFFFF;
pub const PHYS_FLAG_COLLISIONS: u32 = 0x1;
pub const PHYS_FLAG_GROUND_PLANE: u32 = 0x2;
pub const PHYS_FLAG_EXACT_ROTATION: u32 = 0x4;
pub const PHYS_FLAG_BROADPHASE_ONLY: u32 = 0x8;
pub const PHYS_FLAG_SOLVER_PER_COLOR: u32 = 0x10;
pub const PHYS_FLAG_SHARED_GPU: u32 = 0x20;
pub const PHYS_FLAG_SOLVER_CLUSTER: u32 = 0x40;
pub const PHYS_FLAG_EXCLUSIVE_GPU: u32 = 0x80;
pub const PHYS_FLAG_NO_WARM_START: u32 = 0x100;
pub const PHYS_RAY_MISS: u32 = 0xFFFF_FFFE;
pub const PHYS_RAY_GROUND: u32 = 0xFFFF_FFFF;
pub const PHYS_CONTACT_BEGIN: u32 = 1;
pub const PHYS_CONTACT_END: u32 = 2;
pub const PHYS_MAX_TRIGGERS: u32 = 1024;
pub const PHYS_TRIGGER_ENTER: u32 = 1;
pub const PHYS_TRIGGER_EXIT: u32 = 2;

#[repr(C)]
#[derive(Clone, Copy)]
pub struct phys_config {
    pub abi_version: u32,
    pub device: i32,
    pub flags: u32,
    pub gravity_force: [f32; 3],
    pub gravity_offset: [f32; 3],
    pub cg_max_iterations: u32,
    pub cg_max_error: f32,
    pub cg_min_error: f32,
    pub solver_iterations: u32,
    pub baumgarte: f32,
    pub slop: f32,
    pub friction: f32,
    pub contact_margin: f32,
    pub ground_height: f32,
    pub max_bias: f32,
    pub max_pairs: u64,
    pub max_manifolds: u64,
    pub max_ghosts: u64,
}

#[repr(C)]
#[derive(Clone, Copy, Default)]
pub struct phys_stats {
    pub n_bodies: u64,
    pub n_pairs: u64,
    pub n_manifolds: u64,
    pub n_contacts: u64,
    pub n_colors: u32,
    pub color_rounds: u32,
    pub cg_iterations: u32,
    pub cg_converged: i32,
    pub steps: u64,
    pub overflow: u32,
    pub n_ground_manifolds: u32,
    pub max_extent: f32,
    pub n_halo_records: u32,
    pub n_cross_pairs: u64,
    pub n_ghosts: u32,
    pub n_new_manifolds: u32,
}

#[repr(C)]
#[derive(Clone, Copy, Default)]
pub struct phys_contact_event {
    pub body_a: u32,
    pub body_b: u32,
    pub kind: u32,
    pub step: u32,
    pub point: [f32; 3],
    pub impulse: f32,
    pub normal: [f32; 3],
    pub reserved: u32,
}

#[repr(C)]
#[derive(Clone, Copy, Default)]
pub struct phys_trigger_event {
    pub trigger: u32,
    pub body: u32,
    pub kind: u32,
    pub step: u32,
}

#[repr(C)]
pub struct phys_world {
    _private: [u8; 0],
}

#[repr(C)]
pub struct phys_comm {
    _private: [u8; 0],
}

pub const PHYS_STAGE_COUNT: usize = 14;
pub const PHYS_COMM_ID_BYTES: usize = 128;
pub const PHYS_HALO_BODY_RECORD_BYTES: usize = 96;

#[repr(C)]
#[derive(Clone, Copy)]
pub struct phys_profile {
    pub ms: [f64; PHYS_STAGE_COUNT],
    pub launches: [u64; PHYS_STAGE_COUNT],
    pub steps: u64,
}

#[repr(C)]
#[derive(Clone, Copy)]
pub struct phys_device_view {
    pub n: u64,
    pub pos: *mut f32,
    pub rot: *mut f32,
    pub lin_vel: *mut f32,
    pub ang_vel: *mut f32,
    pub aabb: *mut f32,
    pub stream: *mut c_void,
    pub vel_stride: u64,
}

extern "C" {
    pub fn phys_config_default(cfg: *mut phys_config);
    pub fn phys_last_error() -> *const c_char;
    pub fn phys_abi_version() -> u32;
    pub fn phys_create(cfg: *const phys_config, out: *mut *mut phys_world) -> i32;
    pub fn phys_destroy(w: *mut phys_world) -> i32;
    pub fn phys_set_bodies(w: *mut phys_world, n: u64, pos: *const f32, rot_ijkw: *const f32, lin_vel: *const f32,
                           ang_vel: *const f32, mass: *const f32, inertia: *const f32, shape_type: *const u32,
                           half_extent: *const f32) -> i32;
    pub fn phys_add_constraint_fix_point(w: *mut phys_world, body: u64, target: *const f32) -> i32;
    pub fn phys_add_constraint_fix_orientation(w: *mut phys_world, body: u64, target_rpy: *const f32) -> i32;
    pub fn phys_clear_constraints(w: *mut phys_world) -> i32;
    pub fn phys_apply_force_centre_of_gravity(w: *mut phys_world, body: u64, force: *const f32) -> i32;
    pub fn phys_apply_force_at_position(w: *mut phys_world, body: u64, force: *const f32, point: *const f32) -> i32;
    pub fn phys_apply_force_at_offset(w: *mut phys_world, body: u64, force: *const f32, offset: *const f32) -> i32;
    pub fn phys_set_forces(w: *mut phys_world, force: *const f32, torque: *const f32) -> i32;
    pub fn phys_update(w: *mut phys_world, dt_nanos: u64) -> i32;
    pub fn phys_apply_gravity(w: *mut phys_world) -> i32;
    pub fn phys_step(w: *mut phys_world, dt_nanos: u64) -> i32;
    pub fn phys_update_n(w: *mut phys_world, dt_nanos: u64, n: u32) -> i32;
    pub fn phys_sync(w: *mut phys_world) -> i32;
    pub fn phys_get_transforms(w: *mut phys_world, pos_out: *mut f32, rot_ijkw_out: *mut f32) -> i32;
    pub fn phys_get_velocities(w: *mut phys_world, lin_out: *mut f32, ang_out: *mut f32) -> i32;
    pub fn phys_get_forces(w: *mut phys_world, force_out: *mut f32, torque_out: *mut f32) -> i32;
    pub fn phys_get_instance_matrices(w: *mut phys_world, out: *mut f32) -> i32;
    pub fn phys_get_lambda(w: *mut phys_world, lambda_out: *mut f32, cap: u64, n_rows: *mut u64) -> i32;
    pub fn phys_block_spmv(device: i32, nrows: u64, ncols: u64, nblocks: u64, block_desc: *const u64, data: *const f32,
                           vec: *const f32, vec_len: u64, transpose: i32, out: *mut f32) -> i32;
    pub fn phys_broadphase(w: *mut phys_world, pairs_out: *mut u32, cap: u64, n_pairs: *mut u64) -> i32;
    pub fn phys_get_aabbs(w: *mut phys_world, out: *mut f32) -> i32;
    pub fn phys_get_manifolds(w: *mut phys_world, ids_out: *mut u32, counts_out: *mut u32, normals_out: *mut f32,
                              points_out: *mut f32, cap: u64, n_manifolds: *mut u64) -> i32;
    pub fn phys_get_stats(w: *mut phys_world, out: *mut phys_stats) -> i32;
    pub fn phys_get_color_counts(w: *mut phys_world, counts_out: *mut u32) -> i32;
    pub fn phys_raycast(w: *mut phys_world, n_rays: u64, origin: *const f32, dir: *const f32, max_t: *const f32,
                        ignore_body: *const u32, body_out: *mut u32, t_out: *mut f32, normal_out: *mut f32) -> i32;
    pub fn phys_raycast_device(w: *mut phys_world, n_rays: u64, origin: *const f32, dir: *const f32, max_t: *const f32,
                               ignore_body: *const u32, body_out: *mut u32, t_out: *mut f32, normal_out: *mut f32) -> i32;
    pub fn phys_spherecast(w: *mut phys_world, n: u64, origin: *const f32, dir: *const f32, radius: *const f32, max_t: *const f32,
                           ignore_body: *const u32, body_out: *mut u32, t_out: *mut f32, normal_out: *mut f32) -> i32;
    pub fn phys_spherecast_device(w: *mut phys_world, n: u64, origin: *const f32, dir: *const f32, radius: *const f32,
                                  max_t: *const f32, ignore_body: *const u32, body_out: *mut u32, t_out: *mut f32,
                                  normal_out: *mut f32) -> i32;
    pub fn phys_overlap(w: *mut phys_world, n: u64, shape_type: *const u32, pos: *const f32, rot_ijkw: *const f32,
                        half_extent: *const f32, ignore_body: *const u32, cap: u64, offsets_out: *mut u64, ids_out: *mut u32) -> i32;
    pub fn phys_set_static_bodies(w: *mut phys_world, n: u64, pos: *const f32, rot_ijkw: *const f32, shape_type: *const u32,
                                  half_extent: *const f32) -> i32;
    pub fn phys_set_body_filters(w: *mut phys_world, n: u64, category: *const u16, mask: *const u16, group: *const i16) -> i32;
    pub fn phys_get_body_filters(w: *mut phys_world, category_out: *mut u16, mask_out: *mut u16, group_out: *mut i16) -> i32;
    pub fn phys_set_static_filters(w: *mut phys_world, n: u64, category: *const u16, mask: *const u16, group: *const i16) -> i32;
    pub fn phys_set_ground_filter(w: *mut phys_world, category: u16, mask: u16) -> i32;
    pub fn phys_set_body_materials(w: *mut phys_world, n: u64, friction: *const f32, restitution: *const f32) -> i32;
    pub fn phys_get_body_materials(w: *mut phys_world, friction_out: *mut f32, restitution_out: *mut f32) -> i32;
    pub fn phys_set_static_materials(w: *mut phys_world, n: u64, friction: *const f32, restitution: *const f32) -> i32;
    pub fn phys_set_ground_material(w: *mut phys_world, friction: f32, restitution: f32) -> i32;
    pub fn phys_set_restitution_threshold(w: *mut phys_world, v: f32) -> i32;
    pub fn phys_raycast_filtered(w: *mut phys_world, n_rays: u64, origin: *const f32, dir: *const f32, max_t: *const f32,
                                 ignore_body: *const u32, query_mask: *const u16, body_out: *mut u32, t_out: *mut f32,
                                 normal_out: *mut f32) -> i32;
    pub fn phys_raycast_device_filtered(w: *mut phys_world, n_rays: u64, origin: *const f32, dir: *const f32, max_t: *const f32,
                                        ignore_body: *const u32, query_mask: *const u16, body_out: *mut u32, t_out: *mut f32,
                                        normal_out: *mut f32) -> i32;
    pub fn phys_spherecast_filtered(w: *mut phys_world, n: u64, origin: *const f32, dir: *const f32, radius: *const f32,
                                    max_t: *const f32, ignore_body: *const u32, query_mask: *const u16, body_out: *mut u32,
                                    t_out: *mut f32, normal_out: *mut f32) -> i32;
    pub fn phys_spherecast_device_filtered(w: *mut phys_world, n: u64, origin: *const f32, dir: *const f32, radius: *const f32,
                                           max_t: *const f32, ignore_body: *const u32, query_mask: *const u16, body_out: *mut u32,
                                           t_out: *mut f32, normal_out: *mut f32) -> i32;
    pub fn phys_overlap_filtered(w: *mut phys_world, n: u64, shape_type: *const u32, pos: *const f32, rot_ijkw: *const f32,
                                 half_extent: *const f32, ignore_body: *const u32, query_mask: *const u16, cap: u64,
                                 offsets_out: *mut u64, ids_out: *mut u32) -> i32;
    pub fn phys_get_static_stats(w: *mut phys_world, n_static: *mut u64, n_static_pairs: *mut u64, n_static_manifolds: *mut u64) -> i32;
    pub fn phys_contact_events_enable(w: *mut phys_world, capacity: u64) -> i32;
    pub fn phys_get_contact_events(w: *mut phys_world, out: *mut phys_contact_event, cap: u64, n: *mut u64, n_dropped: *mut u64) -> i32;
    pub fn phys_get_contact_impulses(w: *mut phys_world, out: *mut f32, cap: u64, n_manifolds: *mut u64) -> i32;
    pub fn phys_set_triggers(w: *mut phys_world, n: u64, shape_type: *const u32, pos: *const f32, rot_ijkw: *const f32, half_extent: *const f32, mask: *const u16) -> i32;
    pub fn phys_set_trigger_poses(w: *mut phys_world, n: u64, pos: *const f32, rot_ijkw: *const f32) -> i32;
    pub fn phys_trigger_events_enable(w: *mut phys_world, capacity: u64) -> i32;
    pub fn phys_get_trigger_events(w: *mut phys_world, out: *mut phys_trigger_event, cap: u64, n: *mut u64, n_dropped: *mut u64) -> i32;
    pub fn phys_get_trigger_overlaps(w: *mut phys_world, cap: u64, offsets_out: *mut u64, ids_out: *mut u32) -> i32;
    pub fn phys_profile_enable(w: *mut phys_world, on: i32) -> i32;
    pub fn phys_profile_get(w: *mut phys_world, out: *mut phys_profile) -> i32;
    pub fn phys_get_device_view(w: *mut phys_world, out: *mut phys_device_view) -> i32;
    pub fn phys_set_global_ids(w: *mut phys_world, global_ids: *const u32) -> i32;
    pub fn phys_halo_pack(w: *mut phys_world, x_lo: f32, x_hi: f32, reach: f32, dev_records_out: *mut c_void, cap: u64,
                          n_records: *mut u64) -> i32;
    pub fn phys_halo_pairs(w: *mut phys_world, dev_remote_records: *const c_void, n_remote: u64, skip_first: u64,
                           skip_count: u64, n_cross_pairs: *mut u64) -> i32;
    pub fn phys_get_cross_pairs(w: *mut phys_world, pairs_out: *mut u32, cap: u64, n_pairs: *mut u64) -> i32;
    pub fn phys_set_slab(w: *mut phys_world, x_lo: f32, x_hi: f32, reach: f32) -> i32;
    pub fn phys_halo_pack_bodies(w: *mut phys_world, dev_records_out: *mut c_void, cap: u64) -> i32;
    pub fn phys_halo_pack_bodies_face(w: *mut phys_world, dev_records_out: *mut c_void, cap: u64, face: i32) -> i32;
    pub fn phys_halo_unpack_ghosts(w: *mut phys_world, dev_records: *const c_void, n_records: u64, skip_first: u64,
                                   skip_count: u64) -> i32;
    pub fn phys_get_global_ids(w: *mut phys_world, out: *mut u32) -> i32;
    pub fn phys_comm_unique_id(id_out: *mut u8) -> i32;
    pub fn phys_comm_create(w: *mut phys_world, id: *const u8, rank: i32, n_ranks: i32, capacity: u64,
                            out: *mut *mut phys_comm) -> i32;
    pub fn phys_comm_create_local(worlds: *mut *mut phys_world, n: i32, capacity: u64, comms_out: *mut *mut phys_comm) -> i32;
    pub fn phys_comm_destroy(c: *mut phys_comm) -> i32;
    pub fn phys_comm_set_neighbours(c: *mut phys_comm, enable: i32) -> i32;
    pub fn phys_halo_exchange(w: *mut phys_world, c: *mut phys_comm) -> i32;
    pub fn phys_halo_exchange_all(worlds: *mut *mut phys_world, comms: *mut *mut phys_comm, n: i32) -> i32;
    pub fn phys_slab_histogram(pos: *const f32, n: u64, x_min: f32, x_max: f32, bins: u32, hist: *mut u64) -> i32;
    pub fn phys_slab_cuts(hist: *const u64, bins: u32, x_min: f32, x_max: f32, n_ranks: i32, cuts_out: *mut f32) -> i32;
    pub fn phys_slab_owners(pos: *const f32, n: u64, cuts: *const f32, n_ranks: i32, owner_out: *mut i32) -> i32;
}
```

Before: 213.8 million body-steps/s.

## Classify broadphase pairs by contact likelihood and add box-box sliver early exit

The brick pair-finding kernel can now tag each overlapping AABB pair as likely or unlikely to touch and writes likely pairs first in each flushed chunk, so narrowphase waves see more uniform work. Narrowphase box-box gains an early exit that skips face clipping when the separating-axis data already shows a thin sliver contact that would be discarded anyway. The sliver exit is on by default, while pair classes switch on through a heuristic on the previous step's pair and manifold counts. A debug API to read the pair order is added. The early exit uses different thresholds from the existing post-clip sliver test, so contact sets may change slightly.

```diff
diff --git a/include/physics_hip.h b/include/physics_hip.h
--- a/include/physics_hip.h
+++ b/include/physics_hip.h
@@ -114,6 +114,7 @@
                         const float* data, const float* vec, uint64_t vec_len, int32_t transpose, float* out);
 
 int32_t phys_broadphase(phys_world* w, uint32_t* pairs_out , uint64_t cap, uint64_t* n_pairs);
+int32_t phys_get_pair_order(phys_world* w, uint32_t* pairs_out , uint64_t cap, uint64_t* n_pairs);
 int32_t phys_get_aabbs(phys_world* w, float* out );
 int32_t phys_get_manifolds(phys_world* w, uint32_t* ids_out , uint32_t* counts_out ,
                            float* normals_out , float* points_out , uint64_t cap,
diff --git a/include/spec/collide.h b/include/spec/collide.h
--- a/include/spec/collide.h
+++ b/include/spec/collide.h
@@ -252,7 +252,22 @@
     manifold_reduce(cand, cdep, nc, n_ab, m);
 }
 
-PHYS_HD void collide_box_box(const geom_t* A, const geom_t* B, float margin, manifold_t* m, clip_ws_t* ws) {
+PHYS_HD int box_face_sliver_exit(v3 cRef, v3 hRef, v3 cInc, v3 hInc, int r, float sr, float sr1, float sr2, float c0,
+                                 float c1, float c2, float margin) {
+    const float kw = 0.05f, kd = 0.125f;
+    int j = 0; float dj = c0;
+    if (det_absf(c1) > det_absf(dj)) { j = 1; dj = c1; }
+    if (det_absf(c2) > det_absf(dj)) { j = 2; dj = c2; }
+    const int j1 = (j + 1) % 3, j2 = (j + 2) % 3;
+    const int r1 = (r + 1) % 3, r2 = (r + 2) % 3;
+    const float face = det_minf(det_minf(v3_get(hRef, r1), v3_get(hRef, r2)), det_minf(v3_get(hInc, j1), v3_get(hInc, j2)));
+    const float far = det_maxf(det_maxf(det_maxf(det_absf(cRef.x), det_absf(cRef.y)), det_absf(cRef.z)),
+                               det_maxf(det_maxf(det_absf(cInc.x), det_absf(cInc.y)), det_absf(cInc.z)));
+    if (!(far <= 4096.0f * face)) return 0;
+    return det_minf(-sr1, -sr2) < kw * face && -sr < kd * margin;
+}
+
+PHYS_HD void collide_box_box_early(const geom_t* A, const geom_t* B, float margin, manifold_t* m, clip_ws_t* ws, const int early) {
     const v3 d = v3_sub(B->c, A->c);
     float C[3][3], absC[3][3], tA[3], tB[3], hA[3], hB[3];
     hA[0] = A->h.x; hA[1] = A->h.y; hA[2] = A->h.z;
@@ -271,9 +286,11 @@
     for (int j = 0; j < 3; ++j) tB[j] = v3_dot(d, m33_col(&B->R, j));
 
     float aMax = -3.0e38f; int aAxis = 0;
+    float sA[3], sB[3];
     PHYS_UNROLL
     for (int i = 0; i < 3; ++i) {
         const float s = det_absf(tA[i]) - (hA[i] + ((absC[i][0] * hB[0] + absC[i][1] * hB[1]) + absC[i][2] * hB[2]));
+        sA[i] = s;
         if (s > margin) return;
         if (s > aMax) { aMax = s; aAxis = i; }
     }
@@ -281,6 +298,7 @@
     PHYS_UNROLL
     for (int j = 0; j < 3; ++j) {
         const float s = det_absf(tB[j]) - (hB[j] + ((absC[0][j] * hA[0] + absC[1][j] * hA[1]) + absC[2][j] * hA[2]));
+        sB[j] = s;
         if (s > margin) return;
         if (s > bMax) { bMax = s; bAxis = j; }
     }
@@ -341,15 +359,34 @@
         const float sgn = sel3(tB, bAxis) > 0.0f ? -1.0f : 1.0f;
         const v3 nref = v3_scale(m33_col(&B->R, bAxis), sgn);
         m->normal = v3_neg(nref);
+        if (early) {
+            const int r = bAxis, r1 = (r + 1) % 3, r2 = (r + 2) % 3;
+            const float c0 = r == 0 ? C[0][0] : (r == 1 ? C[0][1] : C[0][2]);
+            const float c1 = r == 0 ? C[1][0] : (r == 1 ? C[1][1] : C[1][2]);
+            const float c2 = r == 0 ? C[2][0] : (r == 1 ? C[2][1] : C[2][2]);
+            if (box_face_sliver_exit(B->c, B->h, A->c, A->h, r, bMax, sel3(sB, r1), sel3(sB, r2), c0, c1, c2, margin)) return;
+        }
         box_face_contact(B, A, bAxis, sgn, margin, m->normal, m, ws);
     } else {
         const float sgn = sel3(tA, aAxis) < 0.0f ? -1.0f : 1.0f;
         m->normal = v3_scale(m33_col(&A->R, aAxis), sgn);
+        if (early) {
+            const int r = aAxis, r1 = (r + 1) % 3, r2 = (r + 2) % 3;
+            const float c0 = r == 0 ? C[0][0] : (r == 1 ? C[1][0] : C[2][0]);
+            const float c1 = r == 0 ? C[0][1] : (r == 1 ? C[1][1] : C[2][1]);
+            const float c2 = r == 0 ? C[0][2] : (r == 1 ? C[1][2] : C[2][2]);
+            if (box_face_sliver_exit(A->c, A->h, B->c, B->h, r, aMax, sel3(sA, r1), sel3(sA, r2), c0, c1, c2, margin)) return;
+        }
         box_face_contact(A, B, aAxis, sgn, margin, m->normal, m, ws);
     }
 }
 
-PHYS_HD void collide_pair_sphere_box(const geom_t* A, const geom_t* B, float margin, manifold_t* m, clip_ws_t* ws) {
+PHYS_HD void collide_box_box(const geom_t* A, const geom_t* B, float margin, manifold_t* m, clip_ws_t* ws) {
+    collide_box_box_early(A, B, margin, m, ws, 0);
+}
+
+PHYS_HD void collide_pair_sphere_box_early(const geom_t* A, const geom_t* B, float margin, manifold_t* m, clip_ws_t* ws,
+                                           const int early) {
     manifold_clear(m);
     if (A->type == PHYS_SPEC_SHAPE_SPHERE && B->type == PHYS_SPEC_SHAPE_SPHERE) {
         collide_sphere_sphere(A, B, margin, m);
@@ -359,8 +396,11 @@
         collide_sphere_box_raw(B, A, margin, m);
         m->normal = v3_neg(m->normal);
     } else if (A->type == PHYS_SPEC_SHAPE_BOX && B->type == PHYS_SPEC_SHAPE_BOX) {
-        collide_box_box(A, B, margin, m, ws);
-    }
+        collide_box_box_early(A, B, margin, m, ws, early);
+    }
+}
+PHYS_HD void collide_pair_sphere_box(const geom_t* A, const geom_t* B, float margin, manifold_t* m, clip_ws_t* ws) {
+    collide_pair_sphere_box_early(A, B, margin, m, ws, 0);
 }
 
 PHYS_HD void collide_ground_sphere_box(const geom_t* A, float ground, float margin, manifold_t* m, clip_ws_t* ws) {
@@ -621,7 +661,7 @@
     else if (B->type == PHYS_SPEC_SHAPE_BOX) collide_capsule_box(A, B, margin, m);
 }
 
-PHYS_HD void collide_pair(const geom_t* A, const geom_t* B, float margin, manifold_t* m, clip_ws_t* ws) {
+PHYS_HD void collide_pair_early(const geom_t* A, const geom_t* B, float margin, manifold_t* m, clip_ws_t* ws, const int early) {
     if (A->type == PHYS_SPEC_SHAPE_CAPSULE) {
         manifold_clear(m);
         collide_capsule_any(A, B, margin, m);
@@ -632,8 +672,11 @@
             m->normal = v3_neg(m->normal);
         }
     } else {
-        collide_pair_sphere_box(A, B, margin, m, ws);
-    }
+        collide_pair_sphere_box_early(A, B, margin, m, ws, early);
+    }
+}
+PHYS_HD void collide_pair(const geom_t* A, const geom_t* B, float margin, manifold_t* m, clip_ws_t* ws) {
+    collide_pair_early(A, B, margin, m, ws, 0);
 }
 
 PHYS_HD void collide_capsule_ground(const geom_t* A, float ground, float margin, manifold_t* m) {
diff --git a/physics_amd/_abi.py b/physics_amd/_abi.py
--- a/physics_amd/_abi.py
+++ b/physics_amd/_abi.py
@@ -175,6 +175,7 @@
     "phys_get_lambda": (C.c_int32, [C.c_void_p, f32p, C.c_uint64, u64p]),
     "phys_block_spmv": (C.c_int32, [C.c_int32, C.c_uint64, C.c_uint64, C.c_uint64, u64p, f32p, f32p, C.c_uint64, C.c_int32, f32p]),
     "phys_broadphase": (C.c_int32, [C.c_void_p, u32p, C.c_uint64, u64p]),
+    "phys_get_pair_order": (C.c_int32, [C.c_void_p, u32p, C.c_uint64, u64p]),
     "phys_get_aabbs": (C.c_int32, [C.c_void_p, f32p]),
     "phys_get_manifolds": (C.c_int32, [C.c_void_p, u32p, u32p, f32p, f32p, C.c_uint64, u64p]),
     "phys_get_stats": (C.c_int32, [C.c_void_p, C.POINTER(PhysStats)]),
diff --git a/physics_amd/csrc/abi.hip b/physics_amd/csrc/abi.hip
--- a/physics_amd/csrc/abi.hip
+++ b/physics_amd/csrc/abi.hip
@@ -142,6 +142,8 @@
         s.flow_quad_max = debug_env("PHYS_DEBUG_FLOW_QUAD_MAX", parse_u64).value_or(0);
         s.flow_pipeline = debug_env("PHYS_DEBUG_FLOW_PIPELINE", parse_one);
         s.np_early_probe = debug_env("PHYS_DEBUG_NP_EARLY_PROBE", parse_one);
+        s.np_sliver_exit = debug_env("PHYS_DEBUG_NP_SLIVER_EXIT", parse_one);
+        s.pair_classes = debug_env("PHYS_DEBUG_PAIR_CLASSES", parse_one);
         s.no_flow_preference = debug_set("PHYS_DEBUG_NO_FLOW_PREFERENCE");
         s.flow_stall = debug_set("PHYS_DEBUG_FLOW_STALL");
         s.flow_epoch = debug_env("PHYS_DEBUG_FLOW_EPOCH", [](const char* v) { return (uint32_t)strtoul(v, nullptr, 0); }).value_or(0u);
@@ -563,6 +565,18 @@
     return sorted_pairs_to_host(w, pairs_out, cap, n_pairs);
 }
 
+int32_t phys_get_pair_order(phys_world* w, uint32_t* pairs_out, uint64_t cap, uint64_t* n_pairs) {
+    ENTER(w);
+    if (!n_pairs) return fail(PHYS_ERR_INVALID_ARG, "null n_pairs");
+    PHYS_TRY(fetch_counters(w));
+    if (w->h_counters->overflow & kOvfPairs) return fail(PHYS_ERR_CAPACITY, "pair capacity exceeded: raise phys_config.max_pairs");
+    const uint64_t m = w->h_counters->n_pairs;
+    *n_pairs = m;
+    if (!pairs_out || m == 0) return PHYS_OK;
+    PHYS_HIP_TRY(hipMemcpy(pairs_out, w->pairs.p, 8 * (m < cap ? m : cap), hipMemcpyDeviceToHost));
+    return PHYS_OK;
+}
+
 int32_t phys_get_manifolds(phys_world* w, uint32_t* ids_out, uint32_t* counts_out, float* normals_out,
                            float* points_out, uint64_t cap, uint64_t* n_manifolds) {
     ENTER(w);
diff --git a/physics_amd/csrc/broadphase.hip b/physics_amd/csrc/broadphase.hip
--- a/physics_amd/csrc/broadphase.hip
+++ b/physics_amd/csrc/broadphase.hip
@@ -4,6 +4,7 @@
 #include <cstdlib>
 
 #include "kernels.hpp"
+#include "pair_class.hpp"
 
 namespace phys {
 
@@ -157,13 +158,63 @@
 
 constexpr int kBrickLanesPerBody = 4;
 
-template <int kBrickStagePerWave>
-__device__ __forceinline__ void workgroup_flush(PairStage& st, uint32_t* s_cnt, uint32_t* s_base, uint32_t* __restrict__ pairs,
+struct ClassStage {
+    uint32_t* lds;
+    uint32_t n_likely;
+    uint32_t n_unlikely;
+};
+
+template <int kStageCap>
+__device__ __forceinline__ void stage_flush_classes(ClassStage& st, uint32_t* __restrict__ pairs, uint64_t max_pairs,
+                                                    StepCounters* __restrict__ ctr) {
+    const uint32_t lane = threadIdx.x & 63u;
+    const uint32_t count = st.n_likely + st.n_unlikely;
+    if (count == 0) return;
+    uint32_t base = 0;
+    if (lane == 0) base = atomicAdd(&ctr->n_pairs, count);
+    base = (uint32_t)__shfl((int)base, 0, 64);
+    if ((uint64_t)base + count > max_pairs) {
+        if (lane == 0) flag_overflow(ctr, kOvfPairs);
+    }
+    for (uint32_t k = lane; k < count; k += 64) {
+        const uint64_t dst = (uint64_t)base + k;
+        const uint32_t src = k < st.n_likely ? k : (uint32_t)kStageCap - 1u - (k - st.n_likely);
+        if (dst < max_pairs) reinterpret_cast<uint2*>(pairs)[dst] = reinterpret_cast<const uint2*>(st.lds)[src];
+    }
+    st.n_likely = 0;
+    st.n_unlikely = 0;
+}
+
+template <int kStageCap, bool kClasses>
+__device__ __forceinline__ void stage_push_classes(ClassStage& st, bool hit, bool likely, uint32_t a, uint32_t b,
+                                                   uint32_t* __restrict__ pairs, uint64_t max_pairs,
+                                                   StepCounters* __restrict__ ctr) {
+    const unsigned long long mask = __ballot(hit);
+    if (mask == 0ull) return;
+    const unsigned long long lmask = kClasses ? __ballot(hit && likely) : mask;
+    const uint32_t hits = (uint32_t)__popcll(mask), lhits = kClasses ? (uint32_t)__popcll(lmask) : hits;
+    if (st.n_likely + st.n_unlikely + hits > (uint32_t)kStageCap) stage_flush_classes<kStageCap>(st, pairs, max_pairs, ctr);
+    if (hit) {
+        const uint32_t lrank = lane_rank(lmask);
+        uint32_t at = st.n_likely + lrank;
+        if (kClasses && !likely) at = (uint32_t)kStageCap - 1u - (st.n_unlikely + (lane_rank(mask) - lrank));
+        reinterpret_cast<uint2*>(st.lds)[at] = make_uint2(a, b);
+    }
+    st.n_likely += lhits;
+    if (kClasses) st.n_unlikely += hits - lhits;
+}
+
+template <int kBrickStagePerWave, bool kClasses>
+__device__ __forceinline__ void workgroup_flush(ClassStage& st, uint32_t* s_cnt, uint32_t* s_base, uint32_t* __restrict__ pairs,
                                                 uint64_t max_pairs, StepCounters* __restrict__ ctr, bool force) {
     const uint32_t wave = threadIdx.x >> 6, lane = threadIdx.x & 63u;
-    if (lane == 0) s_cnt[wave] = st.count;
+    if (lane == 0) {
+        s_cnt[wave] = st.n_likely;
+        if (kClasses) s_cnt[4 + wave] = st.n_unlikely;
+    }
     __syncthreads();
-    const uint32_t total = s_cnt[0] + s_cnt[1] + s_cnt[2] + s_cnt[3];
+    const uint32_t total_likely = s_cnt[0] + s_cnt[1] + s_cnt[2] + s_cnt[3];
+    const uint32_t total = total_likely + (kClasses ? s_cnt[4] + s_cnt[5] + s_cnt[6] + s_cnt[7] : 0u);
     const bool go = total != 0u && (force || total >= (uint32_t)(2 * kBrickStagePerWave));
     if (go && threadIdx.x == 0) {
         const uint32_t base = atomicAdd(&ctr->n_pairs, total);
@@ -172,31 +223,39 @@
     }
     __syncthreads();
     if (go) {
-        uint32_t off = *s_base;
-        for (uint32_t k = 0; k < wave; ++k) off += s_cnt[k];
-        for (uint32_t k = lane; k < st.count; k += 64) {
-            const uint64_t dst = (uint64_t)off + k;
+        uint32_t off_l = *s_base, off_u = *s_base + total_likely;
+        for (uint32_t k = 0; k < wave; ++k) { off_l += s_cnt[k]; if (kClasses) off_u += s_cnt[4 + k]; }
+        for (uint32_t k = lane; k < st.n_likely; k += 64) {
+            const uint64_t dst = (uint64_t)off_l + k;
             if (dst < max_pairs) reinterpret_cast<uint2*>(pairs)[dst] = reinterpret_cast<const uint2*>(st.lds)[k];
         }
-        st.count = 0;
+        for (uint32_t k = lane; kClasses && k < st.n_unlikely; k += 64) {
+            const uint64_t dst = (uint64_t)off_u + k;
+            if (dst < max_pairs)
+                reinterpret_cast<uint2*>(pairs)[dst] = reinterpret_cast<const uint2*>(st.lds)[(uint32_t)kBrickStagePerWave - 1u - k];
+        }
+        st.n_likely = 0;
+        st.n_unlikely = 0;
     }
     __syncthreads();
 }
 
-template <int kBrickStagePerWave>
+template <int kBrickStagePerWave, bool kClasses>
 __global__ __launch_bounds__(kPairThreads, 7) void k_find_pairs_brick(const uint32_t* __restrict__ bucket_start, uint32_t n_bricks,
                                                                    GridShape g, const uint32_t* __restrict__ sorted_ids,
                                                                    const float* __restrict__ sorted_box,
                                                                    uint32_t* __restrict__ pairs, uint64_t max_pairs,
-                                                                   StepCounters* __restrict__ ctr, uint32_t cap) {
+                                                                   StepCounters* __restrict__ ctr, uint32_t cap,
+                                                                   float margin ) {
     __shared__ uint32_t stage[(kPairThreads / 64) * kBrickStagePerWave * 2];
     __shared__ uint32_t s_gstart[kRegCells];
     __shared__ uint32_t s_off[kRegCells + 1];
     extern __shared__ float s_rec[];
-    __shared__ uint32_t s_wsum[4], s_cnt[4], s_base;
-    PairStage st;
+    __shared__ uint32_t s_wsum[4], s_cnt[8], s_base;
+    ClassStage st;
     st.lds = stage + (threadIdx.x >> 6) * kBrickStagePerWave * 2;
-    st.count = 0;
+    st.n_likely = 0;
+    st.n_unlikely = 0;
     const float inv_cell = grid_inv_cell(ctr);
     const uint32_t sub = threadIdx.x % kBrickLanesPerBody;
     uint32_t first = blockIdx.x, last = n_bricks, step = gridDim.x;
@@ -297,7 +356,7 @@
                 }
                 const bool own_cell = c == 0;
                 while (__any(t < t_end)) {
-                    bool hit = false;
+                    bool hit = false, likely = true;
                     uint32_t j = 0;
                     if (t < t_end) {
                         aabb_t bj;
@@ -312,15 +371,20 @@
                             bj.hi = ld3(sorted_box, 2 * t + 1);
                         }
                         hit = aabb_overlap(bi, bj) && (!own_cell || i < j);
+                        if (kClasses) {
+                            const float alo[3] = {bi.lo.x, bi.lo.y, bi.lo.z}, ahi[3] = {bi.hi.x, bi.hi.y, bi.hi.z};
+                            const float blo[3] = {bj.lo.x, bj.lo.y, bj.lo.z}, bhi[3] = {bj.hi.x, bj.hi.y, bj.hi.z};
+                            likely = pair_likely_contact(alo, ahi, blo, bhi, margin);
+                        }
                         ++t;
                     }
-                    stage_push<kBrickStagePerWave>(st, hit, i < j ? i : j, i < j ? j : i, pairs, max_pairs, ctr);
+                    stage_push_classes<kBrickStagePerWave, kClasses>(st, hit, likely, i < j ? i : j, i < j ? j : i, pairs, max_pairs, ctr);
                 }
             }
         }
-        workgroup_flush<kBrickStagePerWave>(st, s_cnt, &s_base, pairs, max_pairs, ctr, false);
-    }
-    workgroup_flush<kBrickStagePerWave>(st, s_cnt, &s_base, pairs, max_pairs, ctr, true);
+        workgroup_flush<kBrickStagePerWave, kClasses>(st, s_cnt, &s_base, pairs, max_pairs, ctr, false);
+    }
+    workgroup_flush<kBrickStagePerWave, kClasses>(st, s_cnt, &s_base, pairs, max_pairs, ctr, true);
     if (threadIdx.x == 0 && seen_max > ctr->max_region) atomicMax(&ctr->max_region, seen_max);
 }
 
@@ -542,16 +606,17 @@
     build_sorted_grid(w);
     if (plan.kernel == PairKernel::Brick128 || plan.kernel == PairKernel::Brick256) {
         static bool attr_set[64] = {};
-        (void)allow_dynamic_lds(attr_set, w->device, {reinterpret_cast<const void*>(&k_find_pairs_brick<128>),
-                                                      reinterpret_cast<const void*>(&k_find_pairs_brick<256>)}, 150 * 1024);
+        (void)allow_dynamic_lds(attr_set, w->device, {reinterpret_cast<const void*>(&k_find_pairs_brick<128, false>),
+                                                      reinterpret_cast<const void*>(&k_find_pairs_brick<256, false>),
+                                                      reinterpret_cast<const void*>(&k_find_pairs_brick<128, true>),
+                                                      reinterpret_cast<const void*>(&k_find_pairs_brick<256, true>)}, 150 * 1024);
         const uint32_t n_bricks = T >> 6;
         PHYS_PROF(w, PHYS_STAGE_PAIRS);
-        if (plan.kernel == PairKernel::Brick128)
-            hipLaunchKernelGGL(k_find_pairs_brick<128>, wgs, tb, plan.lds, s, w->bucket_start.p, n_bricks, axis_mask,
-                               w->sorted_ids.p, w->sorted_box.p, w->pairs.p, w->max_pairs, w->counters.p, plan.cap);
-        else
-            hipLaunchKernelGGL(k_find_pairs_brick<256>, wgs, tb, plan.lds, s, w->bucket_start.p, n_bricks, axis_mask,
-                               w->sorted_ids.p, w->sorted_box.p, w->pairs.p, w->max_pairs, w->counters.p, plan.cap);
+        dispatch_bool(plan.kernel == PairKernel::Brick128, [&](auto small_t) { dispatch_bool(plan.classes != 0u, [&](auto cls_t) {
+            constexpr int kStage = decltype(small_t)::value ? 128 : 256;
+            hipLaunchKernelGGL((k_find_pairs_brick<kStage, decltype(cls_t)::value>), wgs, tb, plan.lds, s, w->bucket_start.p, n_bricks, axis_mask,
+                               w->sorted_ids.p, w->sorted_box.p, w->pairs.p, w->max_pairs, w->counters.p, plan.cap, w->cfg.contact_margin);
+        }); });
         return;
     }
     PHYS_PROF(w, PHYS_STAGE_PAIRS);
diff --git a/physics_amd/csrc/narrowphase.hip b/physics_amd/csrc/narrowphase.hip
--- a/physics_amd/csrc/narrowphase.hip
+++ b/physics_amd/csrc/narrowphase.hip
@@ -28,6 +28,7 @@
     StepCounters* __restrict__ ctr,
     uint64_t max_static_pairs ,
     const uint32_t* __restrict__ static_pairs, const float* __restrict__ static_geo ,
+    uint32_t sliver_exit ,
     Filt... filt ) {
     static_assert(sizeof...(Filt) == (kFilters ? 1u : 0u), "one NpFilters argument exactly in the filtered instance");
     NpFilters flt{};
@@ -100,8 +101,8 @@
                     }
                     const geom_t ga = load_geom(a, geo);
                     const geom_t gb = body_pair ? load_geom(b, geo) : load_geom(pr.y, static_geo);
-                    if (kCapsules) collide_pair(&ga, &gb, margin, &m, ws);
-                    else collide_pair_sphere_box(&ga, &gb, margin, &m, ws);
+                    if (kCapsules) collide_pair_early(&ga, &gb, margin, &m, ws, (int)sliver_exit);
+                    else collide_pair_sphere_box_early(&ga, &gb, margin, &m, ws, (int)sliver_exit);
                 }
             }
             const bool has = m.count > 0;
@@ -259,7 +260,7 @@
                                w->max_pairs, w->geo.p, w->cfg.contact_margin, w->cfg.ground_height, w->max_manifolds, w->man_a.p, w->man_b.p,
                                w->man_color.p, w->man_geo.p, w->man_prio.p, w->color_state.p, w->color_state.p + n,
                                reinterpret_cast<ulonglong2*>(w->ctab.p), cache_mask, plan.early_probe, stamp, w->unc_list.p,
-                               w->warm ? w->man_prev.p : nullptr, w->man_imp.p, w->counters.p, st_cap, st_pairs, st_geo, filters...);
+                               w->warm ? w->man_prev.p : nullptr, w->man_imp.p, w->counters.p, st_cap, st_pairs, st_geo, plan.sliver_exit, filters...);
         };
         if constexpr (FLT) launch(flt); else launch();
     }); }); }); });
diff --git a/physics_amd/csrc/pair_class.hpp b/physics_amd/csrc/pair_class.hpp
--- /dev/null
+++ b/physics_amd/csrc/pair_class.hpp
@@ -0,0 +1,26 @@
+#pragma once
+
+#if defined(__HIPCC__)
+#define PHYS_PAIR_CLASS_HD __host__ __device__ __forceinline__
+#else
+#define PHYS_PAIR_CLASS_HD inline
+#endif
+
+namespace phys {
+
+PHYS_PAIR_CLASS_HD int pair_class_axis(float alo, float ahi, float blo, float bhi, float margin) {
+    const float o = (ahi < bhi ? ahi : bhi) - (alo > blo ? alo : blo);
+    const float ea = ahi - alo, eb = bhi - blo;
+    const float e = ea < eb ? ea : eb;
+    return o > 0.25f * e ? 2 : (o - 2.0f * margin >= 0.1f * margin ? 1 : 0);
+}
+
+PHYS_PAIR_CLASS_HD bool pair_likely_contact(const float alo[3], const float ahi[3], const float blo[3], const float bhi[3],
+                                            float margin) {
+    const int x = pair_class_axis(alo[0], ahi[0], blo[0], bhi[0], margin), y = pair_class_axis(alo[1], ahi[1], blo[1], bhi[1], margin),
+              z = pair_class_axis(alo[2], ahi[2], blo[2], bhi[2], margin);
+    const int wide = (x == 2) + (y == 2) + (z == 2);
+    return wide >= 2 || (x != 0 && y != 0 && z != 0);
+}
+
+}
diff --git a/physics_amd/csrc/plan.hpp b/physics_amd/csrc/plan.hpp
--- a/physics_amd/csrc/plan.hpp
+++ b/physics_amd/csrc/plan.hpp
@@ -33,6 +33,7 @@
     int np_threads = 0, pair_lanes = 0, brick_stage = 0;
     bool raycast_stats = false;
     std::optional<bool> flow_pipeline, np_early_probe;
+    std::optional<bool> np_sliver_exit, pair_classes;
     std::optional<bool> color_kernel_lane;
     std::optional<bool> pair_kernel_brick;
 };
@@ -87,6 +88,7 @@
     uint32_t cap = 0;
     size_t lds = 0;
     uint32_t wgs = 0;
+    uint32_t classes = 0;
 };
 inline PairPlan plan_pairs(const PlanInputs& in, const StepHint& h, const DebugSwitches& dbg) {
     PairPlan p;
@@ -113,6 +115,7 @@
         p.cap = cap;
         p.lds = dyn;
         p.wgs = wgs;
+        p.classes = dbg.pair_classes.value_or(h.valid && (uint64_t)h.n_pairs >= 3ull * in.n && 2ull * h.n_manifolds < (uint64_t)h.n_pairs);
         return p;
     }
     if (dbg.pair_lanes ? dbg.pair_lanes == 4 : n <= 65536u) {
@@ -128,12 +131,14 @@
 struct NarrowPlan {
     int threads = 512;
     uint32_t early_probe = 0;
+    uint32_t sliver_exit = 1;
     bool statics = false, capsules = false, filters = false;
     uint32_t blocks = 1;
 };
 inline NarrowPlan plan_narrowphase(const PlanInputs& in, const StepHint& h, const DebugSwitches& dbg) {
     NarrowPlan p;
     p.early_probe = dbg.np_early_probe.value_or(!h.valid || 2ull * h.n_manifolds >= (uint64_t)h.n_pairs);
+    p.sliver_exit = dbg.np_sliver_exit.value_or(true);
     const bool few = h.valid ? h.n_manifolds <= 32768u : (uint32_t)in.n <= 200000u;
     p.threads = (dbg.np_threads ? dbg.np_threads : (few ? 128 : 512)) == 128 ? 128 : 512;
     p.statics = in.statics; p.capsules = in.capsules; p.filters = in.filters;
diff --git a/physics_amd/world.py b/physics_amd/world.py
--- a/physics_amd/world.py
+++ b/physics_amd/world.py
@@ -278,6 +278,14 @@
         out = np.empty((n.value, 2), np.uint32)
         if n.value:
             self._ck(self.lib.phys_broadphase(self.h, _p(out, u32p), n.value, C.byref(n)))
+        return out
+
+    def get_pair_order(self):
+        n = C.c_uint64()
+        self._ck(self.lib.phys_get_pair_order(self.h, None, 0, C.byref(n)))
+        out = np.empty((n.value, 2), np.uint32)
+        if n.value:
+            self._ck(self.lib.phys_get_pair_order(self.h, _p(out, u32p), n.value, C.byref(n)))
         return out
 
     def get_aabbs(self):
diff --git a/rust/physics_hip_sys/src/lib.rs b/rust/physics_hip_sys/src/lib.rs
--- a/rust/physics_hip_sys/src/lib.rs
+++ b/rust/physics_hip_sys/src/lib.rs
@@ -160,6 +160,7 @@
     pub fn phys_block_spmv(device: i32, nrows: u64, ncols: u64, nblocks: u64, block_desc: *const u64, data: *const f32,
                            vec: *const f32, vec_len: u64, transpose: i32, out: *mut f32) -> i32;
     pub fn phys_broadphase(w: *mut phys_world, pairs_out: *mut u32, cap: u64, n_pairs: *mut u64) -> i32;
+    pub fn phys_get_pair_order(w: *mut phys_world, pairs_out: *mut u32, cap: u64, n_pairs: *mut u64) -> i32;
     pub fn phys_get_aabbs(w: *mut phys_world, out: *mut f32) -> i32;
     pub fn phys_get_manifolds(w: *mut phys_world, ids_out: *mut u32, counts_out: *mut u32, normals_out: *mut f32,
                               points_out: *mut f32, cap: u64, n_manifolds: *mut u64) -> i32;
```

Result: slower. 211.6 million body-steps/s (-1.0%).
